# nl1xx/simple-multimodal

Hardware: AMD Instinct MI355X
Metric: fusion fwd+bwd samples/sec at B=16 d=768 (higher is better)
Workload: dtype bf16

## Files before the change

### include/mmfusion.h

```cpp
#ifndef MMFUSION_H
#define MMFUSION_H

#include <stddef.h>
#include <stdint.h>

#ifdef __cplusplus
extern "C" {
#endif

#define MMF_ABI_VERSION 1

enum {
  MMF_OK = 0,
  MMF_E_SHAPE = -1,
  MMF_E_DTYPE = -2,
  MMF_E_ALIGN = -3,
  MMF_E_LAUNCH = -4,
  MMF_E_UNSUPPORTED = -5
};

int mmf_version(void);
const char* mmf_last_error(void);
int mmf_device_cu_count(void);

#define MMF_GEMM_MAX_PROBLEMS 48
enum { MMF_GEMM_NT = 0, MMF_GEMM_NN = 1, MMF_GEMM_TN = 2 };
enum {
  MMF_EPI_BIAS = 1,
  MMF_EPI_RELU = 2,
  MMF_EPI_MASK_AUX = 4,
  MMF_EPI_ADD_AUX = 8,
  MMF_EPI_ACCUM = 16,
  MMF_EPI_COLSUM_A = 32,
  MMF_EPI_DROPOUT = 64
};

typedef struct mmf_gemm_problem {
  const void* A;
  const void* B;
  void* C;
  const float* bias;
  const void* aux;
  int32_t M, N, K;
  int32_t lda, ldb, ldc, ldaux;
} mmf_gemm_problem;

int mmf_gemm_grouped(const mmf_gemm_problem* problems, int num_problems, int layout,
                     int epilogue, int out_f32, void* stream);
typedef struct mmf_gemm_extra {
  float alpha;
  float dropout_p;
  const uint64_t* rng_state;
  uint32_t site;
} mmf_gemm_extra;
int mmf_gemm_grouped_ex(const mmf_gemm_problem* problems, int num_problems, int layout, int epilogue,
                        int out_f32, const mmf_gemm_extra* extra, void* stream);

int mmf_gemm_select_impl(int impl);
int mmf_gemm_last_impl(void);
int mmf_gemm_set_persistent_workgroups(int n);
int mmf_gemm7_set_tile_n(int n);
int mmf_gemm7_last_tile_n(void);
int mmf_gemm7_tile_n(const mmf_gemm_problem* problems, int num_problems, int workgroups);

#define MMF_SKINNY_MAX_PROBLEMS 24
typedef struct mmf_skinny_problem {
  const void* X;
  const void* W;
  void* Y;
  const float* bias;
  const void* aux;
  int32_t M, N, K;
  int32_t ldx, ldw, ldy, ldaux;
} mmf_skinny_problem;
int mmf_skinny_linear_fwd(const mmf_skinny_problem* problems, int num_problems, int flags, int out_f32, void* stream);
int mmf_skinny_linear_dgrad(const mmf_skinny_problem* problems, int num_problems, int flags, float alpha, int out_f32,
                            void* stream);
int mmf_skinny_last_strip(void);
typedef struct mmf_skinny_problem_ex {
  mmf_skinny_problem p;
  void* Y2;
  const void* gate;
  void* dz;
  int32_t ldy2, ldgate, lddz, reserved;
} mmf_skinny_problem_ex;
typedef struct mmf_skinny_extra {
  int32_t x_f32;
  int32_t gate_f32;
  float gate_scale;
  float dropout_p;
  const uint64_t* rng_state;
  uint32_t site;
  uint32_t reserved;
} mmf_skinny_extra;
int mmf_skinny_linear_fwd_ex(const mmf_skinny_problem_ex* problems, int num_problems, int flags, int out_f32,
                             const mmf_skinny_extra* extra, void* stream);
int mmf_skinny_linear_dgrad_ex(const mmf_skinny_problem_ex* problems, int num_problems, int flags, float alpha, int out_f32,
                               const mmf_skinny_extra* extra, void* stream);

int mmf_fusion_loss(const float* logits, int ldl, const int64_t* targets, int B, int C, float label_smoothing,
                    const float* const* extra, const float* extra_w, int n_extra, float* loss, float* dlogits, void* stream);
int mmf_modality_dropout(const float* const* x, float* const* y, float* keep, int B, int d, float p,
                         const uint64_t* rng_state, uint32_t site, int draw, void* stream);

int mmf_distill_kl(const float* student, int lds, const float* teacher, int ldt, int B, int C, float temperature,
                   float* loss, float* dstudent, void* stream);
int mmf_fusion_loss_kd(const float* logits, int ldl, const int64_t* targets, int B, int C, float label_smoothing,
                       const float* const* extra, const float* extra_w, int n_extra,
                       const float* teacher, int ldt, float temperature, float kd_weight,
                       float* loss, float* dlogits, void* stream);

int mmf_robust_head_fwd(const float* const f[3], const float* h, const float* W2, const float* b2,
                        const float* const Wm[3], const float* const bm[3], int avail, float* a, float* const p[3],
                        float* wn, float* y, int B, int d, int C, void* stream);
int mmf_robust_head_bwd(const float* const f[3], const float* h, const float* W2, const float* const Wm[3],
                        const float* a, const float* const p[3], const float* wn, int avail, const float* g,
                        const float* const dP[3], const float* dA, const float* dN, float* const df[3], float* dh,
                        float* dW2, float* db2, float* const dWm[3], float* const dbm[3], int B, int d, int C, void* stream);

int mmf_fewshot_proto_fwd(const float* const s[3], float* sf, float* mean, int n_way, int n_shot, int d, void* stream);
int mmf_fewshot_proto_bwd(const float* dmean, const float* dsf, float* ds, int n_way, int n_shot, int d, void* stream);
int mmf_fewshot_dist_fwd(const float* const q[3], const float* P, float* qf, float* dist, float* pred, int Nq, int n_way,
                         int d, void* stream);
int mmf_fewshot_dist_bwd(const float* qf, const float* P, const float* dist, const float* pred, const float* gdist,
                         const float* gpred, float* dq, float* dp, int Nq, int n_way, int d, void* stream);

#define MMF_EVAL_MAX_HEADS 4
#define MMF_EVAL_NSUMS 4
int mmf_eval_accumulate(const float* const* logits, const int* ld, int n_heads, const int64_t* targets, int B, int C,
                        float label_smoothing, int64_t* counts, double* sums, int64_t* pred_out, int64_t* target_out,
                        float* prob_out, int64_t row0, int64_t capacity, void* stream);

#define MMF_ATTN_MAX_PROBLEMS 12
typedef struct mmf_attn_problem {
  const void* Q; const void* K; const void* V;
  void* O;
  float* LSE;
  const void* dO;
  float* delta;
  void* dQ; void* dK; void* dV;
  int32_t B, H, Tq, Tk;
  int32_t ldq, ldk, ldv, ldo;
} mmf_attn_problem;

int mmf_attn_fwd_grouped(const mmf_attn_problem* problems, int num_problems, int head_dim,
                         float scale, void* stream);
int mmf_attn_bwd_grouped(const mmf_attn_problem* problems, int num_problems, int head_dim,
                         float scale, void* stream);
int mmf_attn_fwd_grouped_ex(const mmf_attn_problem* problems, int num_problems, int head_dim, float scale,
                            float dropout_p, const uint64_t* rng_state, uint32_t site, void* stream);
int mmf_attn_select_impl(int impl);
int mmf_attn_bwd_grouped_ex(const mmf_attn_problem* problems, int num_problems, int head_dim, float scale,
                            float dropout_p, const uint64_t* rng_state, uint32_t site, void* stream);

#define MMF_LN_MAX_PROBLEMS 8
typedef struct mmf_ln_problem {
  const void* x;
  void* y;
  const float* gamma;
  const float* beta;
  float* mean;
  float* rstd;
  const void* dy;
  void* dx;
  float* dgamma;
  float* dbeta;
  int32_t rows;
} mmf_ln_problem;

int mmf_layernorm_fwd_grouped(const mmf_ln_problem* problems, int num_problems, int d, float eps,
                              void* stream);
size_t mmf_layernorm_bwd_workspace_bytes(int d);
int mmf_layernorm_bwd_grouped(const mmf_ln_problem* problems, int num_problems, int d,
                              void* workspace, size_t workspace_bytes, void* stream);
int mmf_layernorm_last_form(void);

int mmf_cast_f32_to_bf16(const float* src, void* dst, int64_t n, void* stream);
int mmf_cast_bf16_to_f32(const void* src, float* dst, int64_t n, void* stream);
int mmf_cast_f32_to_bf16_2d(const float* src, void* dst, int rows, int cols, int ld_src, void* stream);
int mmf_cast_bf16_to_f32_scaled(const void* src, float* dst, int64_t n, float scale, void* stream);
int mmf_add3_bf16(const void* a, const void* b, const void* c, void* y, int64_t n, void* stream);
#define MMF_ADD3_MAX 8
typedef struct mmf_add3_problem {
  const void* a; const void* b; const void* c;
  void* y;
  int64_t n;
} mmf_add3_problem;
int mmf_add3_grouped(const mmf_add3_problem* problems, int num_problems, void* stream);
#define MMF_ADDN_MAX 8
int mmf_addn_bf16(const void* const* xs, int n, void* y, int64_t numel, int out_f32, void* stream);
#define MMF_ADDN_GROUP_MAX 4
typedef struct mmf_addn_problem {
  const void* x[MMF_ADDN_MAX];
  void* y;
  int64_t numel;
  int32_t n;
} mmf_addn_problem;
int mmf_addn_grouped(const mmf_addn_problem* problems, int num_problems, void* stream);
int mmf_meanpool_fwd(const void* x, void* y, int B, int T, int d, int ldy, void* stream);
int mmf_meanpool_bwd(const void* dy, void* dx, int B, int T, int d, int lddy, void* stream);
#define MMF_POOL_MAX 4
int mmf_meanpool_cat_fwd(const void* const* xs, const int* Ts, int n, void* y, int B, int d, int ldy, void* stream);
int mmf_meanpool_cat_bwd(const void* dy, void* const* dxs, const int* Ts, int n, int B, int d, int lddy, void* stream);
int mmf_colsum_bf16(const void* x, float* out, int M, int N, int ldx, void* stream);
#define MMF_COLSUM_MAX_PROBLEMS 24
typedef struct mmf_colsum_problem {
  const void* x;
  float* out;
  int32_t M, N, ldx;
} mmf_colsum_problem;
int mmf_colsum_grouped(const mmf_colsum_problem* problems, int num_problems, void* stream);
int mmf_dropout(const void* x, void* y, int64_t n, int is_f32, float p, const uint64_t* rng_state,
                uint32_t site, void* stream);
#define MMF_ZERO_MAX_RANGES 48
int mmf_zero_ranges_f32(float* base, const int64_t* starts, const int64_t* ends, int n, void* stream);
int mmf_relu_bwd_bf16(const void* dy, const void* y, void* dx, int64_t n, void* stream);
int mmf_relu_bwd_mixed(const void* dy, int dy_f32, const void* y, int y_f32, void* dx, int64_t n, void* stream);

typedef struct mmf_gat3_params {
  int32_t B, heads, C, relu;
  float negative_slope, dropout_p;
  const uint64_t* rng_state;
  uint32_t site;
} mmf_gat3_params;
int mmf_gat3_dense_fwd(const float* h, const float* att_src, const float* att_dst, const float* bias,
                       void* y_bf16, void* pooled_bf16, float* alpha, float* sdots,
                       const mmf_gat3_params* p, void* stream);
int mmf_gat3_dense_bwd(const float* h, const float* att_src, const float* att_dst, const void* y_bf16,
                       const float* alpha, const float* sdots, const void* dy_bf16, const void* dpooled_bf16,
                       float* dh, float* datt_src, float* datt_dst, float* dbias,
                       const mmf_gat3_params* p, void* stream);
int mmf_infonce_fwd(const float* const z[3], float* const n[3], float* inv_norm, float* losses, float* lse,
                    int B, int D, float temperature, void* stream);
int mmf_infonce_bwd(const float* const n[3], const float* inv_norm, const float* lse, const float* const dn[3],
                    const float* const dloss[3], float* const dz[3], int B, int D, float temperature, void* stream);
int mmf_adaptive_combine_fwd(const float* hp, const float* W2, const float* b2, const float* attended,
                             float* aw, void* weighted_bf16, int B, int d, void* stream);
int mmf_adaptive_combine_bwd(const float* hp, const float* W2, const float* attended, const float* aw,
                             const void* dweighted_bf16, const float* daw, float* dattended, float* dhp,
                             float* dW2, float* db2, int B, int d, void* stream);
int mmf_adaptive_attn_weights(const void* qkv_bf16, float* w, int B, int heads, int head_dim, void* stream);
int mmf_attn_weights_mean(const void* qkv_bf16, float* w, int B, int T, int heads, int head_dim, void* stream);
int mmf_linear_narrow_fwd(const float* x, const float* W, const float* b, float* y, int M, int N, int K, void* stream);
int mmf_linear_narrow_bwd(const float* x, const float* W, const float* dy, float* dx, float* dW, float* db,
                          int M, int N, int K, void* stream);
int mmf_stack3_embed_fwd(const float* f0, const float* f1, const float* f2, const float* emb, void* x_bf16,
                         int B, int d, int ldf, void* stream);
int mmf_stack3_embed_bwd(const void* dx_bf16, float* d0, float* d1, float* d2, float* demb, int B, int d, int ldd,
                         void* stream);
int mmf_rowmask_apply(const float* x, const float* mask, float* y, int B, int d, void* stream);

int mmf_sqnorm_f32(const float* x, int64_t n, float* out, void* stream);
int mmf_adamw_advance(int64_t* step, float* hparams, const double* sched, void* stream);
int mmf_adamw_step(float* master, const float* grad, float* exp_avg, float* exp_avg_sq, void* shadow_bf16,
                   int64_t n, const float* hparams, const float* gnorm_sq, void* stream);

int mmf_gemm_f32_grouped(const mmf_gemm_problem* problems, int num_problems, int layout, int epilogue, float alpha,
                         void* stream);
int mmf_gemm_f32_batched(const mmf_gemm_problem* problem, int layout, int epilogue, float alpha, int nb0, int nb1,
                         const int64_t strideA[2], const int64_t strideB[2], const int64_t strideC[2], void* stream);
int mmf_softmax_rows_f32(float* S, int64_t rows, int cols, float scale, void* stream);
int mmf_softmax_bwd_rows_f32(const float* P, float* dP, int64_t rows, int cols, float scale, void* stream);
int mmf_layernorm_f32_fwd(const float* x, float* y, const float* gamma, const float* beta, float* mean, float* rstd,
                          int rows, int d, float eps, void* stream);
int mmf_layernorm_f32_bwd(const float* x, const float* dy, const float* gamma, const float* mean, const float* rstd,
                          float* dx, float* dgamma, float* dbeta, int rows, int d, void* stream);

typedef struct mmf_bilstm_args {
  const void* gx;
  const void* w_hh[2];
  const float* b_ih[2];
  const float* b_hh[2];
  void* y;
  float* gates;
  float* cell;
  const void* dy;
  void* dgates;
  int32_t T, B, H;
} mmf_bilstm_args;
size_t mmf_bilstm_workspace_bytes(void);
int mmf_bilstm_layer_fwd(const mmf_bilstm_args* args, void* workspace, size_t workspace_bytes, void* stream);
int mmf_bilstm_layer_bwd(const mmf_bilstm_args* args, void* workspace, size_t workspace_bytes, void* stream);

int mmf_swap01(const void* in, void* out, int n0, int n1, int d, int in_f32, int out_f32, void* stream);

int mmf_vit_patchify(const float* pixels, void* patches_bf16, int N, int C, int H, int W, int P, void* stream);
int mmf_vit_embed_tokens(const void* patch_emb_bf16, const float* cls, const float* pos, void* tokens_bf16, int N, int T, int d,
                         void* stream);
int mmf_bias_gelu_bf16(void* x_bf16, const float* bias, int64_t rows, int cols, int ld, void* stream);

#define MMF_W2V_STATS_SLOTS 128
int mmf_w2v_conv0_stats(const float* wave, const float* weight, float* stats, float* partial, int N, int L, int C0, int k0, int s0,
                        void* stream);
int mmf_w2v_conv0_norm_gelu(const float* wave, const float* weight, const float* stats, const float* gamma, const float* beta,
                            void* out_bf16, int N, int L, int C0, int k0, int s0, int k1, int s1, float eps, void* stream);
int mmf_w2v_gelu_window(const void* x_bf16, void* out_bf16, int N, int T_in, int C, int k, int s, void* stream);
int mmf_w2v_posconv(const void* x_bf16, const void* w_bf16, const float* bias, void* y_bf16, int N, int T, int C, int groups, int k,
                    void* stream);

int mmf_deberta_embed(const int64_t* ids, const float* embeds, const float* table, const float* gamma, const float* beta, float eps,
                      const void* mask, int mask_kind, void* out_bf16, int64_t rows, int d, int vocab, void* stream);
int mmf_deberta_attn_fwd(const void* qkv_bf16, const void* posq_bf16, const void* posk_bf16, int ld_pos, const int* idx,
                         const void* mask, int mask_kind, void* out_bf16, int n, int H, int T, int S, int head_dim, float scale,
                         void* stream);

int mmf_video_prepare(const uint8_t* frames, const uint8_t* live, const float* brightness, const uint8_t* flip, float* pixels,
                      int N, int Hs, int Ws, int H, int W, int bgr, void* stream);
int mmf_video_prepare_patches(const uint8_t* frames, const uint8_t* live, const float* brightness, const uint8_t* flip,
                              void* patches_bf16, int N, int Hs, int Ws, int H, int W, int P, int bgr, void* stream);
int mmf_audio_resample(const float* wave, const int* len, const float* table, int64_t table_elems, float* out, int B, int C,
                       int64_t Ls, int64_t L, int orig, int new_, int width, void* stream);
int mmf_audio_augment(const float* x, float* out, const uint8_t* noise_on, const int* stretch_len, const uint64_t* rng_state,
                      uint32_t site, int B, int64_t L, void* stream);

#ifdef __cplusplus
}
#endif
#endif
```

### simple-multimodal_amd/csrc/gemm.hip

```cpp
#include "mmf_internal.h"
#include <stdlib.h>

int mmf_gemm2_launch(const mmf_gemm_problem* problems, int num_problems, int layout, int epilogue,
                     int out_f32, const mmf_gemm_extra* extra, hipStream_t s);
int mmf_gemm6_launch(const mmf_gemm_problem* problems, int num_problems, int layout, int epilogue,
                     int out_f32, const mmf_gemm_extra* extra, hipStream_t s);
bool mmf_gemm6_supports(const mmf_gemm_problem* problems, int num_problems, int layout);
bool mmf_gemm6_supports_epi(int epilogue, int out_f32);
int mmf_gemm7_launch(const mmf_gemm_problem* problems, int num_problems, int layout, int epilogue,
                     int out_f32, const mmf_gemm_extra* extra, hipStream_t s);
bool mmf_gemm7_supports(const mmf_gemm_problem* problems, int num_problems, int layout, int epilogue, int out_f32, const mmf_gemm_extra* extra);

static bool impl_built(int v) { return v == 0 || v == 2 || v == 6 || v == 7; }
static int g_gemm_impl = [] {
  const char* e = getenv("MMF_GEMM_IMPL");
  const int v = (e && e[0] >= '0' && e[0] <= '9') ? e[0] - '0' : 0;
  return impl_built(v) ? v : 0;
}();

static int auto_impl(const mmf_gemm_problem* p, int n, int layout) {
  long tiles = 0;
  for (int i = 0; i < n; ++i) tiles += (long)((p[i].M + 255) / 256) * ((p[i].N + 255) / 256);
  static const int cus = [] { int c = mmf_device_cu_count(); return c > 0 ? c : 256; }();
  const long need = layout == MMF_GEMM_TN ? (cus + 1) / 2 : (cus + 3) / 4;
  return (tiles >= need && mmf_gemm6_supports(p, n, layout)) ? 6 : 2;
}
static int gemm_impl() { return g_gemm_impl; }
static thread_local int t_last_impl = 0;
extern "C" int mmf_gemm_last_impl(void) { return t_last_impl; }
extern "C" int mmf_gemm_select_impl(int impl) {
  if (!impl_built(impl))
    MMF_FAIL(MMF_E_UNSUPPORTED, "mmf_gemm_select_impl: generation %d is not built (0 = automatic, 2, 6, 7; 1 / 3 left in round 3, 4 / 5 in round 4)", impl);
  g_gemm_impl = impl;
  return MMF_OK;
}

extern "C" int mmf_gemm_grouped(const mmf_gemm_problem* problems, int num_problems, int layout,
                                int epilogue, int out_f32, void* stream) {
  return mmf_gemm_grouped_ex(problems, num_problems, layout, epilogue, out_f32, nullptr, stream);
}

extern "C" int mmf_gemm_grouped_ex(const mmf_gemm_problem* problems, int num_problems, int layout,
                                   int epilogue, int out_f32, const mmf_gemm_extra* extra, void* stream) {
  if (!problems || num_problems <= 0 || num_problems > MMF_GEMM_MAX_PROBLEMS)
    MMF_FAIL(MMF_E_SHAPE, "mmf_gemm_grouped: num_problems=%d out of range [1,%d]", num_problems,
             MMF_GEMM_MAX_PROBLEMS);
  if (layout < MMF_GEMM_NT || layout > MMF_GEMM_TN)
    MMF_FAIL(MMF_E_UNSUPPORTED, "mmf_gemm_grouped: unknown layout %d", layout);
  if ((epilogue & MMF_EPI_ACCUM) && !out_f32)
    MMF_FAIL(MMF_E_UNSUPPORTED, "mmf_gemm_grouped: MMF_EPI_ACCUM needs f32 output");
  if ((epilogue & MMF_EPI_MASK_AUX) && (epilogue & MMF_EPI_ADD_AUX))
    MMF_FAIL(MMF_E_UNSUPPORTED, "mmf_gemm_grouped: MASK_AUX and ADD_AUX are exclusive");
  if ((epilogue & MMF_EPI_COLSUM_A) && (layout != MMF_GEMM_TN || (epilogue & MMF_EPI_BIAS)))
    MMF_FAIL(MMF_E_UNSUPPORTED, "mmf_gemm_grouped: COLSUM_A is a TN (wgrad) epilogue and excludes BIAS");
  if (epilogue & MMF_EPI_DROPOUT) {
    if (!extra || !extra->rng_state || !(extra->dropout_p >= 0.f) || extra->dropout_p >= 1.f)
      MMF_FAIL(MMF_E_SHAPE, "mmf_gemm_grouped_ex: MMF_EPI_DROPOUT needs rng_state and 0 <= p < 1");
  }
  int impl = gemm_impl();
  const bool pinned = impl != 0;
  if (impl == 0) impl = auto_impl(problems, num_problems, layout);
  const bool ok6 = mmf_gemm6_supports(problems, num_problems, layout) && mmf_gemm6_supports_epi(epilogue, out_f32);
  if (impl == 6 && !pinned && mmf_gemm7_supports(problems, num_problems, layout, epilogue, out_f32, extra)) impl = 7;
  if (impl == 7 && !mmf_gemm7_supports(problems, num_problems, layout, epilogue, out_f32, extra)) impl = 6;
  if (impl == 6 && !ok6) impl = 2;
  t_last_impl = impl;
  for (int i = 0; i < num_problems; ++i) {
    const mmf_gemm_problem& p = problems[i];
    if (p.M <= 0 || p.N <= 0 || p.K <= 0)
      MMF_FAIL(MMF_E_SHAPE, "mmf_gemm_grouped[%d]: empty problem M=%d N=%d K=%d", i, p.M, p.N, p.K);
    if (!p.A || !p.B || !p.C) MMF_FAIL(MMF_E_SHAPE, "mmf_gemm_grouped[%d]: null operand", i);
    if ((epilogue & (MMF_EPI_BIAS | MMF_EPI_COLSUM_A)) && !p.bias) MMF_FAIL(MMF_E_SHAPE, "mmf_gemm_grouped[%d]: bias is null", i);
    if ((epilogue & (MMF_EPI_MASK_AUX | MMF_EPI_ADD_AUX)) && !p.aux)
      MMF_FAIL(MMF_E_SHAPE, "mmf_gemm_grouped[%d]: aux is null", i);
    const int a_cols = (layout == MMF_GEMM_TN) ? p.M : p.K;
    const int b_cols = (layout == MMF_GEMM_NT) ? p.K : p.N;
    if ((a_cols & 7) || (b_cols & 7) || (p.lda & 7) || (p.ldb & 7) || (p.N & 3) || (p.ldc & 3) ||
        ((epilogue & (MMF_EPI_MASK_AUX | MMF_EPI_ADD_AUX)) && (p.ldaux & 3)))
      MMF_FAIL(MMF_E_ALIGN, "mmf_gemm_grouped[%d]: M=%d N=%d K=%d lda=%d ldb=%d ldc=%d ldaux=%d violate "
               "the 8-element (operands) / 4-element (output) granularity", i, p.M, p.N, p.K, p.lda,
               p.ldb, p.ldc, p.ldaux);
    if (p.lda < a_cols || p.ldb < b_cols || p.ldc < p.N)
      MMF_FAIL(MMF_E_SHAPE, "mmf_gemm_grouped[%d]: leading dimension smaller than the row", i);
    if (!mmf_aligned16(p.A) || !mmf_aligned16(p.B) || !mmf_aligned16(p.C) ||
        (p.bias && !mmf_aligned16(p.bias)) || (p.aux && (reinterpret_cast<uintptr_t>(p.aux) & 7)))
      MMF_FAIL(MMF_E_ALIGN, "mmf_gemm_grouped[%d]: operand pointers must be 16-byte aligned", i);
  }
  hipStream_t s = static_cast<hipStream_t>(stream);
  if (impl == 2) return mmf_gemm2_launch(problems, num_problems, layout, epilogue, out_f32, extra, s);
  if (impl == 6) return mmf_gemm6_launch(problems, num_problems, layout, epilogue, out_f32, extra, s);
  if (impl == 7) return mmf_gemm7_launch(problems, num_problems, layout, epilogue, out_f32, extra, s);
  MMF_FAIL(MMF_E_UNSUPPORTED, "mmf_gemm_grouped: kernel generation %d is not built (2, 6, 7)", impl);
}
```

### simple-multimodal_amd/csrc/gemm7.hip

```cpp
#include <algorithm>
#include <vector>
#include "gemm6_parts.h"

namespace {

constexpr int TILE = 256 * BK * 2, PPO = BK / 8;
template <int TN> struct Form {
  static constexpr int BNT = 64 * TN, TILE_B = BNT * BK * 2, STAGE = TILE + TILE_B, PPB = TN, PPW = PPO + PPB;
  static constexpr int LDS = NS * STAGE + 4 * 8192;
};
static_assert(Form<4>::LDS == 160 * 1024 && Form<3>::LDS == 144 * 1024, "LDS of the two forms");

struct TileSrc {
  const unsigned short* Ab;
  const unsigned short* Bb;
  int recA, recB, stepB, KT;
};
struct TileDst {
  int pi, m0, n0;
};

__device__ __forceinline__ int to_sgpr(int x) {
  int r;
  asm volatile("s_nop 0\n\tv_readfirstlane_b32 %0, %1\n\ts_nop 4" : "=s"(r) : "v"(x));
  return r;
}

template <bool B_KR, int TN>
__device__ __forceinline__ void locate_tile(const GemmArgs& args, const int total_tiles, const int orig, TileSrc& s, TileDst& d, int& lda, int& ldb) {
  const int bid = to_sgpr(mmf_xcd_tile(orig, total_tiles, args.xcd_granule));
  int pi = 0;
  while (pi + 1 < args.nprob && bid >= args.tile_start[pi + 1]) ++pi;
  const mmf_gemm_problem& P = args.p[pi];
  int m0, n0;
  tile_origin<Form<TN>::BNT>(P, bid - args.tile_start[pi], m0, n0);
  m0 = to_sgpr(m0);
  n0 = to_sgpr(n0);
  d.pi = pi; d.m0 = m0; d.n0 = n0;
  lda = P.lda; ldb = P.ldb;
  s.Ab = static_cast<const unsigned short*>(P.A) + (size_t)m0 * P.lda;
  s.Bb = static_cast<const unsigned short*>(P.B) + (B_KR ? (size_t)n0 : (size_t)n0 * P.ldb);
  s.recA = (int)(((long)(P.M - m0 - 1) * P.lda + P.K) * 2);
  s.recB = (int)((B_KR ? ((long)(P.K - 1) * P.ldb + (P.N - n0)) : ((long)(P.N - n0 - 1) * P.ldb + P.K)) * 2);
  s.stepB = (B_KR ? BK * P.ldb : BK) * 2;
  s.KT = P.K / BK;
}

template <int CT, int TN>
__device__ __forceinline__ void drain_tile(const GemmArgs& args, const int pi, const mmf_gemm_problem& P, const int mb, const int nb,
                                           f32x16_t (&acc)[TN][4], char* region, const int lane) {
  constexpr bool AUX = (CT & (MMF_EPI_MASK_AUX | MMF_EPI_ADD_AUX)) != 0;
  constexpr bool DROP = (CT & MMF_EPI_DROPOUT) != 0;
  const unsigned drop_key = DROP ? mmf_rng_key(*args.rng_state, args.site, (unsigned)args.orig[pi]) : 0u;
  const float drop_scale = DROP ? 1.f / (1.f - (float)args.drop_thresh * (1.f / 4294967296.f)) : 1.f;
  const float alpha = (CT & MMF_EPI_MASK_AUX) ? args.alpha : 1.f;
  const int r = lane & 31, h = lane >> 5, q = lane >> 4, cq = lane & 15;
  const unsigned wr_base = (unsigned)(r * 256 + 8 * h + 16 * (r & 15));
  const unsigned rd_base = (unsigned)(q * 256 + ((cq ^ q) << 4));
  auto acc_at = [&](int c) { return region + (wr_base ^ (unsigned)(c << 4)); };
  auto row_at = [&](int it) { return region + it * 1024 + (rd_base ^ (unsigned)((it & 3) << 6)); };
  const bool col_ok = cq < 4 * TN && nb + 8 * cq < P.N;
  const __amdgpu_buffer_rsrc_t crs = __builtin_amdgcn_make_buffer_rsrc(P.C, 0, (int)((((long)P.M - 1) * P.ldc + P.N) * 2), 0x00020000);
  const __amdgpu_buffer_rsrc_t ars = __builtin_amdgcn_make_buffer_rsrc(const_cast<void*>(AUX ? P.aux : P.C), 0,
                                                                       AUX ? (int)((((long)P.M - 1) * P.ldaux + P.N) * 2) : 0, 0x00020000);
  const unsigned c_off0 = col_ok ? (unsigned)(((long)(mb + q) * P.ldc + nb + 8 * cq) * 2) : 0x80000000u;
  const unsigned a_off0 = col_ok ? (unsigned)(((long)(mb + q) * P.ldaux + nb + 8 * cq) * 2) : 0x80000000u;
  const unsigned c_row4 = (unsigned)(4 * P.ldc * 2), a_row4 = (unsigned)(4 * P.ldaux * 2);

  u32x4_t auxr[2][8];
  auto load_aux = [&](int tm, int slot) {
#pragma unroll
    for (int it = 0; it < 8; ++it)
      auxr[slot][it] = __builtin_bit_cast(u32x4_t, __builtin_amdgcn_raw_buffer_load_b128(ars, a_off0 + (unsigned)(8 * tm + it) * a_row4, 0, 0));
  };
  if constexpr (AUX) { load_aux(0, 0); load_aux(1, 1); }
#pragma unroll
  for (int tm = 0; tm < 4; ++tm) {
    u32x2_t axv[TN][4];
    if constexpr (AUX) {
#pragma unroll
      for (int it = 0; it < 8; ++it) *reinterpret_cast<u32x4_t*>(row_at(it)) = auxr[tm & 1][it];
#pragma unroll
      for (int tn = 0; tn < TN; ++tn)
#pragma unroll
        for (int g = 0; g < 4; ++g) axv[tn][g] = *reinterpret_cast<const u32x2_t*>(acc_at(4 * tn + g));
      __builtin_amdgcn_sched_barrier(0);
      if (tm + 2 < 4) load_aux(tm + 2, tm & 1);
      __builtin_amdgcn_sched_barrier(0);
    }
#pragma unroll
    for (int tn = 0; tn < TN; ++tn) {
      asm volatile("" : "+a"(acc[tn][tm]));
#pragma unroll
      for (int g = 0; g < 4; ++g) {
        f32x4_t v = {acc[tn][tm][4 * g], acc[tn][tm][4 * g + 1], acc[tn][tm][4 * g + 2], acc[tn][tm][4 * g + 3]};
        if constexpr (CT & MMF_EPI_RELU) {
#pragma unroll
          for (int e = 0; e < 4; ++e) v[e] = fmaxf(v[e], 0.f);
        }
        if constexpr (DROP) {
          const unsigned idx = (unsigned)(mb + 32 * tm + r) * (unsigned)P.N + (unsigned)(nb + 32 * tn + 8 * g + 4 * h);
#pragma unroll
          for (int e = 0; e < 4; ++e) v[e] = mmf_keep(drop_key, idx + e, args.drop_thresh) ? v[e] * drop_scale : 0.f;
        }
        if constexpr (AUX) {
          const u32x2_t a = axv[tn][g];
          const float a0 = bf16lo(a[0]), a1 = bf16hi(a[0]), a2 = bf16lo(a[1]), a3 = bf16hi(a[1]);
          if constexpr (CT & MMF_EPI_MASK_AUX) {
            v[0] = a0 > 0.f ? v[0] * alpha : 0.f; v[1] = a1 > 0.f ? v[1] * alpha : 0.f;
            v[2] = a2 > 0.f ? v[2] * alpha : 0.f; v[3] = a3 > 0.f ? v[3] * alpha : 0.f;
          } else {
            v[0] += a0; v[1] += a1; v[2] += a2; v[3] += a3;
          }
        }
        *reinterpret_cast<u32x2_t*>(acc_at(4 * tn + g)) = u32x2_t{pack_bf16x2(v[0], v[1]), pack_bf16x2(v[2], v[3])};
      }
      __builtin_amdgcn_sched_barrier(0);
    }
    u32x4_t w[8];
#pragma unroll
    for (int it = 0; it < 8; ++it) w[it] = *reinterpret_cast<const u32x4_t*>(row_at(it));
#pragma unroll
    for (int it = 0; it < 8; ++it) __builtin_amdgcn_raw_buffer_store_b128(w[it], crs, c_off0 + (unsigned)(8 * tm + it) * c_row4, 0, 0);
    __builtin_amdgcn_sched_barrier(0);
  }
}

template <bool B_KR, int CT, int TN>
__device__ __forceinline__ void gemm7_body(const GemmArgs& args, const int total_tiles, char* smem) {
  constexpr bool A_KR = false;
  using F = Form<TN>;
  constexpr int BNT = F::BNT, STAGE = F::STAGE, PPW = F::PPW, NMF = 4 * TN, NRD = 4 + TN;
  constexpr int WA = BK, WB = B_KR ? BNT : BK;

  const int tid = threadIdx.x, lane = tid & 63;
  const int wave = __builtin_amdgcn_readfirstlane(tid >> 6);
  const int wm = wave >> 1, wn = wave & 1;
  const int nwg = gridDim.x;
  const int wid = blockIdx.x;
  auto walk = [&](int round) { return round * nwg + ((round & 1) ? nwg - 1 - wid : wid); };
  int round = 0;
  int orig = walk(0);
  TileSrc ns;
  TileDst cd, nd;
  int KT, lda, ldb;
  locate_tile<B_KR, TN>(args, total_tiles, orig, ns, cd, lda, ldb);
  KT = ns.KT;

  unsigned voff[PPW], voffn[PPW];
  auto set_voff = [&](unsigned (&v)[PPW], int la, int lb) {
#pragma unroll
    for (int i = 0; i < PPO; ++i) v[i] = piece_voff<A_KR>(wave + 4 * i, la, lane);
#pragma unroll
    for (int i = 0; i < TN; ++i) v[PPO + i] = piece_voff<B_KR, BNT>(wave + 4 * i, lb, lane);
  };
  set_voff(voff, lda, ldb);
  char* const my_pieces = smem + wave * 1024;

  struct Desc { int lo, hi, rec; };
  auto mkdesc = [](const unsigned short* p, int rec) {
    const unsigned long long a = (unsigned long long)(uintptr_t)p;
    return Desc{(int)(unsigned)a, (int)((unsigned)(a >> 32) & 0xffffu), rec};
  };
  auto advance = [](Desc& d, int bytes) {
    const unsigned long long a = (((unsigned long long)(unsigned)d.hi << 32) | (unsigned)d.lo) + (unsigned long long)bytes;
    d.lo = (int)(unsigned)a; d.hi = (int)(unsigned)(a >> 32);
    int r;
    asm("s_sub_i32 %0, %1, %2\n\ts_max_i32 %0, %0, 0" : "=s"(r) : "s"(d.rec), "s"(bytes) : "scc");
    d.rec = r;
  };
  Desc dA = mkdesc(ns.Ab, ns.recA);
  Desc dB = mkdesc(ns.Bb, ns.recB);
  constexpr int stepA = BK * 2;
  int stepB = ns.stepB;
  const unsigned lds_pieces = (unsigned)(uintptr_t)(const __attribute__((address_space(3))) char*)my_pieces;
  auto hot_piece = [&](auto ic, const unsigned ring_base) {
    constexpr int I = decltype(ic)::value, OFF = I < PPO ? I * 4096 : TILE + (I - PPO) * 4096;
    const Desc& d = I < PPO ? dA : dB;
    const i32x4_t q = {d.lo, d.hi, d.rec, 0x00020000};
    int m0w;
    asm volatile("s_add_i32 %0, %1, %4\n\ts_nop 0\n\tbuffer_load_dwordx4 %2, %3, 0 offen lds" : "={m0}"(m0w) : "s"(ring_base), "v"(voff[I]), "s"(q), "n"(OFF) : "memory");
    __builtin_amdgcn_sched_barrier(0);
  };

#pragma unroll
  for (int s = 0; s < NS; ++s) {
    const unsigned rb = lds_pieces + (unsigned)(s * STAGE);
    hot_piece(std::integral_constant<int, 0>{}, rb); hot_piece(std::integral_constant<int, 1>{}, rb);
    hot_piece(std::integral_constant<int, 2>{}, rb); hot_piece(std::integral_constant<int, 3>{}, rb);
    if (s + 1 < NS) {
      hot_piece(std::integral_constant<int, 4>{}, rb); hot_piece(std::integral_constant<int, 5>{}, rb);
      hot_piece(std::integral_constant<int, 6>{}, rb);
      if constexpr (TN == 4) hot_piece(std::integral_constant<int, 7>{}, rb);
      advance(dA, stepA); advance(dB, stepB);
    }
  }

  bool has_next = walk(1) < total_tiles;
  nd = cd;
  if (has_next) {
    int la, lb;
    locate_tile<B_KR, TN>(args, total_tiles, walk(1), ns, nd, la, lb);
    set_voff(voffn, la, lb);
  } else {
    ns.recA = 0; ns.recB = 0; ns.stepB = 0;
#pragma unroll
    for (int i = 0; i < PPW; ++i) voffn[i] = voff[i];
  }

  unsigned la0, la1, lb0, lb1;
  Frag4<A_KR>::lane_parts(WA, lane, la0, la1);
  Frag4<B_KR>::lane_parts(WB, lane, lb0, lb1);
  const unsigned smem_base = (unsigned)(uintptr_t)(const __attribute__((address_space(3))) char*)smem;
  const unsigned qa = (unsigned)((WA / 32) * 2048 * 4 * wm);
  const unsigned qb = (unsigned)(B_KR ? 512 * TN * wn : (WB / 32) * 2048 * TN * wn);
  la0 += smem_base + qa; la1 += smem_base + qa;
  lb0 += smem_base + TILE + qb; lb1 += smem_base + TILE + qb;

  f32x16_t acc[TN][4];

  constexpr bool use_bias = (CT & MMF_EPI_BIAS) != 0;
  float bcur[TN] = {};
  auto load_bias = [&](float (&b)[TN], const TileDst& d) {
    const mmf_gemm_problem& P = args.p[d.pi];
    const __amdgpu_buffer_rsrc_t brs = __builtin_amdgcn_make_buffer_rsrc(const_cast<float*>(P.bias), 0, P.N * 4, 0x00020000);
    const unsigned off = (unsigned)((d.n0 + 32 * TN * wn + (lane & 31)) * 4);
#pragma unroll
    for (int tn = 0; tn < TN; ++tn)
      b[tn] = __uint_as_float((unsigned)__builtin_amdgcn_raw_buffer_load_b32(brs, off + (unsigned)(32 * tn * 4), 0, 0));
  };
  auto split3 = [&](float x) {
    const bool lo = lane < 32;
    const unsigned hh = __float_as_uint(x) & 0xffff0000u;
    const float r1 = x - __uint_as_float(hh);
    const unsigned mm = __float_as_uint(r1) & 0xffff0000u;
    const float r2 = r1 - __uint_as_float(mm);
    const unsigned ll = __float_as_uint(r2) & 0xffff0000u;
    const u32x4_t w = {lo ? ((hh >> 16) | mm) : 0u, lo ? (ll >> 16) : 0u, 0u, 0u};
    return __builtin_bit_cast(bf16x8_t, w);
  };
  auto bias_init = [&](const float (&b)[TN]) {
    const f32x16_t zero = {0.f, 0.f, 0.f, 0.f, 0.f, 0.f, 0.f, 0.f, 0.f, 0.f, 0.f, 0.f, 0.f, 0.f, 0.f, 0.f};
    const u32x4_t ow = {lane < 32 ? 0x3f803f80u : 0u, lane < 32 ? 0x00003f80u : 0u, 0u, 0u};
    u32x4_t ones[4] = {ow, ow, ow, ow};
#pragma unroll
    for (int tm = 0; tm < 4; ++tm) asm volatile("" : "+v"(ones[tm]));
#pragma unroll
    for (int tn = 0; tn < TN; ++tn) {
      u32x4_t bw = __builtin_bit_cast(u32x4_t, use_bias ? split3(b[tn]) : __builtin_bit_cast(bf16x8_t, u32x4_t{0u, 0u, 0u, 0u}));
      asm volatile("" : "+v"(bw));
#pragma unroll
      for (int tm = 0; tm < 4; ++tm) {
        acc[tn][tm] = __builtin_amdgcn_mfma_f32_32x32x16_bf16(__builtin_bit_cast(bf16x8_t, bw), __builtin_bit_cast(bf16x8_t, ones[tm]), zero, 0, 0, 0);
        __builtin_amdgcn_sched_barrier(0);
      }
    }
  };
  if constexpr (use_bias) load_bias(bcur, cd);

  vm_wait<PPW * (NS - 2) + PPO>();
  __builtin_amdgcn_s_barrier();
  Frag4<A_KR> fa[2];
  Frag4<B_KR, TN> fb[2];
  fa[0].template issue<WA, 0, 0>(la0, la1);
  fb[0].template issue<WB, 0, 0>(lb0, lb1);
  frag_wait(fa[0], fb[0]);

  auto mf = [&](const Frag4<A_KR>& a, const Frag4<B_KR, TN>& b, int i) {
    const int tm = i / TN, tn = i % TN;
    acc[tn][tm] = __builtin_amdgcn_mfma_f32_32x32x16_bf16(b.get(tn), a.get(tm), acc[tn][tm], 0, 0, 0);
    asm volatile("" ::"a"(acc[tn][tm]));
    __builtin_amdgcn_sched_barrier(0);
  };

  auto stage = [&](const unsigned g, const int kt, const int ksw) {
    unsigned long long swmask;
    const Desc nA = mkdesc(ns.Ab, ns.recA), nB = mkdesc(ns.Bb, ns.recB);
    const unsigned so = (g % NS) * STAGE;
    const unsigned ring_cur = lds_pieces + so, ring_prev = lds_pieces + ((g + NS - 1) % NS) * STAGE;
#pragma unroll
    for (int i = 0; i < NMF; ++i) {
      mf(fa[0], fb[0], i);
      if (i < NRD) MMF_G6_READ(TN, fa[1], fb[1], 1, i, so);
      if (i == NRD)     hot_piece(std::integral_constant<int, 4>{}, ring_prev);
      if (i == NRD + 2) hot_piece(std::integral_constant<int, 5>{}, ring_prev);
      if (i == NRD + 4) hot_piece(std::integral_constant<int, 6>{}, ring_prev);
      if constexpr (TN == 4) { if (i == NRD + 6) hot_piece(std::integral_constant<int, 7>{}, ring_prev); }
    }
    frag_wait(fa[1], fb[1]);
    const unsigned sn = ((g + 1) % NS) * STAGE;
#pragma unroll
    for (int i = 0; i < 4; ++i) mf(fa[1], fb[1], i);
    vm_wait<PPW * (NS - 2)>();
    __builtin_amdgcn_s_barrier();
    __builtin_amdgcn_sched_barrier(0);
#pragma unroll
    for (int i = 4; i < NMF; ++i) {
      mf(fa[1], fb[1], i);
      if (i < 4 + NRD) MMF_G6_READ(TN, fa[0], fb[0], 0, i - 4, sn);
      if (i == 4) {
        advance(dA, stepA);
        advance(dB, stepB);
        asm volatile("" ::"s"(dA.lo), "s"(dA.hi), "s"(dA.rec), "s"(dB.lo), "s"(dB.hi), "s"(dB.rec));
        __builtin_amdgcn_sched_barrier(0);
      }
      if (i == 5) {
        asm volatile("s_cmp_eq_u32 %8, %16\n\t"
                     "s_cselect_b32 %0, %9, %0\n\ts_cselect_b32 %1, %10, %1\n\ts_cselect_b32 %2, %11, %2\n\t"
                     "s_cselect_b32 %3, %12, %3\n\ts_cselect_b32 %4, %13, %4\n\ts_cselect_b32 %5, %14, %5\n\t"
                     "s_cselect_b32 %6, %15, %6\n\ts_cselect_b64 %7, -1, 0"
                     : "+s"(dA.lo), "+s"(dA.hi), "+s"(dA.rec), "+s"(dB.lo), "+s"(dB.hi), "+s"(dB.rec), "+s"(stepB), "=s"(swmask)
                     : "s"(kt), "s"(nA.lo), "s"(nA.hi), "s"(nA.rec), "s"(nB.lo), "s"(nB.hi), "s"(nB.rec), "s"(ns.stepB), "s"(ksw)
                     : "scc");
        __builtin_amdgcn_sched_barrier(0);
      }
      if (i == 6) {
        asm volatile("v_cndmask_b32_e64 %0, %0, %4, %8\n\tv_cndmask_b32_e64 %1, %1, %5, %8\n\t"
                     "v_cndmask_b32_e64 %2, %2, %6, %8\n\tv_cndmask_b32_e64 %3, %3, %7, %8"
                     : "+v"(voff[0]), "+v"(voff[1]), "+v"(voff[2]), "+v"(voff[3])
                     : "v"(voffn[0]), "v"(voffn[1]), "v"(voffn[2]), "v"(voffn[3]), "s"(swmask));
        __builtin_amdgcn_sched_barrier(0);
      }
      if (i == 7) {
        if constexpr (TN == 4)
          asm volatile("v_cndmask_b32_e64 %0, %0, %4, %8\n\tv_cndmask_b32_e64 %1, %1, %5, %8\n\t"
                       "v_cndmask_b32_e64 %2, %2, %6, %8\n\tv_cndmask_b32_e64 %3, %3, %7, %8"
                       : "+v"(voff[4]), "+v"(voff[5]), "+v"(voff[6]), "+v"(voff[7])
                       : "v"(voffn[4]), "v"(voffn[5]), "v"(voffn[6]), "v"(voffn[7]), "s"(swmask));
        else
          asm volatile("v_cndmask_b32_e64 %0, %0, %3, %6\n\tv_cndmask_b32_e64 %1, %1, %4, %6\n\t"
                       "v_cndmask_b32_e64 %2, %2, %5, %6"
                       : "+v"(voff[4]), "+v"(voff[5]), "+v"(voff[6])
                       : "v"(voffn[4]), "v"(voffn[5]), "v"(voffn[6]), "s"(swmask));
        __builtin_amdgcn_sched_barrier(0);
      }
      if (i == NMF - 4) hot_piece(std::integral_constant<int, 0>{}, ring_cur);
      if (i == NMF - 3) hot_piece(std::integral_constant<int, 1>{}, ring_cur);
      if (i == NMF - 2) hot_piece(std::integral_constant<int, 2>{}, ring_cur);
      if (i == NMF - 1) hot_piece(std::integral_constant<int, 3>{}, ring_cur);
    }
    frag_wait(fa[0], fb[0]);
  };

  char* const region = smem + NS * STAGE + wave * 8192;
  unsigned g = 0;
  for (;;) {
    bias_init(bcur);
    const int ksw = KT - NS;
    for (int kt = 0; kt < KT; ++kt, ++g) stage(g, kt, ksw);
    const mmf_gemm_problem& P = args.p[cd.pi];
    const int mb = cd.m0 + 128 * wm, nb = cd.n0 + 32 * TN * wn;
    if constexpr (use_bias) { if (has_next) load_bias(bcur, nd); }
#ifndef MMF_G7_NODRAIN
    drain_tile<CT & ~MMF_EPI_BIAS, TN>(args, cd.pi, P, mb, nb, acc, region, lane);
#else
    if (lane == 0 && mb == -1) static_cast<volatile unsigned short*>(P.C)[0] = (unsigned short)acc[0][0][0];
#endif
    if (!has_next) break;
    ++round;
    orig = walk(round);
    cd = nd;
    KT = ns.KT;
    has_next = walk(round + 1) < total_tiles;
    if (has_next) {
      int la, lb;
      locate_tile<B_KR, TN>(args, total_tiles, walk(round + 1), ns, nd, la, lb);
      set_voff(voffn, la, lb);
    } else {
      ns.recA = 0; ns.recB = 0; ns.stepB = 0;
    }
  }
  vm_wait<0>();
}

template <bool B_KR, int CT, int TN>
__global__ __launch_bounds__(NTHREADS, 1)
void gemm7_persistent_kernel(const GemmArgs args, const int total_tiles) {
  __shared__ __attribute__((aligned(1024))) char smem[Form<TN>::LDS];
  gemm7_body<B_KR, CT, TN>(args, total_tiles, smem);
}

template <bool B_KR, int CT>
void launch7(const GemmArgs& a, int total, int grid, int tile_n, hipStream_t s) {
  if (tile_n == 192) hipLaunchKernelGGL((gemm7_persistent_kernel<B_KR, CT, 3>), dim3(grid), dim3(NTHREADS), 0, s, a, total);
  else               hipLaunchKernelGGL((gemm7_persistent_kernel<B_KR, CT, 4>), dim3(grid), dim3(NTHREADS), 0, s, a, total);
}
bool launch7_select(int layout, int eflags, const GemmArgs* a, int total, int grid, hipStream_t s, int tile_n = 256) {
  if (layout == MMF_GEMM_NT) {
    if (eflags == 0)                                      { if (a) launch7<false, 0>(*a, total, grid, tile_n, s); return true; }
    if (eflags == MMF_EPI_BIAS)                           { if (a) launch7<false, MMF_EPI_BIAS>(*a, total, grid, tile_n, s); return true; }
    if (eflags == (MMF_EPI_BIAS | MMF_EPI_RELU))          { if (a) launch7<false, MMF_EPI_BIAS | MMF_EPI_RELU>(*a, total, grid, tile_n, s); return true; }
    if (eflags == (MMF_EPI_BIAS | MMF_EPI_ADD_AUX))       { if (a) launch7<false, MMF_EPI_BIAS | MMF_EPI_ADD_AUX>(*a, total, grid, tile_n, s); return true; }
    if (eflags == (MMF_EPI_BIAS | MMF_EPI_RELU | MMF_EPI_DROPOUT)) {
      if (a) launch7<false, MMF_EPI_BIAS | MMF_EPI_RELU | MMF_EPI_DROPOUT>(*a, total, grid, tile_n, s);
      return true;
    }
  } else if (layout == MMF_GEMM_NN) {
    if (eflags == 0)                                      { if (a) launch7<true, 0>(*a, total, grid, tile_n, s); return true; }
    if (eflags == MMF_EPI_MASK_AUX)                       { if (a) launch7<true, MMF_EPI_MASK_AUX>(*a, total, grid, tile_n, s); return true; }
    if (eflags == MMF_EPI_ADD_AUX)                        { if (a) launch7<true, MMF_EPI_ADD_AUX>(*a, total, grid, tile_n, s); return true; }
  }
  return false;
}
}

static int g_persistent_wgs = [] { const char* e = getenv("MMF_GEMM7_WGS"); const int v = e ? atoi(e) : 0; return v > 0 ? v : 0; }();
extern "C" int mmf_gemm_set_persistent_workgroups(int n) {
  if (n < 0 || n > 65536) MMF_FAIL(MMF_E_SHAPE, "mmf_gemm_set_persistent_workgroups: %d not in 0..65536", n);
  g_persistent_wgs = n;
  return MMF_OK;
}
static int g_tile_n = 0;
static thread_local int t_last_tile_n = 0;
extern "C" int mmf_gemm7_set_tile_n(int n) {
  if (n != 0 && n != 256 && n != 192) MMF_FAIL(MMF_E_SHAPE, "mmf_gemm7_set_tile_n: %d is not 0, 256 or 192", n);
  g_tile_n = n;
  return MMF_OK;
}
extern "C" int mmf_gemm7_last_tile_n(void) { return t_last_tile_n; }

namespace {
int persistent_grid_cap() {
  static const int cus = [] { int c = mmf_device_cu_count(); return c > 0 ? c : 256; }();
  return g_persistent_wgs > 0 ? g_persistent_wgs : cus;
}
int tiles_of(const mmf_gemm_problem& p, int bn) { return ((p.M + BM - 1) / BM) * ((p.N + bn - 1) / bn); }
long long walk_makespan(const mmf_gemm_problem* problems, const int* order, int n, int bn, int cap, int granule) {
  int start[MMF_GEMM_MAX_PROBLEMS + 1];
  start[0] = 0;
  for (int i = 0; i < n; ++i) start[i + 1] = start[i] + tiles_of(problems[order[i]], bn);
  const int total = start[n], grid = total < cap ? total : cap;
  if (total == 0) return 0;
  static thread_local std::vector<long long> load;
  load.assign(grid, 0);
  for (int o = 0; o < total; ++o) {
    const int round = o / grid, pos = o % grid, wid = (round & 1) ? grid - 1 - pos : pos;
    const int bid = mmf_xcd_tile(o, total, granule);
    const int pi = (int)(std::upper_bound(start, start + n + 1, bid) - start) - 1;
    load[wid] += (long long)problems[order[pi]].K * bn;
  }
  return *std::max_element(load.begin(), load.end());
}
struct TileNMemo {
  int cap, granule, n, width;
  int mnk[3 * MMF_GEMM_MAX_PROBLEMS];
};
int pick_tile_n(const mmf_gemm_problem* problems, const int* order, int n, int cap) {
  const int granule = mmf_xcd_granule();
  static thread_local TileNMemo memo[16];
  static thread_local int used = 0, next = 0;
  TileNMemo key;
  key.cap = cap; key.granule = granule; key.n = n;
  for (int i = 0; i < n; ++i) {
    const mmf_gemm_problem& p = problems[order[i]];
    key.mnk[3 * i] = p.M; key.mnk[3 * i + 1] = p.N; key.mnk[3 * i + 2] = p.K;
  }
  for (int e = 0; e < used; ++e) {
    const TileNMemo& m = memo[e];
    if (m.cap == cap && m.granule == granule && m.n == n && std::equal(key.mnk, key.mnk + 3 * n, m.mnk)) return m.width;
  }
  key.width = walk_makespan(problems, order, n, 192, cap, granule) < walk_makespan(problems, order, n, 256, cap, granule) ? 192 : 256;
  memo[next] = key;
  next = (next + 1) % 16;
  if (used < 16) ++used;
  return key.width;
}
void sort_by_k(const mmf_gemm_problem* problems, int n, int* order) {
  for (int i = 0; i < n; ++i) order[i] = i;
  std::stable_sort(order, order + n, [&](int x, int y) { return problems[x].K > problems[y].K; });
}
}

extern "C" int mmf_gemm7_tile_n(const mmf_gemm_problem* problems, int num_problems, int workgroups) {
  if (!problems || num_problems < 1 || num_problems > MMF_GEMM_MAX_PROBLEMS || workgroups < 0)
    MMF_FAIL(MMF_E_SHAPE, "mmf_gemm7_tile_n: %d problems, %d workgroups", num_problems, workgroups);
  int order[MMF_GEMM_MAX_PROBLEMS];
  sort_by_k(problems, num_problems, order);
  return pick_tile_n(problems, order, num_problems, workgroups > 0 ? workgroups : persistent_grid_cap());
}

bool mmf_gemm7_supports(const mmf_gemm_problem* problems, int num_problems, int layout, int epilogue, int out_f32, const mmf_gemm_extra* extra) {
  if (out_f32 || !launch7_select(layout, epilogue, nullptr, 0, 0, nullptr)) return false;
  if (extra && extra->alpha != 1.f && !(layout == MMF_GEMM_NN && epilogue == MMF_EPI_MASK_AUX)) return false;
  if ((epilogue & MMF_EPI_DROPOUT) && !(extra && extra->rng_state)) return false;
  for (int i = 0; i < num_problems; ++i) {
    const mmf_gemm_problem& p = problems[i];
    if (p.K % BK || p.K < (NS + 1) * BK || (p.N & 7) || (p.ldc & 7) || (p.aux && ((p.ldaux & 7) || !mmf_aligned16(p.aux)))) return false;
  }
  return true;
}

int mmf_gemm7_launch(const mmf_gemm_problem* problems, int num_problems, int layout, int epilogue,
                     int out_f32, const mmf_gemm_extra* extra, hipStream_t s) {
  if (!mmf_gemm7_supports(problems, num_problems, layout, epilogue, out_f32, extra))
    MMF_FAIL(MMF_E_UNSUPPORTED, "mmf_gemm_grouped: the persistent kernel takes NT / NN launches with bf16 output, K %% 32 == 0, K >= %d, N and the "
             "leading dimensions of C / aux multiples of 8, and the flag sets of the fusion step (alpha only with the NN ReLU mask)", (NS + 1) * BK);
  GemmArgs a;
  a.nprob = num_problems;
  a.epi = epilogue;
  a.xcd_granule = mmf_xcd_granule();
  a.alpha = extra ? extra->alpha : 1.f;
  a.drop_thresh = (extra && (epilogue & MMF_EPI_DROPOUT)) ? mmf_drop_thresh(extra->dropout_p) : 0u;
  a.site = extra ? extra->site : 0u;
  a.rng_state = extra ? reinterpret_cast<const unsigned long long*>(extra->rng_state) : nullptr;
  int total = 0;
  int order[MMF_GEMM_MAX_PROBLEMS];
  sort_by_k(problems, num_problems, order);
  const int cap = persistent_grid_cap();
  const int tile_n = g_tile_n ? g_tile_n : pick_tile_n(problems, order, num_problems, cap);
  for (int i = 0; i < num_problems; ++i) {
    const mmf_gemm_problem& p = problems[order[i]];
    const size_t a_bytes = (size_t)p.M * p.lda * 2;
    const size_t b_bytes = (size_t)(layout == MMF_GEMM_NT ? p.N : p.K) * p.ldb * 2;
    const size_t c_bytes = (size_t)p.M * p.ldc * 2, x_bytes = p.aux ? (size_t)p.M * p.ldaux * 2 : 0;
    if (a_bytes >= 0x7fffffffull || b_bytes >= 0x7fffffffull || c_bytes >= 0x7fffffffull || x_bytes >= 0x7fffffffull)
      MMF_FAIL(MMF_E_UNSUPPORTED, "mmf_gemm_grouped[%d]: operand larger than 2 GiB", i);
    a.tile_start[i] = total;
    total += tiles_of(p, tile_n);
    a.p[i] = p;
    a.orig[i] = (short)order[i];
  }
  a.tile_start[num_problems] = total;
  const int grid = total < cap ? total : cap;
  t_last_tile_n = tile_n;
  launch7_select(layout, epilogue, &a, total, grid, s, tile_n);
  MMF_CHECK_LAUNCH("mmf_gemm_grouped(v7)");
  return MMF_OK;
}
```

### simple-multimodal_amd/csrc/layernorm.hip

```cpp
#include "mmf_internal.h"

namespace {

constexpr int ROWS_PER_BLOCK = 4;
constexpr int MAX_CH = 4;

constexpr int FWD_BLOCKS = 1024, FWD_BLOCKS_LARGE = 2048;
constexpr long long FWD_LARGE_ROWS = 20000;
constexpr int BWD_BLOCKS_LANE = 512;
constexpr int BWD_BLOCKS_CHUNK = 2048;

struct LnArgs {
  int nprob;
  int d;
  float eps;
  float* ws;
  int blk_start[MMF_LN_MAX_PROBLEMS + 1];
  mmf_ln_problem p[MMF_LN_MAX_PROBLEMS];
};

template <int NCH>
__global__ __launch_bounds__(256)
void ln_fwd_kernel(const LnArgs a) {
  const int pi = mmf_group_problem(a.blk_start, a.nprob, blockIdx.x);
  const mmf_ln_problem& P = a.p[pi];
  const int lane = threadIdx.x & 63, wave = threadIdx.x >> 6;
  const int row = ((int)blockIdx.x - a.blk_start[pi]) * ROWS_PER_BLOCK + wave;
  if (row >= P.rows) return;
  const int d = a.d;
  const unsigned short* x = static_cast<const unsigned short*>(P.x) + (size_t)row * d;
  float v[NCH][8];
  float s = 0.f;
#pragma unroll
  for (int c = 0; c < NCH; ++c) {
    const int col = (c * 64 + lane) * 8;
    if (col < d) {
      unpack8(*reinterpret_cast<const u32x4_t*>(x + col), v[c]);
#pragma unroll
      for (int e = 0; e < 8; ++e) s += v[c][e];
    } else {
#pragma unroll
      for (int e = 0; e < 8; ++e) v[c][e] = 0.f;
    }
  }
  const float mean = wave_sum(s) / (float)d;
  float q = 0.f;
#pragma unroll
  for (int c = 0; c < NCH; ++c) {
    const int col = (c * 64 + lane) * 8;
    if (col < d) {
#pragma unroll
      for (int e = 0; e < 8; ++e) { const float t = v[c][e] - mean; q += t * t; }
    }
  }
  const float rstd = rsqrtf(wave_sum(q) / (float)d + a.eps);
  unsigned short* y = static_cast<unsigned short*>(P.y) + (size_t)row * d;
#pragma unroll
  for (int c = 0; c < NCH; ++c) {
    const int col = (c * 64 + lane) * 8;
    if (col < d) {
      const f32x4_t g0 = *reinterpret_cast<const f32x4_t*>(P.gamma + col);
      const f32x4_t g1 = *reinterpret_cast<const f32x4_t*>(P.gamma + col + 4);
      const f32x4_t b0 = *reinterpret_cast<const f32x4_t*>(P.beta + col);
      const f32x4_t b1 = *reinterpret_cast<const f32x4_t*>(P.beta + col + 4);
      float o[8];
#pragma unroll
      for (int e = 0; e < 4; ++e) {
        o[e] = (v[c][e] - mean) * rstd * g0[e] + b0[e];
        o[e + 4] = (v[c][e + 4] - mean) * rstd * g1[e] + b1[e];
      }
      *reinterpret_cast<u32x4_t*>(y + col) = pack8(o);
    }
  }
  if (lane == 0) { P.mean[row] = mean; P.rstd[row] = rstd; }
}

template <int NV, int H8>
struct LaneCols {
  static constexpr int EP = 8 * NV + 4 * H8, D = 512 * NV + 256 * H8;
  struct Bf16 { u32x4_t v[NV > 0 ? NV : 1]; u32x2_t t; };
  static __device__ __forceinline__ void load(const unsigned short* row, int lane, Bf16& r) {
#pragma unroll
    for (int c = 0; c < NV; ++c) r.v[c] = *reinterpret_cast<const u32x4_t*>(row + 512 * c + 8 * lane);
    if (H8) r.t = *reinterpret_cast<const u32x2_t*>(row + 512 * NV + 4 * lane);
  }
  static __device__ __forceinline__ void unpack(const Bf16& r, float (&f)[EP]) {
#pragma unroll
    for (int c = 0; c < NV; ++c) {
      float t[8];
      unpack8(r.v[c], t);
#pragma unroll
      for (int e = 0; e < 8; ++e) f[8 * c + e] = t[e];
    }
    if (H8) { f[8 * NV] = bf16lo(r.t[0]); f[8 * NV + 1] = bf16hi(r.t[0]); f[8 * NV + 2] = bf16lo(r.t[1]); f[8 * NV + 3] = bf16hi(r.t[1]); }
  }
  static __device__ __forceinline__ void store(unsigned short* row, int lane, const float (&o)[EP]) {
#pragma unroll
    for (int c = 0; c < NV; ++c) {
      const u32x4_t w = {pack_bf16x2(o[8 * c], o[8 * c + 1]), pack_bf16x2(o[8 * c + 2], o[8 * c + 3]),
                         pack_bf16x2(o[8 * c + 4], o[8 * c + 5]), pack_bf16x2(o[8 * c + 6], o[8 * c + 7])};
      *reinterpret_cast<u32x4_t*>(row + 512 * c + 8 * lane) = w;
    }
    if (H8) {
      const u32x2_t w = {pack_bf16x2(o[8 * NV], o[8 * NV + 1]), pack_bf16x2(o[8 * NV + 2], o[8 * NV + 3])};
      *reinterpret_cast<u32x2_t*>(row + 512 * NV + 4 * lane) = w;
    }
  }
  static __device__ __forceinline__ void load_f32(const float* p, int lane, float (&f)[EP]) {
#pragma unroll
    for (int c = 0; c < NV; ++c)
#pragma unroll
      for (int h = 0; h < 2; ++h) {
        const f32x4_t g = *reinterpret_cast<const f32x4_t*>(p + 512 * c + 8 * lane + 4 * h);
#pragma unroll
        for (int e = 0; e < 4; ++e) f[8 * c + 4 * h + e] = g[e];
      }
    if (H8) {
      const f32x4_t g = *reinterpret_cast<const f32x4_t*>(p + 512 * NV + 4 * lane);
#pragma unroll
      for (int e = 0; e < 4; ++e) f[8 * NV + e] = g[e];
    }
  }
  static __device__ __forceinline__ void store_f32(float* p, int lane, const float (&f)[EP]) {
#pragma unroll
    for (int c = 0; c < NV; ++c)
#pragma unroll
      for (int h = 0; h < 2; ++h)
        *reinterpret_cast<f32x4_t*>(p + 512 * c + 8 * lane + 4 * h) =
            f32x4_t{f[8 * c + 4 * h], f[8 * c + 4 * h + 1], f[8 * c + 4 * h + 2], f[8 * c + 4 * h + 3]};
    if (H8) *reinterpret_cast<f32x4_t*>(p + 512 * NV + 4 * lane) = f32x4_t{f[8 * NV], f[8 * NV + 1], f[8 * NV + 2], f[8 * NV + 3]};
  }
};

template <int NV, int H8>
__global__ __launch_bounds__(256)
void ln_fwd_lane_kernel(const LnArgs a) {
  using LC = LaneCols<NV, H8>;
  constexpr int EP = LC::EP, d = LC::D;
  const int pi = mmf_group_problem(a.blk_start, a.nprob, blockIdx.x);
  const mmf_ln_problem& P = a.p[pi];
  const int lane = threadIdx.x & 63, wave = threadIdx.x >> 6;
  const int nblk = a.blk_start[pi + 1] - a.blk_start[pi];
  const float inv_d = 1.f / (float)d;
  float gam[EP], bet[EP];
  LC::load_f32(P.gamma, lane, gam);
  LC::load_f32(P.beta, lane, bet);
  auto fetch = [&](int row, typename LC::Bf16& r) { LC::load(static_cast<const unsigned short*>(P.x) + (size_t)row * d, lane, r); };
  const int step = nblk * ROWS_PER_BLOCK;
  int row = ((int)blockIdx.x - a.blk_start[pi]) * ROWS_PER_BLOCK + wave;
  typename LC::Bf16 cur, nxt;
  if (row < P.rows) fetch(row, cur);
  for (; row < P.rows; row += step) {
    const bool more = row + step < P.rows;
    if (more) fetch(row + step, nxt);
    float v[EP];
    LC::unpack(cur, v);
    float s = 0.f;
#pragma unroll
    for (int e = 0; e < EP; ++e) s += v[e];
    const float mean = wave_sum(s) * inv_d;
    float q = 0.f;
#pragma unroll
    for (int e = 0; e < EP; ++e) { v[e] -= mean; q += v[e] * v[e]; }
    const float rstd = rsqrtf(wave_sum(q) * inv_d + a.eps);
    float o[EP];
#pragma unroll
    for (int e = 0; e < EP; ++e) o[e] = v[e] * rstd * gam[e] + bet[e];
    LC::store(static_cast<unsigned short*>(P.y) + (size_t)row * d, lane, o);
    if (lane == 0) { P.mean[row] = mean; P.rstd[row] = rstd; }
    if (more) cur = nxt;
  }
}

template <int NCH>
__global__ __launch_bounds__(256)
void ln_bwd_kernel(const LnArgs a) {
  __shared__ float red[2][3][NCH * 512];
  const int pi = mmf_group_problem(a.blk_start, a.nprob, blockIdx.x);
  const mmf_ln_problem& P = a.p[pi];
  const int lane = threadIdx.x & 63, wave = threadIdx.x >> 6;
  const int nblk = a.blk_start[pi + 1] - a.blk_start[pi];
  const int d = a.d;
  float dg[NCH][8], db[NCH][8];
#pragma unroll
  for (int c = 0; c < NCH; ++c)
#pragma unroll
    for (int e = 0; e < 8; ++e) { dg[c][e] = 0.f; db[c][e] = 0.f; }

  for (int row = ((int)blockIdx.x - a.blk_start[pi]) * ROWS_PER_BLOCK + wave; row < P.rows;
       row += nblk * ROWS_PER_BLOCK) {
    const unsigned short* x = static_cast<const unsigned short*>(P.x) + (size_t)row * d;
    const unsigned short* dy = static_cast<const unsigned short*>(P.dy) + (size_t)row * d;
    const float mean = P.mean[row], rstd = P.rstd[row];
    float xh[NCH][8], g[NCH][8];
    float s1 = 0.f, s2 = 0.f;
#pragma unroll
    for (int c = 0; c < NCH; ++c) {
      const int col = (c * 64 + lane) * 8;
      if (col < d) {
        float xv[8], dv[8];
        unpack8(*reinterpret_cast<const u32x4_t*>(x + col), xv);
        unpack8(*reinterpret_cast<const u32x4_t*>(dy + col), dv);
        const f32x4_t g0 = *reinterpret_cast<const f32x4_t*>(P.gamma + col);
        const f32x4_t g1 = *reinterpret_cast<const f32x4_t*>(P.gamma + col + 4);
#pragma unroll
        for (int e = 0; e < 8; ++e) {
          const float gam = e < 4 ? g0[e] : g1[e - 4];
          xh[c][e] = (xv[e] - mean) * rstd;
          g[c][e] = dv[e] * gam;
          s1 += g[c][e];
          s2 += g[c][e] * xh[c][e];
          dg[c][e] += dv[e] * xh[c][e];
          db[c][e] += dv[e];
        }
      } else {
#pragma unroll
        for (int e = 0; e < 8; ++e) { xh[c][e] = 0.f; g[c][e] = 0.f; }
      }
    }
    const float c1 = wave_sum(s1) / (float)d, c2 = wave_sum(s2) / (float)d;
    unsigned short* dx = static_cast<unsigned short*>(P.dx) + (size_t)row * d;
#pragma unroll
    for (int c = 0; c < NCH; ++c) {
      const int col = (c * 64 + lane) * 8;
      if (col < d) {
        float o[8];
#pragma unroll
        for (int e = 0; e < 8; ++e) o[e] = rstd * (g[c][e] - c1 - xh[c][e] * c2);
        *reinterpret_cast<u32x4_t*>(dx + col) = pack8(o);
      }
    }
  }
  if (wave > 0) {
#pragma unroll
    for (int c = 0; c < NCH; ++c)
#pragma unroll
      for (int e = 0; e < 8; ++e) {
        red[0][wave - 1][(c * 64 + lane) * 8 + e] = dg[c][e];
        red[1][wave - 1][(c * 64 + lane) * 8 + e] = db[c][e];
      }
  }
  __syncthreads();
  if (wave == 0) {
    float* wsg = a.ws + (size_t)blockIdx.x * 2 * d;
#pragma unroll
    for (int c = 0; c < NCH; ++c) {
      const int col = (c * 64 + lane) * 8;
      if (col < d) {
        f32x4_t g0, g1, b0, b1;
#pragma unroll
        for (int e = 0; e < 8; ++e) {
          float sg = dg[c][e], sb = db[c][e];
#pragma unroll
          for (int w = 0; w < 3; ++w) { sg += red[0][w][col + e]; sb += red[1][w][col + e]; }
          if (e < 4) { g0[e] = sg; b0[e] = sb; } else { g1[e - 4] = sg; b1[e - 4] = sb; }
        }
        *reinterpret_cast<f32x4_t*>(wsg + col) = g0;
        *reinterpret_cast<f32x4_t*>(wsg + col + 4) = g1;
        *reinterpret_cast<f32x4_t*>(wsg + d + col) = b0;
        *reinterpret_cast<f32x4_t*>(wsg + d + col + 4) = b1;
      }
    }
  }
}

template <int NV, int H8>
__global__ __launch_bounds__(256)
void ln_bwd_lane_kernel(const LnArgs a) {
  using LC = LaneCols<NV, H8>;
  constexpr int EP = LC::EP, d = LC::D;
  __shared__ float red[2][3][64 * EP];
  const int pi = mmf_group_problem(a.blk_start, a.nprob, blockIdx.x);
  const mmf_ln_problem& P = a.p[pi];
  const int lane = threadIdx.x & 63, wave = threadIdx.x >> 6;
  const int nblk = a.blk_start[pi + 1] - a.blk_start[pi];
  const float inv_d = 1.f / (float)d;
  float gam[EP], dg[EP], db[EP];
  LC::load_f32(P.gamma, lane, gam);
#pragma unroll
  for (int e = 0; e < EP; ++e) { dg[e] = 0.f; db[e] = 0.f; }

  struct Row { typename LC::Bf16 x, dy; float mean, rstd; };
  auto fetch = [&](int row, Row& r) {
    LC::load(static_cast<const unsigned short*>(P.x) + (size_t)row * d, lane, r.x);
    LC::load(static_cast<const unsigned short*>(P.dy) + (size_t)row * d, lane, r.dy);
    r.mean = P.mean[row];
    r.rstd = P.rstd[row];
  };
  const int step = nblk * ROWS_PER_BLOCK;
  int row = ((int)blockIdx.x - a.blk_start[pi]) * ROWS_PER_BLOCK + wave;
  Row cur, nxt;
  if (row < P.rows) fetch(row, cur);
  for (; row < P.rows; row += step) {
    const bool more = row + step < P.rows;
    if (more) fetch(row + step, nxt);
    float xv[EP], dv[EP];
    LC::unpack(cur.x, xv);
    LC::unpack(cur.dy, dv);
    const float mean = cur.mean, rstd = cur.rstd;
    float s1 = 0.f, s2 = 0.f;
#pragma unroll
    for (int e = 0; e < EP; ++e) {
      xv[e] = (xv[e] - mean) * rstd;
      const float g = dv[e] * gam[e];
      s1 += g;
      s2 += g * xv[e];
      dg[e] += dv[e] * xv[e];
      db[e] += dv[e];
      dv[e] = g;
    }
    const float c1 = wave_sum(s1) * inv_d, c2 = wave_sum(s2) * inv_d;
    float o[EP];
#pragma unroll
    for (int e = 0; e < EP; ++e) o[e] = rstd * (dv[e] - c1 - xv[e] * c2);
    LC::store(static_cast<unsigned short*>(P.dx) + (size_t)row * d, lane, o);
    if (more) cur = nxt;
  }
  if (wave > 0) {
#pragma unroll
    for (int e = 0; e < EP; ++e) { red[0][wave - 1][e * 64 + lane] = dg[e]; red[1][wave - 1][e * 64 + lane] = db[e]; }
  }
  __syncthreads();
  if (wave == 0) {
    float* wsg = a.ws + (size_t)blockIdx.x * 2 * d;
#pragma unroll
    for (int e = 0; e < EP; ++e)
#pragma unroll
      for (int w = 0; w < 3; ++w) { dg[e] += red[0][w][e * 64 + lane]; db[e] += red[1][w][e * 64 + lane]; }
    LC::store_f32(wsg, lane, dg);
    LC::store_f32(wsg + d, lane, db);
  }
}

constexpr int FIN_SLICES = 64;
__global__ __launch_bounds__(256)
void ln_bwd_finalize_kernel(const LnArgs a) {
  const int pi = blockIdx.y;
  const int col = blockIdx.x * 256 + threadIdx.x;
  if (col >= a.d) return;
  const int b0 = a.blk_start[pi], nb = a.blk_start[pi + 1] - b0;
  const int per = (nb + FIN_SLICES - 1) / FIN_SLICES;
  const int lo = b0 + blockIdx.z * per, hi = min(b0 + nb, lo + per);
  if (lo >= hi) return;
  float sg[4] = {0.f, 0.f, 0.f, 0.f}, sb[4] = {0.f, 0.f, 0.f, 0.f};
  int b = lo;
  for (; b + 4 <= hi; b += 4) {
#pragma unroll
    for (int u = 0; u < 4; ++u) {
      const float* w = a.ws + (size_t)(b + u) * 2 * a.d;
      sg[u] += w[col];
      sb[u] += w[a.d + col];
    }
  }
  for (; b < hi; ++b) {
    const float* w = a.ws + (size_t)b * 2 * a.d;
    sg[0] += w[col];
    sb[0] += w[a.d + col];
  }
  atomicAdd(a.p[pi].dgamma + col, (sg[0] + sg[1]) + (sg[2] + sg[3]));
  atomicAdd(a.p[pi].dbeta + col, (sb[0] + sb[1]) + (sb[2] + sb[3]));
}

thread_local int t_last_form = 0;

using LnKernel = void (*)(const LnArgs);
const LnKernel CHUNK_FWD[MAX_CH] = {ln_fwd_kernel<1>, ln_fwd_kernel<2>, ln_fwd_kernel<3>, ln_fwd_kernel<4>};
const LnKernel CHUNK_BWD[MAX_CH] = {ln_bwd_kernel<1>, ln_bwd_kernel<2>, ln_bwd_kernel<3>, ln_bwd_kernel<4>};
struct LaneWidth { int d, form; LnKernel fwd, bwd; };
template <int NV, int H8>
constexpr LaneWidth lane_width_of() {
  return {LaneCols<NV, H8>::D, 100 + 10 * NV + H8, ln_fwd_lane_kernel<NV, H8>, ln_bwd_lane_kernel<NV, H8>};
}
const LaneWidth LANE_WIDTHS[] = {lane_width_of<0, 1>(), lane_width_of<1, 0>(), lane_width_of<1, 1>(), lane_width_of<2, 0>()};
const LaneWidth* lane_width(int d) {
  for (const LaneWidth& w : LANE_WIDTHS) if (w.d == d) return &w;
  return nullptr;
}

int check_common(const char* who, const mmf_ln_problem* p, int n, int d) {
  if (!p || n <= 0 || n > MMF_LN_MAX_PROBLEMS) MMF_FAIL(MMF_E_SHAPE, "%s: num_problems=%d out of range", who, n);
  if (d <= 0 || (d & 7) || d > MAX_CH * 512) MMF_FAIL(MMF_E_SHAPE, "%s: d=%d must be a multiple of 8, <= 2048", who, d);
  return MMF_OK;
}

int full_blocks(int rows) { return (rows + ROWS_PER_BLOCK - 1) / ROWS_PER_BLOCK; }

int share_blocks(LnArgs& a, const mmf_ln_problem* problems, int num_problems, int budget) {
  long long total_rows = 0;
  for (int i = 0; i < num_problems; ++i) total_rows += problems[i].rows;
  int total = 0;
  for (int i = 0; i < num_problems; ++i) {
    const int rows = problems[i].rows, full = full_blocks(rows);
    const int nb = (int)(((long long)rows * budget + total_rows - 1) / total_rows);
    a.blk_start[i] = total;
    total += nb > full ? full : (nb < 1 ? 1 : nb);
  }
  a.blk_start[num_problems] = total;
  return total;
}

}

extern "C" int mmf_layernorm_last_form(void) { return t_last_form; }

extern "C" int mmf_layernorm_fwd_grouped(const mmf_ln_problem* problems, int num_problems, int d,
                                         float eps, void* stream) {
  if (int rc = check_common("mmf_layernorm_fwd_grouped", problems, num_problems, d)) return rc;
  LnArgs a; a.nprob = num_problems; a.d = d; a.eps = eps; a.ws = nullptr;
  int total = 0;
  long long total_rows = 0;
  for (int i = 0; i < num_problems; ++i) {
    const mmf_ln_problem& p = problems[i];
    if (p.rows <= 0 || !p.x || !p.y || !p.gamma || !p.beta || !p.mean || !p.rstd)
      MMF_FAIL(MMF_E_SHAPE, "mmf_layernorm_fwd_grouped[%d]: null operand or rows=%d", i, p.rows);
    if (!mmf_aligned16(p.x) || !mmf_aligned16(p.y) || !mmf_aligned16(p.gamma) || !mmf_aligned16(p.beta))
      MMF_FAIL(MMF_E_ALIGN, "mmf_layernorm_fwd_grouped[%d]: pointers must be 16-byte aligned", i);
    a.blk_start[i] = total;
    total += full_blocks(p.rows);
    total_rows += p.rows;
    a.p[i] = p;
  }
  a.blk_start[num_problems] = total;
  hipStream_t s = static_cast<hipStream_t>(stream);
  const int budget = total_rows > FWD_LARGE_ROWS ? FWD_BLOCKS_LARGE : FWD_BLOCKS;
  const LaneWidth* lw = lane_width(d);
  if (lw && total > budget) {
    total = share_blocks(a, problems, num_problems, budget);
    hipLaunchKernelGGL(lw->fwd, dim3(total), dim3(256), 0, s, a);
    t_last_form = lw->form;
    MMF_CHECK_LAUNCH("mmf_layernorm_fwd_grouped(lane)");
    return MMF_OK;
  }
  const int nch = (d + 511) / 512;
  hipLaunchKernelGGL(CHUNK_FWD[nch - 1], dim3(total), dim3(256), 0, s, a);
  t_last_form = nch;
  MMF_CHECK_LAUNCH("mmf_layernorm_fwd_grouped");
  return MMF_OK;
}

extern "C" size_t mmf_layernorm_bwd_workspace_bytes(int d) {
  return (size_t)(BWD_BLOCKS_CHUNK + MMF_LN_MAX_PROBLEMS) * 2 * (size_t)(d > 0 ? d : 0) * sizeof(float);
}

extern "C" int mmf_layernorm_bwd_grouped(const mmf_ln_problem* problems, int num_problems, int d,
                                         void* workspace, size_t workspace_bytes, void* stream) {
  if (int rc = check_common("mmf_layernorm_bwd_grouped", problems, num_problems, d)) return rc;
  if (!workspace || workspace_bytes < mmf_layernorm_bwd_workspace_bytes(d) || !mmf_aligned16(workspace))
    MMF_FAIL(MMF_E_SHAPE, "mmf_layernorm_bwd_grouped: workspace of %zu bytes (16-byte aligned) required",
             mmf_layernorm_bwd_workspace_bytes(d));
  LnArgs a; a.nprob = num_problems; a.d = d; a.eps = 0.f; a.ws = static_cast<float*>(workspace);
  for (int i = 0; i < num_problems; ++i) {
    const mmf_ln_problem& p = problems[i];
    if (p.rows <= 0 || !p.x || !p.dy || !p.dx || !p.gamma || !p.mean || !p.rstd || !p.dgamma || !p.dbeta)
      MMF_FAIL(MMF_E_SHAPE, "mmf_layernorm_bwd_grouped[%d]: null operand or rows=%d", i, p.rows);
    if (!mmf_aligned16(p.x) || !mmf_aligned16(p.dy) || !mmf_aligned16(p.dx) || !mmf_aligned16(p.gamma))
      MMF_FAIL(MMF_E_ALIGN, "mmf_layernorm_bwd_grouped[%d]: pointers must be 16-byte aligned", i);
    a.p[i] = p;
  }
  const LaneWidth* lw = lane_width(d);
  const int total = share_blocks(a, problems, num_problems, lw ? BWD_BLOCKS_LANE : BWD_BLOCKS_CHUNK);
  hipStream_t s = static_cast<hipStream_t>(stream);
  const int nch = (d + 511) / 512;
  hipLaunchKernelGGL(lw ? lw->bwd : CHUNK_BWD[nch - 1], dim3(total), dim3(256), 0, s, a);
  t_last_form = lw ? lw->form : nch;
  MMF_CHECK_LAUNCH(lw ? "mmf_layernorm_bwd_grouped(lane)" : "mmf_layernorm_bwd_grouped");
  hipLaunchKernelGGL(ln_bwd_finalize_kernel, dim3((d + 255) / 256, num_problems, FIN_SLICES), dim3(256), 0, s, a);
  MMF_CHECK_LAUNCH("mmf_layernorm_bwd_grouped(finalize)");
  return MMF_OK;
}
```

### simple-multimodal_amd/mmfusion/lib.py

```python
from __future__ import annotations

import ctypes as C
import os
from typing import List, Optional, Sequence

_HERE = os.path.dirname(os.path.abspath(__file__))
LIB_PATH = os.environ.get("MMF_LIB_PATH") or os.path.join(_HERE, "libmmfusion.so")

GEMM_NT, GEMM_NN, GEMM_TN = 0, 1, 2
EPI_BIAS, EPI_RELU, EPI_MASK_AUX, EPI_ADD_AUX, EPI_ACCUM, EPI_COLSUM_A, EPI_DROPOUT = 1, 2, 4, 8, 16, 32, 64
GEMM_MAX_PROBLEMS, ATTN_MAX_PROBLEMS, LN_MAX_PROBLEMS, COLSUM_MAX_PROBLEMS = 48, 12, 8, 24
EVAL_MAX_HEADS, EVAL_NSUMS = 4, 4

SYMBOLS = (
    "mmf_version", "mmf_last_error", "mmf_device_cu_count", "mmf_gemm_grouped", "mmf_gemm_grouped_ex", "mmf_gemm_select_impl", "mmf_gemm_last_impl", "mmf_gemm_set_persistent_workgroups",
    "mmf_gemm7_set_tile_n", "mmf_gemm7_last_tile_n", "mmf_gemm7_tile_n",
    "mmf_attn_fwd_grouped_ex", "mmf_attn_bwd_grouped_ex", "mmf_dropout", "mmf_attn_select_impl",
    "mmf_attn_fwd_grouped", "mmf_attn_bwd_grouped", "mmf_layernorm_fwd_grouped",
    "mmf_layernorm_bwd_grouped", "mmf_layernorm_bwd_workspace_bytes", "mmf_layernorm_last_form", "mmf_cast_f32_to_bf16", "mmf_cast_bf16_to_f32", "mmf_cast_bf16_to_f32_scaled", "mmf_cast_f32_to_bf16_2d", "mmf_add3_bf16", "mmf_add3_grouped", "mmf_addn_bf16", "mmf_addn_grouped",
    "mmf_meanpool_fwd", "mmf_meanpool_bwd", "mmf_meanpool_cat_fwd", "mmf_meanpool_cat_bwd", "mmf_colsum_bf16", "mmf_colsum_grouped", "mmf_relu_bwd_bf16", "mmf_relu_bwd_mixed",
    "mmf_sqnorm_f32", "mmf_adamw_step", "mmf_adamw_advance", "mmf_skinny_linear_fwd", "mmf_skinny_linear_dgrad", "mmf_skinny_linear_fwd_ex", "mmf_skinny_linear_dgrad_ex", "mmf_skinny_last_strip",
    "mmf_gat3_dense_fwd", "mmf_gat3_dense_bwd", "mmf_infonce_fwd", "mmf_infonce_bwd", "mmf_adaptive_combine_fwd",
    "mmf_adaptive_combine_bwd", "mmf_adaptive_attn_weights", "mmf_linear_narrow_fwd", "mmf_linear_narrow_bwd", "mmf_stack3_embed_fwd",
    "mmf_stack3_embed_bwd", "mmf_rowmask_apply", "mmf_zero_ranges_f32", "mmf_fusion_loss", "mmf_modality_dropout",
    "mmf_attn_weights_mean", "mmf_gemm_f32_grouped", "mmf_gemm_f32_batched", "mmf_softmax_rows_f32", "mmf_softmax_bwd_rows_f32",
    "mmf_layernorm_f32_fwd", "mmf_layernorm_f32_bwd", "mmf_bilstm_workspace_bytes", "mmf_bilstm_layer_fwd", "mmf_bilstm_layer_bwd", "mmf_swap01",
    "mmf_distill_kl", "mmf_fusion_loss_kd", "mmf_robust_head_fwd", "mmf_robust_head_bwd",
    "mmf_fewshot_proto_fwd", "mmf_fewshot_proto_bwd", "mmf_fewshot_dist_fwd", "mmf_fewshot_dist_bwd",
    "mmf_eval_accumulate",
    "mmf_vit_patchify", "mmf_vit_embed_tokens", "mmf_bias_gelu_bf16",
    "mmf_w2v_conv0_stats", "mmf_w2v_conv0_norm_gelu", "mmf_w2v_gelu_window", "mmf_w2v_posconv",
    "mmf_deberta_embed", "mmf_deberta_attn_fwd",
    "mmf_video_prepare", "mmf_video_prepare_patches", "mmf_audio_resample", "mmf_audio_augment",
)


class GemmProblem(C.Structure):
    _fields_ = [("A", C.c_void_p), ("B", C.c_void_p), ("C", C.c_void_p), ("bias", C.c_void_p),
                ("aux", C.c_void_p), ("M", C.c_int32), ("N", C.c_int32), ("K", C.c_int32),
                ("lda", C.c_int32), ("ldb", C.c_int32), ("ldc", C.c_int32), ("ldaux", C.c_int32)]


class AttnProblem(C.Structure):
    _fields_ = [("Q", C.c_void_p), ("K", C.c_void_p), ("V", C.c_void_p), ("O", C.c_void_p),
                ("LSE", C.c_void_p), ("dO", C.c_void_p), ("delta", C.c_void_p), ("dQ", C.c_void_p),
                ("dK", C.c_void_p), ("dV", C.c_void_p), ("B", C.c_int32), ("H", C.c_int32),
                ("Tq", C.c_int32), ("Tk", C.c_int32), ("ldq", C.c_int32), ("ldk", C.c_int32),
                ("ldv", C.c_int32), ("ldo", C.c_int32)]


class LnProblem(C.Structure):
    _fields_ = [("x", C.c_void_p), ("y", C.c_void_p), ("gamma", C.c_void_p), ("beta", C.c_void_p),
                ("mean", C.c_void_p), ("rstd", C.c_void_p), ("dy", C.c_void_p), ("dx", C.c_void_p),
                ("dgamma", C.c_void_p), ("dbeta", C.c_void_p), ("rows", C.c_int32)]


class GemmExtra(C.Structure):
    _fields_ = [("alpha", C.c_float), ("dropout_p", C.c_float), ("rng_state", C.c_void_p), ("site", C.c_uint32)]


class SkinnyProblem(C.Structure):
    _fields_ = [("X", C.c_void_p), ("W", C.c_void_p), ("Y", C.c_void_p), ("bias", C.c_void_p), ("aux", C.c_void_p),
                ("M", C.c_int32), ("N", C.c_int32), ("K", C.c_int32), ("ldx", C.c_int32), ("ldw", C.c_int32),
                ("ldy", C.c_int32), ("ldaux", C.c_int32)]


class SkinnyProblemEx(C.Structure):
    _fields_ = [("p", SkinnyProblem), ("Y2", C.c_void_p), ("gate", C.c_void_p), ("dz", C.c_void_p),
                ("ldy2", C.c_int32), ("ldgate", C.c_int32), ("lddz", C.c_int32), ("reserved", C.c_int32)]


class SkinnyExtra(C.Structure):
    _fields_ = [("x_f32", C.c_int32), ("gate_f32", C.c_int32), ("gate_scale", C.c_float), ("dropout_p", C.c_float),
                ("rng_state", C.c_void_p), ("site", C.c_uint32), ("reserved", C.c_uint32)]


SKINNY_MAX_M, SKINNY_MAX_PROBLEMS = 64, 24
ADD3_MAX = 8
ADDN_MAX = 8
ADDN_GROUP_MAX = 4


class AddNProblem(C.Structure):
    _fields_ = [("x", C.c_void_p * 8), ("y", C.c_void_p), ("numel", C.c_int64), ("n", C.c_int32)]


class Add3Problem(C.Structure):
    _fields_ = [("a", C.c_void_p), ("b", C.c_void_p), ("c", C.c_void_p), ("y", C.c_void_p), ("n", C.c_int64)]

ZERO_MAX_RANGES = 48
POOL_MAX = 4


class Gat3Params(C.Structure):
    _fields_ = [("B", C.c_int32), ("heads", C.c_int32), ("C", C.c_int32), ("relu", C.c_int32),
                ("negative_slope", C.c_float), ("dropout_p", C.c_float), ("rng_state", C.c_void_p), ("site", C.c_uint32)]


class BiLstmArgs(C.Structure):
    _fields_ = [("gx", C.c_void_p), ("w_hh", C.c_void_p * 2), ("b_ih", C.c_void_p * 2), ("b_hh", C.c_void_p * 2),
                ("y", C.c_void_p), ("gates", C.c_void_p), ("cell", C.c_void_p), ("dy", C.c_void_p), ("dgates", C.c_void_p),
                ("T", C.c_int32), ("B", C.c_int32), ("H", C.c_int32)]


class ColsumProblem(C.Structure):
    _fields_ = [("x", C.c_void_p), ("out", C.c_void_p), ("M", C.c_int32), ("N", C.c_int32), ("ldx", C.c_int32)]


_lib: Optional[C.CDLL] = None


def load() -> C.CDLL:
    global _lib
    if _lib is not None:
        return _lib
    if not os.path.exists(LIB_PATH):
        raise RuntimeError(
            f"{LIB_PATH} is missing: the MI355X fusion path has no fallback. Build it with "
            f"`python -c 'import __graft_entry__ as g; g.build()'` or `make -C simple-multimodal_amd/csrc`.")
    import torch
    lib = C.CDLL(LIB_PATH)
    lib.mmf_last_error.restype = C.c_char_p
    lib.mmf_version.restype = C.c_int
    vp, i32, i64, f32 = C.c_void_p, C.c_int, C.c_int64, C.c_float
    lib.mmf_gemm_grouped.argtypes = [C.POINTER(GemmProblem), i32, i32, i32, i32, vp]
    lib.mmf_gemm_grouped_ex.argtypes = [C.POINTER(GemmProblem), i32, i32, i32, i32, C.POINTER(GemmExtra), vp]
    lib.mmf_gemm7_tile_n.argtypes = [C.POINTER(GemmProblem), i32, i32]
    lib.mmf_attn_fwd_grouped_ex.argtypes = [C.POINTER(AttnProblem), i32, i32, f32, f32, vp, C.c_uint32, vp]
    lib.mmf_attn_bwd_grouped_ex.argtypes = [C.POINTER(AttnProblem), i32, i32, f32, f32, vp, C.c_uint32, vp]
    lib.mmf_dropout.argtypes = [vp, vp, i64, i32, f32, vp, C.c_uint32, vp]
    lib.mmf_attn_fwd_grouped.argtypes = [C.POINTER(AttnProblem), i32, i32, f32, vp]
    lib.mmf_attn_select_impl.argtypes = [i32]
    lib.mmf_attn_bwd_grouped.argtypes = [C.POINTER(AttnProblem), i32, i32, f32, vp]
    lib.mmf_layernorm_fwd_grouped.argtypes = [C.POINTER(LnProblem), i32, i32, f32, vp]
    lib.mmf_layernorm_bwd_grouped.argtypes = [C.POINTER(LnProblem), i32, i32, vp, C.c_size_t, vp]
    lib.mmf_layernorm_bwd_workspace_bytes.argtypes = [i32]
    lib.mmf_layernorm_bwd_workspace_bytes.restype = C.c_size_t
    lib.mmf_cast_f32_to_bf16.argtypes = [vp, vp, i64, vp]
    lib.mmf_cast_bf16_to_f32.argtypes = [vp, vp, i64, vp]
    lib.mmf_cast_bf16_to_f32_scaled.argtypes = [vp, vp, i64, f32, vp]
    lib.mmf_cast_f32_to_bf16_2d.argtypes = [vp, vp, i32, i32, i32, vp]
    lib.mmf_add3_bf16.argtypes = [vp, vp, vp, vp, i64, vp]
    lib.mmf_add3_grouped.argtypes = [C.POINTER(Add3Problem), i32, vp]
    lib.mmf_addn_bf16.argtypes = [C.POINTER(C.c_void_p), i32, vp, i64, i32, vp]
    lib.mmf_addn_grouped.argtypes = [C.POINTER(AddNProblem), i32, vp]
    lib.mmf_meanpool_fwd.argtypes = [vp, vp, i32, i32, i32, i32, vp]
    lib.mmf_meanpool_bwd.argtypes = [vp, vp, i32, i32, i32, i32, vp]
    lib.mmf_meanpool_cat_fwd.argtypes = [C.POINTER(C.c_void_p), C.POINTER(C.c_int), i32, vp, i32, i32, i32, vp]
    lib.mmf_meanpool_cat_bwd.argtypes = [vp, C.POINTER(C.c_void_p), C.POINTER(C.c_int), i32, i32, i32, i32, vp]
    lib.mmf_colsum_bf16.argtypes = [vp, vp, i32, i32, i32, vp]
    lib.mmf_colsum_grouped.argtypes = [C.POINTER(ColsumProblem), i32, vp]
    lib.mmf_relu_bwd_bf16.argtypes = [vp, vp, vp, i64, vp]
    lib.mmf_relu_bwd_mixed.argtypes = [vp, C.c_int, vp, C.c_int, vp, i64, vp]
    lib.mmf_skinny_linear_fwd.argtypes = [C.POINTER(SkinnyProblem), i32, i32, i32, vp]
    lib.mmf_skinny_linear_dgrad.argtypes = [C.POINTER(SkinnyProblem), i32, i32, f32, i32, vp]
    lib.mmf_fusion_loss.argtypes = [vp, i32, vp, i32, i32, f32, C.POINTER(vp), C.POINTER(f32), i32, vp, vp, vp]
    lib.mmf_modality_dropout.argtypes = [C.POINTER(vp), C.POINTER(vp), vp, i32, i32, f32, vp, C.c_uint32, i32, vp]
    lib.mmf_distill_kl.argtypes = [vp, i32, vp, i32, i32, i32, f32, vp, vp, vp]
    lib.mmf_fusion_loss_kd.argtypes = [vp, i32, vp, i32, i32, f32, C.POINTER(vp), C.POINTER(f32), i32, vp, i32, f32, f32, vp, vp, vp]
    pp = C.POINTER(vp)
    lib.mmf_robust_head_fwd.argtypes = [pp, vp, vp, vp, pp, pp, i32, vp, pp, vp, vp, i32, i32, i32, vp]
    lib.mmf_robust_head_bwd.argtypes = [pp, vp, vp, pp, vp, pp, vp, i32, vp, pp, vp, vp, pp, vp, vp, vp, pp, pp,
                                        i32, i32, i32, vp]
    lib.mmf_fewshot_proto_fwd.argtypes = [pp, vp, vp, i32, i32, i32, vp]
    lib.mmf_fewshot_proto_bwd.argtypes = [vp, vp, vp, i32, i32, i32, vp]
    lib.mmf_fewshot_dist_fwd.argtypes = [pp, vp, vp, vp, vp, i32, i32, i32, vp]
    lib.mmf_fewshot_dist_bwd.argtypes = [vp, vp, vp, vp, vp, vp, vp, vp, i32, i32, i32, vp]
    lib.mmf_eval_accumulate.argtypes = [pp, C.POINTER(C.c_int), i32, vp, i32, i32, f32, vp, vp, vp, vp, vp, i64, i64, vp]
    lib.mmf_skinny_linear_fwd_ex.argtypes = [C.POINTER(SkinnyProblemEx), i32, i32, i32, C.POINTER(SkinnyExtra), vp]
    lib.mmf_skinny_linear_dgrad_ex.argtypes = [C.POINTER(SkinnyProblemEx), i32, i32, f32, i32, C.POINTER(SkinnyExtra), vp]
    lib.mmf_sqnorm_f32.argtypes = [vp, i64, vp, vp]
    P3 = C.c_void_p * 3
    lib.mmf_gat3_dense_fwd.argtypes = [vp] * 8 + [C.POINTER(Gat3Params), vp]
    lib.mmf_gat3_dense_bwd.argtypes = [vp] * 12 + [C.POINTER(Gat3Params), vp]
    lib.mmf_infonce_fwd.argtypes = [P3, P3, vp, vp, vp, i32, i32, f32, vp]
    lib.mmf_infonce_bwd.argtypes = [P3, vp, vp, P3, P3, P3, i32, i32, f32, vp]
    lib.mmf_adaptive_combine_fwd.argtypes = [vp] * 6 + [i32, i32, vp]
    lib.mmf_adaptive_combine_bwd.argtypes = [vp] * 10 + [i32, i32, vp]
    lib.mmf_adaptive_attn_weights.argtypes = [vp, vp, i32, i32, i32, vp]
    lib.mmf_attn_weights_mean.argtypes = [vp, vp, i32, i32, i32, i32, vp]
    lib.mmf_linear_narrow_fwd.argtypes = [vp, vp, vp, vp, i32, i32, i32, vp]
    lib.mmf_linear_narrow_bwd.argtypes = [vp, vp, vp, vp, vp, vp, i32, i32, i32, vp]
    lib.mmf_stack3_embed_fwd.argtypes = [vp, vp, vp, vp, vp, i32, i32, i32, vp]
    lib.mmf_stack3_embed_bwd.argtypes = [vp, vp, vp, vp, vp, i32, i32, i32, vp]
    lib.mmf_rowmask_apply.argtypes = [vp, vp, vp, i32, i32, vp]
    lib.mmf_zero_ranges_f32.argtypes = [vp, C.POINTER(C.c_int64), C.POINTER(C.c_int64), i32, vp]
    lib.mmf_adamw_step.argtypes = [vp, vp, vp, vp, vp, i64, vp, vp, vp]
    lib.mmf_adamw_advance.argtypes = [vp, vp, vp, vp]
    lib.mmf_bilstm_workspace_bytes.restype = C.c_size_t
    lib.mmf_bilstm_layer_fwd.argtypes = [C.POINTER(BiLstmArgs), vp, C.c_size_t, vp]
    lib.mmf_bilstm_layer_bwd.argtypes = [C.POINTER(BiLstmArgs), vp, C.c_size_t, vp]
    lib.mmf_swap01.argtypes = [vp, vp, i32, i32, i32, i32, i32, vp]
    lib.mmf_vit_patchify.argtypes = [vp, vp, i32, i32, i32, i32, i32, vp]
    lib.mmf_vit_embed_tokens.argtypes = [vp, vp, vp, vp, i32, i32, i32, vp]
    lib.mmf_bias_gelu_bf16.argtypes = [vp, vp, i64, i32, i32, vp]
    lib.mmf_w2v_conv0_stats.argtypes = [vp, vp, vp, vp, i32, i32, i32, i32, i32, vp]
    lib.mmf_w2v_conv0_norm_gelu.argtypes = [vp, vp, vp, vp, vp, vp, i32, i32, i32, i32, i32, i32, i32, f32, vp]
    lib.mmf_w2v_gelu_window.argtypes = [vp, vp, i32, i32, i32, i32, i32, vp]
    lib.mmf_w2v_posconv.argtypes = [vp, vp, vp, vp, i32, i32, i32, i32, i32, vp]
    lib.mmf_deberta_embed.argtypes = [vp, vp, vp, vp, vp, f32, vp, i32, vp, i64, i32, i32, vp]
    lib.mmf_deberta_attn_fwd.argtypes = [vp, vp, vp, i32, vp, vp, i32, vp, i32, i32, i32, i32, i32, f32, vp]
    lib.mmf_video_prepare.argtypes = [vp, vp, vp, vp, vp, i32, i32, i32, i32, i32, i32, vp]
    lib.mmf_video_prepare_patches.argtypes = [vp, vp, vp, vp, vp, i32, i32, i32, i32, i32, i32, i32, vp]
    lib.mmf_audio_resample.argtypes = [vp, vp, vp, i64, vp, i32, i32, i64, i64, i32, i32, i32, vp]
    lib.mmf_audio_augment.argtypes = [vp, vp, vp, vp, vp, C.c_uint32, i32, i64, vp]
    S2 = C.c_int64 * 2
    lib.mmf_gemm_f32_grouped.argtypes = [C.POINTER(GemmProblem), i32, i32, i32, f32, vp]
    lib.mmf_gemm_f32_batched.argtypes = [C.POINTER(GemmProblem), i32, i32, f32, i32, i32, S2, S2, S2, vp]
    lib.mmf_softmax_rows_f32.argtypes = [vp, i64, i32, f32, vp]
    lib.mmf_softmax_bwd_rows_f32.argtypes = [vp, vp, i64, i32, f32, vp]
    lib.mmf_layernorm_f32_fwd.argtypes = [vp, vp, vp, vp, vp, vp, i32, i32, f32, vp]
    lib.mmf_layernorm_f32_bwd.argtypes = [vp, vp, vp, vp, vp, vp, vp, vp, i32, i32, vp]
    for name in SYMBOLS:
        getattr(lib, name)
    if lib.mmf_version() != 1:
        raise RuntimeError(f"libmmfusion ABI version {lib.mmf_version()} != 1")
    _lib = lib
    if os.environ.get("MMF_GEMM_IMPL"):
        check(lib.mmf_gemm_select_impl(int(os.environ["MMF_GEMM_IMPL"])))
    return lib


def check(rc: int) -> None:
    if rc != 0:
        raise RuntimeError(f"libmmfusion error {rc}: {load().mmf_last_error().decode()}")


def stream_ptr() -> int:
    import torch
    return torch.cuda.current_stream().cuda_stream


PROFILE: Optional[list] = None
_LAYOUT_NAME = {GEMM_NT: "NT", GEMM_NN: "NN", GEMM_TN: "TN"}


class _Timed:
    def __init__(self, label: str, flops: float, detail=None):
        self.label, self.flops, self.detail = label, flops, detail

    def __enter__(self):
        if PROFILE is not None:
            import torch
            self.e0, self.e1 = torch.cuda.Event(enable_timing=True), torch.cuda.Event(enable_timing=True)
            self.e0.record(torch.cuda.current_stream())
        return self

    def __exit__(self, *exc):
        if PROFILE is not None:
            import torch
            self.e1.record(torch.cuda.current_stream())
            PROFILE.append((self.label, self.flops, self.e0, self.e1, self.detail))


def gemm_grouped(problems: Sequence[GemmProblem], layout: int, epilogue: int, out_f32: bool,
                 alpha: float = 1.0, dropout_p: float = 0.0, rng_state_ptr: Optional[int] = None, site: int = 0) -> None:
    arr = (GemmProblem * len(problems))(*problems)
    flops = sum(2.0 * p.M * p.N * p.K for p in problems) if PROFILE is not None else 0.0
    detail = [(p.M, p.N, p.K) for p in problems] if PROFILE is not None else None
    with _Timed(f"gemm_grouped_kernel<{_LAYOUT_NAME[layout]},{'f32' if out_f32 else 'bf16'}>", flops, detail) as tm:
        if alpha == 1.0 and not (epilogue & EPI_DROPOUT):
            check(load().mmf_gemm_grouped(arr, len(problems), layout, epilogue, int(out_f32), stream_ptr()))
        else:
            ex = GemmExtra(alpha, dropout_p, rng_state_ptr, site)
            check(load().mmf_gemm_grouped_ex(arr, len(problems), layout, epilogue, int(out_f32), C.byref(ex), stream_ptr()))
        if PROFILE is not None:
            tm.label = f"gemm{load().mmf_gemm_last_impl()}_grouped_kernel<{_LAYOUT_NAME[layout]},{'f32' if out_f32 else 'bf16'}>"


def attn_fwd_grouped(problems: Sequence[AttnProblem], head_dim: int, scale: float, dropout_p: float = 0.0,
                     rng_state_ptr: Optional[int] = None, site: int = 0) -> None:
    arr = (AttnProblem * len(problems))(*problems)
    flops = sum(4.0 * p.B * p.H * p.Tq * p.Tk * head_dim for p in problems) if PROFILE is not None else 0.0
    with _Timed(f"attn_fwd_kernel<{head_dim}>", flops, [(p.Tq, p.Tk) for p in problems] if PROFILE is not None else None):
        check(load().mmf_attn_fwd_grouped_ex(arr, len(problems), head_dim, scale, dropout_p, rng_state_ptr, site,
                                             stream_ptr()))


def attn_bwd_grouped(problems: Sequence[AttnProblem], head_dim: int, scale: float, dropout_p: float = 0.0,
                     rng_state_ptr: Optional[int] = None, site: int = 0) -> None:
    arr = (AttnProblem * len(problems))(*problems)
    flops = sum(8.0 * p.B * p.H * p.Tq * p.Tk * head_dim for p in problems) if PROFILE is not None else 0.0
    with _Timed(f"attn_bwd_kernels<{head_dim}>", flops, [(p.Tq, p.Tk) for p in problems] if PROFILE is not None else None):
        check(load().mmf_attn_bwd_grouped_ex(arr, len(problems), head_dim, scale, dropout_p, rng_state_ptr, site,
                                             stream_ptr()))


def layernorm_fwd_grouped(problems: Sequence[LnProblem], d: int, eps: float) -> None:
    arr = (LnProblem * len(problems))(*problems)
    check(load().mmf_layernorm_fwd_grouped(arr, len(problems), d, eps, stream_ptr()))


def layernorm_bwd_grouped(problems: Sequence[LnProblem], d: int, workspace) -> None:
    arr = (LnProblem * len(problems))(*problems)
    check(load().mmf_layernorm_bwd_grouped(arr, len(problems), d, workspace.data_ptr(),
                                           workspace.numel() * workspace.element_size(), stream_ptr()))


def colsum_grouped(problems: Sequence[ColsumProblem]) -> None:
    for i in range(0, len(problems), COLSUM_MAX_PROBLEMS):
        chunk = problems[i:i + COLSUM_MAX_PROBLEMS]
        arr = (ColsumProblem * len(chunk))(*chunk)
        check(load().mmf_colsum_grouped(arr, len(chunk), stream_ptr()))


def skinny_fwd(problems: Sequence[SkinnyProblem], flags: int, out_f32: bool) -> None:
    for i in range(0, len(problems), SKINNY_MAX_PROBLEMS):
        chunk = problems[i:i + SKINNY_MAX_PROBLEMS]
        arr = (SkinnyProblem * len(chunk))(*chunk)
        check(load().mmf_skinny_linear_fwd(arr, len(chunk), flags, int(out_f32), stream_ptr()))


def skinny_fwd_ex(problems: Sequence[SkinnyProblemEx], flags: int, out_f32: bool, extra: SkinnyExtra) -> None:
    if len(problems) > SKINNY_MAX_PROBLEMS:
        raise ValueError("a fused row-linear group must fit one launch")
    arr = (SkinnyProblemEx * len(problems))(*problems)
    check(load().mmf_skinny_linear_fwd_ex(arr, len(problems), flags, int(out_f32), C.byref(extra), stream_ptr()))


def skinny_dgrad_ex(problems: Sequence[SkinnyProblemEx], flags: int, alpha: float, out_f32: bool, extra: SkinnyExtra) -> None:
    if len(problems) > SKINNY_MAX_PROBLEMS:
        raise ValueError("a fused row-linear group must fit one launch")
    arr = (SkinnyProblemEx * len(problems))(*problems)
    check(load().mmf_skinny_linear_dgrad_ex(arr, len(problems), flags, alpha, int(out_f32), C.byref(extra), stream_ptr()))


def skinny_dgrad(problems: Sequence[SkinnyProblem], flags: int, alpha: float, out_f32: bool) -> None:
    for i in range(0, len(problems), SKINNY_MAX_PROBLEMS):
        chunk = problems[i:i + SKINNY_MAX_PROBLEMS]
        arr = (SkinnyProblem * len(chunk))(*chunk)
        check(load().mmf_skinny_linear_dgrad(arr, len(chunk), flags, alpha, int(out_f32), stream_ptr()))


def vit_patchify(pixels, patches, N: int, C: int, H: int, W: int, P: int) -> None:
    if pixels.numel() != N * C * H * W or not pixels.is_contiguous() or not patches.is_contiguous() \
            or patches.numel() != pixels.numel():
        raise ValueError("vit_patchify: pixels / patches do not hold N x C x H x W contiguous elements")
    with _Timed("vit_patchify_kernel", 0.0, [(N, C * H * W)]):
        check(load().mmf_vit_patchify(pixels.data_ptr(), patches.data_ptr(), N, C, H, W, P, stream_ptr()))


def vit_embed_tokens(patch_emb, cls, pos, tokens, N: int, T: int, d: int) -> None:
    if patch_emb.numel() != N * (T - 1) * d or not patch_emb.is_contiguous() or cls.numel() != d or pos.numel() != T * d \
            or tokens.numel() < N * T * d or not tokens.is_contiguous():
        raise ValueError("vit_embed_tokens: operand sizes do not match N, T, d")
    with _Timed("vit_embed_tokens_kernel", 0.0, [(N * T, d)]):
        check(load().mmf_vit_embed_tokens(patch_emb.data_ptr(), cls.data_ptr(), pos.data_ptr(), tokens.data_ptr(), N, T, d,
                                          stream_ptr()))


def bias_gelu(x, bias=None) -> None:
    if x.dim() != 2 or x.stride(1) != 1 or (bias is not None and (bias.numel() != x.shape[1] or not bias.is_contiguous())):
        raise ValueError("bias_gelu: x must be 2-D with contiguous rows and bias one value per column")
    with _Timed("bias_gelu_kernel", 0.0, [tuple(x.shape)]):
        check(load().mmf_bias_gelu_bf16(x.data_ptr(), bias.data_ptr() if bias is not None else None, x.shape[0], x.shape[1],
                                        x.stride(0), stream_ptr()))


W2V_STATS_SLOTS = 128


def _w2v_f32(*ts) -> None:
    import torch
    for t in ts:
        if not t.is_cuda:
            raise RuntimeError("w2v kernels run on the GPU only (no CPU fallback)")
        if t.dtype != torch.float32 or not t.is_contiguous():
            raise ValueError("w2v: the f32 operands must be contiguous float32 tensors")


def _w2v_bf16(*ts) -> None:
    import torch
    for t in ts:
        if not t.is_cuda:
            raise RuntimeError("w2v kernels run on the GPU only (no CPU fallback)")
        if t.dtype != torch.bfloat16:
            raise TypeError(f"w2v: expected a bfloat16 operand, got {t.dtype}")


def w2v_conv0_stats(wave, weight, stats, partial, k0: int, s0: int) -> None:
    _w2v_f32(wave, weight, stats, partial)
    N, L = wave.shape
    C0 = weight.shape[0]
    if weight.numel() != C0 * k0 or stats.numel() < N * 2 * C0 or partial.numel() < N * W2V_STATS_SLOTS * 2 * C0:
        raise ValueError("w2v_conv0_stats: operand sizes do not match N, C0, k0")
    with _Timed("w2v_conv0_stats_kernels", 2.0 * N * ((L - k0) // s0 + 1) * C0 * k0, [(N, L)]):
        check(load().mmf_w2v_conv0_stats(wave.data_ptr(), weight.data_ptr(), stats.data_ptr(), partial.data_ptr(), N, L, C0, k0, s0,
                                         stream_ptr()))


def w2v_conv0_norm_gelu(wave, weight, stats, gamma, beta, out, k0: int, s0: int, k1: int, s1: int, eps: float) -> None:
    _w2v_f32(wave, weight, stats, gamma, beta)
    _w2v_bf16(out)
    N, L = wave.shape
    C0 = weight.shape[0]
    T1 = (((L - k0) // s0 + 1) - k1) // s1 + 1
    if weight.numel() != C0 * k0 or stats.numel() < N * 2 * C0 or gamma.numel() != C0 or beta.numel() != C0 \
            or T1 < 1 or out.numel() < N * T1 * k1 * C0 or not out.is_contiguous():
        raise ValueError("w2v_conv0_norm_gelu: operand sizes do not match N, L, C0 and the two kernels")
    with _Timed("w2v_conv0_norm_gelu_kernel", 2.0 * N * ((L - k0) // s0 + 1) * C0 * k0, [(N, L)]):
        check(load().mmf_w2v_conv0_norm_gelu(wave.data_ptr(), weight.data_ptr(), stats.data_ptr(), gamma.data_ptr(), beta.data_ptr(),
                                             out.data_ptr(), N, L, C0, k0, s0, k1, s1, eps, stream_ptr()))


def w2v_gelu_window(x, out, N: int, T_in: int, C: int, k: int, s: int) -> None:
    _w2v_bf16(x, out)
    T_out = (T_in - k) // s + 1
    if x.numel() < N * T_in * C or not x.is_contiguous() or T_out < 1 or out.numel() < N * T_out * k * C or not out.is_contiguous():
        raise ValueError("w2v_gelu_window: operand sizes do not match N, T_in, C, k, s")
    with _Timed("w2v_gelu_window_kernel", 0.0, [(N * T_out, k * C)]):
        check(load().mmf_w2v_gelu_window(x.data_ptr(), out.data_ptr(), N, T_in, C, k, s, stream_ptr()))


def w2v_posconv(x, w, bias, y, N: int, T: int, C: int, groups: int, k: int) -> None:
    _w2v_bf16(x, w, y)
    _w2v_f32(bias)
    cg = C // max(groups, 1)
    Kp = (k * cg + 31) // 32 * 32
    if x.numel() < N * T * C or y.numel() < N * T * C or w.numel() != C * Kp or bias.numel() != C or not (
            x.is_contiguous() and y.is_contiguous() and w.is_contiguous() and bias.is_contiguous()):
        raise ValueError("w2v_posconv: operand sizes do not match N, T, C, groups, k")
    with _Timed("w2v_posconv_kernel", 2.0 * N * T * C * cg * k, [(N * T, C, k * cg)]):
        check(load().mmf_w2v_posconv(x.data_ptr(), w.data_ptr(), bias.data_ptr(), y.data_ptr(), N, T, C, groups, k, stream_ptr()))


def _deberta_mask(mask, numel: int):
    import torch
    if mask is None:
        return None, 0
    if not mask.is_cuda:
        raise RuntimeError("deberta kernels run on the GPU only (no CPU fallback)")
    if mask.dtype not in (torch.float32, torch.uint8, torch.bool) or not mask.is_contiguous() or mask.numel() != numel:
        raise ValueError("deberta: the mask must be a contiguous float32 / uint8 / bool tensor with one value per token")
    return mask.data_ptr(), 1 if mask.dtype == torch.float32 else 2


def deberta_embed(out, table, gamma, beta, eps: float, ids=None, embeds=None, mask=None) -> None:
    import torch
    _w2v_bf16(out)
    _w2v_f32(gamma, beta)
    if (ids is None) == (embeds is None):
        raise ValueError("deberta_embed: exactly one of ids / embeds")
    rows, d = out.shape
# ... 101 lines not shown
```

### simple-multimodal_amd/mmfusion/ops.py

```python
from __future__ import annotations

import ctypes as C
import math
import os
from dataclasses import dataclass
from itertools import accumulate
from typing import List, Optional, Sequence, Tuple

import torch

from . import lib
from .lib import (AttnProblem, GemmProblem, LnProblem, EPI_ACCUM, EPI_ADD_AUX, EPI_BIAS, EPI_COLSUM_A,
                  EPI_DROPOUT, EPI_MASK_AUX, EPI_RELU, GEMM_NN, GEMM_NT, GEMM_TN)

BF16 = torch.bfloat16

_PRECISION = "bf16"


def set_precision(mode: str) -> str:
    global _PRECISION
    if mode not in ("bf16", "fp32"):
        raise ValueError(f"precision must be 'bf16' or 'fp32', got {mode!r}")
    old, _PRECISION = _PRECISION, mode
    return old


def fp32_mode() -> bool:
    return _PRECISION == "fp32"


def _f32():
    from . import ops_f32
    return ops_f32


@dataclass
class W:
    p: torch.nn.Parameter
    r0: int = 0
    r1: Optional[int] = None

    def rows(self) -> Tuple[int, int]:
        return self.r0, (self.p.shape[0] if self.r1 is None else self.r1)

    @property
    def w16(self) -> torch.Tensor:
        return shadow(self.p)[self.rows()[0]:self.rows()[1]]

    @property
    def grad(self) -> torch.Tensor:
        g = self.p.grad
        if g is None or g.dtype != torch.float32 or not g.is_contiguous():
            raise RuntimeError("parameter has no fp32 arena gradient: call mmfusion.arena.ensure(module)")
        a, b = self.rows()
        return g[a:b]

    @property
    def master(self) -> torch.Tensor:
        a, b = self.rows()
        return self.p.detach()[a:b]


def shadow(p: torch.nn.Parameter) -> torch.Tensor:
    s = getattr(p, "_mmf_bf16", None)
    if s is None:
        raise RuntimeError("parameter is not arena-managed: call mmfusion.arena.ensure(module) first")
    if _PRECISION == "fp32":
        return p.detach()
    if p._mmf_late:
        p._mmf_arena.join()
    return s


def _ld(t: torch.Tensor) -> int:
    if t.dim() != 2 or t.stride(1) != 1:
        raise ValueError(f"expected a 2-D row-major (possibly row-strided) tensor, got {tuple(t.shape)} strides {t.stride()}")
    return t.stride(0)


def _req(t: torch.Tensor, dtype) -> None:
    if not t.is_cuda:
        raise RuntimeError("mmfusion ops run on the GPU only (no CPU fallback)")
    if t.dtype != dtype:
        raise TypeError(f"expected {dtype}, got {t.dtype}")


def _ptr(t: Optional[torch.Tensor]) -> Optional[int]:
    return None if t is None else t.data_ptr()


def _column_views(t: Optional[torch.Tensor], widths: Sequence[int]) -> list:
    offs = [0, *accumulate(widths)]
    return [None if t is None else t[:, a:b] for a, b in zip(offs, offs[1:])]


def _column_blocks(ts: Sequence[torch.Tensor]) -> Optional[torch.Tensor]:
    base = ts[0]._base if len(ts) else None
    if base is None or base.dim() != 2 or not base.is_contiguous():
        return None
    rows, width = base.shape
    off = 0
    for t in ts:
        if (t._base is not base or t.dtype != base.dtype or t.dim() != 2 or t.shape[0] != rows
                or t.stride() != (width, 1) or t.data_ptr() != base.data_ptr() + base.element_size() * off):
            return None
        off += t.shape[1]
    return base if off == width else None


def cast_to_bf16(x: torch.Tensor) -> torch.Tensor:
    _req(x, torch.float32)
    if (x.dim() == 2 and not x.is_contiguous() and x.stride(1) == 1 and x.shape[1] % 4 == 0 and x.stride(0) % 4 == 0
            and x.data_ptr() % 16 == 0):
        y = torch.empty(x.shape, dtype=BF16, device=x.device)
        lib.check(lib.load().mmf_cast_f32_to_bf16_2d(x.data_ptr(), y.data_ptr(), x.shape[0], x.shape[1], x.stride(0),
                                                     lib.stream_ptr()))
        return y
    x = x.contiguous()
    y = torch.empty(x.shape, dtype=BF16, device=x.device)
    lib.check(lib.load().mmf_cast_f32_to_bf16(x.data_ptr(), y.data_ptr(), x.numel(), lib.stream_ptr()))
    return y


def cast_to_f32(x: torch.Tensor) -> torch.Tensor:
    _req(x, BF16)
    x = x.contiguous()
    y = torch.empty(x.shape, dtype=torch.float32, device=x.device)
    lib.check(lib.load().mmf_cast_bf16_to_f32(x.data_ptr(), y.data_ptr(), x.numel(), lib.stream_ptr()))
    return y


def _grad_bf16(g: Optional[torch.Tensor]) -> Optional[torch.Tensor]:
    if g is None:
        return None
    return g.contiguous() if g.dtype == BF16 else cast_to_bf16(g)


def _gemm_problems(layout: int, probs: Sequence[tuple], epilogue: int, dtype, c_dtype) -> List[GemmProblem]:
    ps: List[GemmProblem] = []
    for (A, Bm, Cm, bias, aux) in probs:
        _req(A, dtype), _req(Bm, dtype)
        M, N = Cm.shape
        K = A.shape[0] if layout == GEMM_TN else A.shape[1]
        a_shape, b_shape = (K, M) if layout == GEMM_TN else (M, K), (N, K) if layout == GEMM_NT else (K, N)
        if A.shape != a_shape or Bm.shape != b_shape or Cm.dtype != c_dtype:
            raise ValueError(f"gemm layout {layout}: A{tuple(A.shape)} B{tuple(Bm.shape)} C{tuple(Cm.shape)} {Cm.dtype}")
        if aux is not None and tuple(aux.shape) != (M, N):
            raise ValueError("aux must match C")
        if bias is not None:
            _req(bias, torch.float32)
            if bias.numel() != (M if epilogue & EPI_COLSUM_A else N) or not bias.is_contiguous():
                raise ValueError("bias must be contiguous [N] ([M] for the fused bias gradient)")
        ps.append(GemmProblem(A.data_ptr(), Bm.data_ptr(), Cm.data_ptr(), _ptr(bias), _ptr(aux), M, N, K,
                              _ld(A), _ld(Bm), _ld(Cm), _ld(aux) if aux is not None else 0))
    return ps


def gemm(layout: int, A: torch.Tensor, Bm: torch.Tensor, C: torch.Tensor, *, bias=None, aux=None,
         epilogue: int = 0) -> None:
    gemm_group(layout, [(A, Bm, C, bias, aux)], epilogue)


def gemm_group(layout: int, probs: Sequence[tuple], epilogue: int, alpha: float = 1.0,
               dropout: Optional[tuple] = None) -> None:
    out_f32 = probs[0][2].dtype == torch.float32
    ps = _gemm_problems(layout, probs, epilogue, BF16, torch.float32 if out_f32 else BF16)
    if dropout is not None:
        if len(ps) > lib.GEMM_MAX_PROBLEMS:
            raise ValueError("a dropout GEMM group must fit one launch (the problem index keys the mask)")
        lib.gemm_grouped(ps, layout, epilogue | EPI_DROPOUT, out_f32, alpha, dropout[0],
                         rng_state().data_ptr(), dropout[1])
        return
    for i in range(0, len(ps), lib.GEMM_MAX_PROBLEMS):
        lib.gemm_grouped(ps[i:i + lib.GEMM_MAX_PROBLEMS], layout, epilogue, out_f32, alpha)


_rng_state: Optional[torch.Tensor] = None
_site = 0


def rng_state() -> torch.Tensor:
    global _rng_state
    if _rng_state is None:
        _rng_state = torch.full((1,), (torch.initial_seed() & 0x7FFFFFFF) << 20, dtype=torch.int64, device="cuda")
    return _rng_state


def seed_dropout(seed: int) -> None:
    rng_state().fill_((seed & 0x7FFFFFFF) << 20)


def begin_training_forward() -> None:
    global _site
    _site = 0
    rng_state().add_(1)


def next_site() -> int:
    global _site
    _site += 1
    return _site


class dropout_state:

    def __init__(self, state: torch.Tensor):
        self.state = state

    def __enter__(self):
        global _rng_state, _site
        self.saved = (rng_state(), _site)
        _rng_state, _site = self.state, 0
        return self.state

    def __exit__(self, *exc):
        global _rng_state, _site
        _rng_state, _site = self.saved


class _Dropout(torch.autograd.Function):
    @staticmethod
    def forward(ctx, x, p, site):
        x = x.contiguous()
        y = torch.empty_like(x)
        lib.check(lib.load().mmf_dropout(x.data_ptr(), y.data_ptr(), x.numel(), int(x.dtype == torch.float32), p,
                                         rng_state().data_ptr(), site, lib.stream_ptr()))
        ctx.p, ctx.site = p, site
        return y

    @staticmethod
    def backward(ctx, g):
        g = g.contiguous()
        dx = torch.empty_like(g)
        lib.check(lib.load().mmf_dropout(g.data_ptr(), dx.data_ptr(), g.numel(), int(g.dtype == torch.float32), ctx.p,
                                         rng_state().data_ptr(), ctx.site, lib.stream_ptr()))
        return dx, None, None


def dropout(x: torch.Tensor, p: float, training: bool) -> torch.Tensor:
    if not training or p <= 0.0:
        return x
    if _PRECISION == "fp32":
        raise RuntimeError("the fp32 parity mode runs without dropout (use p = 0 or eval())")
    if x.dtype not in (BF16, torch.float32):
        raise TypeError("dropout expects bf16 or fp32")
    return _Dropout.apply(x, float(p), next_site())


_WGRAD_EARLY = os.environ.get("MMF_WGRAD_EARLY", "0") == "1"
_pending_wgrad: List[tuple] = []
_wgrad_stream: Optional[torch.cuda.Stream] = None


class _Backward:

    def __init__(self, expected: int = 0):
        self.expected = expected
        self.multi_writer: set = set()
        self.callback_queued = False
        self.early = 0
        self.round_issued = 0
        self.rounds_cut = 0
        self.round_ptrs: List[int] = []


_bw = _Backward()


_branch_streams: List[torch.cuda.Stream] = []


def branch_stream(i: int = 0) -> torch.cuda.Stream:
    while len(_branch_streams) <= i:
        _branch_streams.append(torch.cuda.Stream())
    return _branch_streams[i]


def join_branch_streams() -> None:
    cur = torch.cuda.current_stream()
    for s in _branch_streams:
        cur.wait_stream(s)


def _wgrad_rounds(pend: List[tuple]) -> List[List[tuple]]:
    rounds: List[List[tuple]] = []
    spans: List[Tuple[int, int, int]] = []
    def span(t: torch.Tensor) -> Tuple[int, int]:
        if t.dim() == 2:
            return t.data_ptr(), t.data_ptr() + 4 * ((t.shape[0] - 1) * t.stride(0) + t.shape[1])
        return t.data_ptr(), t.data_ptr() + 4 * t.numel()

    for q in pend:
        mine = [span(q[2])]
        if q[3] is not None:
            mine.append(span(q[3]))
        r = 0
        for a, b in mine:
            for s0, e0, r0 in spans:
                if a < e0 and s0 < b:
                    r = max(r, r0 + 1)
        for a, b in mine:
            spans.append((a, b, r))
        while len(rounds) <= r:
            rounds.append([])
        rounds[r].append(q)
    return rounds


# ... 284 lines not shown
            if g is None:
                continue
            if ctx.x_needs[i]:
                dx = dxs[i] if dxs else torch.empty(xs[i].shape, dtype=torch.float32 if ctx.f32_in else BF16, device=g.device)
                dgrad.append((g, ws[i], dx, None, None))
                grads[4 * i] = dx
            if s.w.p.requires_grad:
                queue_wgrad(g, xs[i], s.w.grad, s.b.grad if has_bias else None)
            if ctx.has_res:
                grads[4 * i + 1] = g
        if dgrad:
            if all(g.shape[0] <= lib.SKINNY_MAX_M for (g, _, _, _, _) in dgrad):
                lib.skinny_dgrad([_skinny(g, w, dx) for (g, w, dx, _, _) in dgrad], 0, 1.0, ctx.f32_in)
            else:
                gemm_group(GEMM_NN, dgrad, 0)
        return (None, None, None, *grads)


def _rows2d(t: torch.Tensor) -> torch.Tensor:
    if t.dim() != 2:
        raise ValueError(f"expected a 2-D tensor, got {tuple(t.shape)}")
    return t if t.stride(1) == 1 else t.contiguous()


class _RowLinear(torch.autograd.Function):

    @staticmethod
    def forward(ctx, specs: List[LinearSpec], opts, *tensors):
        out_f32, p, dual = opts
        n = len(specs)
        relu, has_bias, _ = _one_epilogue(specs)
        xs = [_rows2d(tensors[3 * i]) for i in range(n)]
        f32_in = xs[0].dtype == torch.float32
        for x in xs:
            if not x.is_cuda:
                raise RuntimeError("mmfusion ops run on the GPU only (no CPU fallback)")
            if x.dtype not in (BF16, torch.float32) or (x.dtype == torch.float32) != f32_in:
                raise TypeError("a row-linear group's inputs must share one dtype (bf16 or f32)")
        site = next_site() if p > 0.0 else 0
        probs, outs, outs2, x16s = [], [], [], []
        for i, s in enumerate(specs):
            x, w16 = xs[i], s.w.w16
            M, K, N = x.shape[0], x.shape[1], w16.shape[0]
            y = torch.empty((M, N), dtype=torch.float32 if out_f32 else BF16, device=x.device)
            y2 = torch.empty((M, N), dtype=BF16 if out_f32 else torch.float32, device=x.device) if dual else None
            x16 = torch.empty((M, K), dtype=BF16, device=x.device) if f32_in else x
            bias = s.b.master if has_bias else None
            probs.append(lib.SkinnyProblemEx(
                _skinny(x, w16, y, bias), _ptr(y2), None, x16.data_ptr() if f32_in else None,
                _ld(y2) if y2 is not None else 0, 0, _ld(x16) if f32_in else 0, 0))
            outs.append(y), outs2.append(y2), x16s.append(x16)
        flags = (EPI_BIAS if has_bias else 0) | (EPI_RELU if relu else 0) | (EPI_DROPOUT if p > 0.0 else 0)
        extra = lib.SkinnyExtra(int(f32_in), 0, 1.0, float(p), rng_state().data_ptr() if p > 0.0 else None, site, 0)
        lib.skinny_fwd_ex(probs, flags, out_f32, extra)
        ctx.specs, ctx.opts, ctx.site, ctx.f32_in = specs, opts, site, f32_in
        ctx.save_for_backward(*x16s, *(outs if relu else []))
        ctx.x_needs = [tensors[3 * i].requires_grad for i in range(n)]
        return tuple(outs) + (tuple(outs2) if dual else ())

    @staticmethod
    def backward(ctx, *gs):
        specs = ctx.specs
        out_f32, p, dual = ctx.opts
        n = len(specs)
        relu, has_bias = specs[0].relu, specs[0].b is not None
        saved = ctx.saved_tensors
        x16s, ys = saved[:n], (saved[n:] if relu else [None] * n)
        grads: List[Optional[torch.Tensor]] = [None] * (3 * n)
        todo = []
        for i in range(n):
            g, g2 = gs[i], (gs[n + i] if dual else None)
            if g is not None and g2 is not None:
                g = g.float() + g2.float()
            elif g is None:
                g = g2
            if g is not None:
                g = _rows2d(g)
                if g.data_ptr() % 16 or g.stride(0) % (4 if g.dtype == torch.float32 else 8):
                    g = g.contiguous()
                todo.append((i, g))
        for want_f32 in (False, True):
            grp = [(i, g) for i, g in todo if (g.dtype == torch.float32) == want_f32]
            if not grp:
                continue
            gated = relu or p > 0.0
            probs, dxs = [], []
            for i, g in grp:
                w16 = specs[i].w.w16
                M, N, K = g.shape[0], w16.shape[0], w16.shape[1]
                if g.dtype not in (BF16, torch.float32):
                    raise TypeError("row-linear backward: bf16 or f32 gradients only")
                dz = torch.empty((M, N), dtype=BF16, device=g.device) if (gated or want_f32) else g
                dx = torch.empty((M, K), dtype=torch.float32 if ctx.f32_in else BF16, device=g.device)
                y = ys[i]
                probs.append(lib.SkinnyProblemEx(
                    _skinny(g, w16, dx), None, _ptr(y), dz.data_ptr() if dz is not g else None,
                    0, _ld(y) if y is not None else 0, _ld(dz) if dz is not g else 0, 0))
                dxs.append(dx)
                if specs[i].w.p.requires_grad:
                    queue_wgrad(dz, x16s[i], specs[i].w.grad, specs[i].b.grad if has_bias else None)
                if ctx.x_needs[i]:
                    grads[3 * i] = dx
            regen = p > 0.0 and not relu
            extra = lib.SkinnyExtra(int(want_f32), int(relu and ys[grp[0][0]].dtype == torch.float32),
                                    1.0 / (1.0 - p) if (relu and p > 0.0) else 1.0, float(p) if regen else 0.0,
                                    rng_state().data_ptr() if regen else None, ctx.site, 0)
            lib.skinny_dgrad_ex(probs, EPI_DROPOUT if regen else 0, 1.0, ctx.f32_in, extra)
        return (None, None, *grads)


def row_linear_ok(items: Sequence[tuple]) -> bool:
    if _PRECISION == "fp32" or len(items) > lib.SKINNY_MAX_PROBLEMS:
        return False
    for x, spec, res in items:
        if res is not None or x.dim() != 2 or x.shape[0] > lib.SKINNY_MAX_M or x.shape[1] % 8 or spec.w.w16.shape[0] % 4:
            return False
        if x.dtype == torch.float32 and (x.stride(1) != 1 or x.stride(0) % 4 or x.data_ptr() % 16):
            return False
        if x.dtype == BF16 and (x.stride(1) != 1 or x.stride(0) % 8 or x.data_ptr() % 16):
            return False
    return True


def linear_group(items: Sequence[tuple], out_f32: bool = False, cat: bool = False, dropout_p: float = 0.0, dual: bool = False):
    if _PRECISION == "fp32":
        ys = _f32().linear_group(items, cat)
        if dropout_p > 0.0:
            raise RuntimeError("the fp32 parity mode runs without dropout (use p = 0 or eval())")
        return [(y, y) for y in ys] if dual else ys
    if not cat and row_linear_ok(items):
        specs, tensors = _flatten_items(items, residual=False)
        outs = _RowLinear.apply(specs, (bool(out_f32), float(dropout_p), bool(dual)), *tensors)
        n = len(specs)
        return [(outs[i], outs[n + i]) for i in range(n)] if dual else list(outs)
    specs, tensors = _flatten_items(items)
    if cat:
        if dropout_p > 0.0 or dual:
            raise ValueError("a concatenated linear group has no dropout / dual form")
        return _GroupedLinear.apply(specs, bool(out_f32), True, *tensors)
    ys = [dropout(y, dropout_p, True) for y in _GroupedLinear.apply(specs, bool(out_f32), False, *tensors)]
    if dual:
        return [(y, (to_bf16(y) if out_f32 else to_f32(y))) for y in ys]
    return ys


def linear(x: torch.Tensor, w: W, b: Optional[W] = None, relu: bool = False,
           residual: Optional[torch.Tensor] = None, out_f32: bool = False, dropout_p: float = 0.0, dual: bool = False):
    return linear_group([(x, LinearSpec(w, b, relu), residual)], out_f32, dropout_p=dropout_p, dual=dual)[0]


class _GroupedFFN(torch.autograd.Function):

    @staticmethod
    def forward(ctx, layers, drop, *tensors):
        n = len(layers)
        xs = [tensors[5 * i] for i in range(n)]
        for x in xs:
            _req(x, BF16)
        hs = [torch.empty((x.shape[0], l1.weight.shape[0]), dtype=BF16, device=x.device) for x, (l1, _) in zip(xs, layers)]
        gemm_group(GEMM_NT, [(x, shadow(l1.weight), h, l1.bias.detach(), None)
                             for x, h, (l1, _) in zip(xs, hs, layers)], EPI_BIAS | EPI_RELU, dropout=drop)
        ctx.keep_scale = 1.0 / (1.0 - drop[0]) if drop is not None else 1.0
        ys = [torch.empty_like(x) for x in xs]
        gemm_group(GEMM_NT, [(h, shadow(l2.weight), y, l2.bias.detach(), x)
                             for x, h, y, (_, l2) in zip(xs, hs, ys, layers)], EPI_BIAS | EPI_ADD_AUX)
        ctx.layers = layers
        ctx.save_for_backward(*xs, *hs)
        return tuple(ys)

    @staticmethod
    def backward(ctx, *gys):
        layers = ctx.layers
        n = len(layers)
        xs, hs = ctx.saved_tensors[:n], ctx.saved_tensors[n:]
        idx = [i for i, g in enumerate(gys) if g is not None]
        dys = {i: gys[i].contiguous() for i in idx}
        dhs = {i: torch.empty_like(hs[i]) for i in idx}
        dxs = {i: torch.empty_like(xs[i]) for i in idx}
        gemm_group(GEMM_NN, [(dys[i], shadow(layers[i][1].weight), dhs[i], None, hs[i]) for i in idx], EPI_MASK_AUX,
                   alpha=ctx.keep_scale)
        gemm_group(GEMM_NN, [(dhs[i], shadow(layers[i][0].weight), dxs[i], None, dys[i]) for i in idx], EPI_ADD_AUX)
        for i in idx:
            for l, dy_, x_ in ((layers[i][1], dys[i], hs[i]), (layers[i][0], dhs[i], xs[i])):
                if l.weight.requires_grad:
                    queue_wgrad(dy_, x_, l.weight.grad, l.bias.grad)
        grads: List[Optional[torch.Tensor]] = [None] * (5 * n)
        for i in idx:
            grads[5 * i] = dxs[i]
        return (None, None, *grads)


def ffn_residual_group(items: Sequence[tuple], dropout_p: float = 0.0) -> List[torch.Tensor]:
    if _PRECISION == "fp32":
        if dropout_p > 0.0:
            raise RuntimeError("the fp32 parity mode runs without dropout (use p = 0 or eval())")
        return _f32().ffn_residual_group(items)
    layers, tensors = [], []
    for x, l1, l2 in items:
        for p in (l1.weight, l1.bias, l2.weight, l2.bias):
            if getattr(p, "_mmf_bf16", None) is None or p.grad is None:
                raise RuntimeError("FFN parameters are not arena-managed: call mmfusion.arena.ensure(module)")
        layers.append((l1, l2))
        tensors += [x, l1.weight, l1.bias, l2.weight, l2.bias]
    drop = (float(dropout_p), next_site()) if dropout_p > 0.0 else None
    return list(_GroupedFFN.apply(layers, drop, *tensors))


class _GroupedLayerNorm(torch.autograd.Function):

    @staticmethod
    def forward(ctx, eps: float, *tensors):
        n = len(tensors) // 3
        d = tensors[0].shape[-1]
        outs, stats, probs, keep = [], [], [], []
        for i in range(n):
            x, g, b = tensors[3 * i:3 * i + 3]
            _req(x, BF16)
            x = x.contiguous()
            keep.append(x)
            rows = x.numel() // d
            y = torch.empty_like(x)
            st = torch.empty((2, rows), dtype=torch.float32, device=x.device)
            probs.append(LnProblem(x.data_ptr(), y.data_ptr(), g.data_ptr(), b.data_ptr(), st[0].data_ptr(),
                                   st[1].data_ptr(), None, None, None, None, rows))
            outs.append(y), stats.append(st)
        for i in range(0, n, lib.LN_MAX_PROBLEMS):
            lib.layernorm_fwd_grouped(probs[i:i + lib.LN_MAX_PROBLEMS], d, eps)
        ctx.n, ctx.d = n, d
        ctx.params = [(tensors[3 * i + 1], tensors[3 * i + 2]) for i in range(n)]
        ctx.save_for_backward(*[tensors[3 * i] for i in range(n)], *stats)
        return tuple(outs)

    @staticmethod
    def backward(ctx, *gys):
        n, d = ctx.n, ctx.d
        xs, stats = ctx.saved_tensors[:n], ctx.saved_tensors[n:]
        grads: List[Optional[torch.Tensor]] = [None] * (3 * n)
        probs, keep = [], []
        for i, g in enumerate(gys):
            if g is None:
                continue
            g = g.contiguous()
            x = xs[i].contiguous()
            keep += [g, x]
            gamma, beta = ctx.params[i]
            if gamma.grad is None or beta.grad is None:
                raise RuntimeError("LayerNorm parameters have no arena gradient")
            dx = torch.empty_like(x)
            rows = x.numel() // d
            probs.append(LnProblem(x.data_ptr(), None, gamma.data_ptr(), None, stats[i][0].data_ptr(),
                                   stats[i][1].data_ptr(), g.data_ptr(), dx.data_ptr(),
                                   gamma.grad.data_ptr(), beta.grad.data_ptr(), rows))
            grads[3 * i] = dx
        ws_bytes = lib.load().mmf_layernorm_bwd_workspace_bytes(d)
        for i in range(0, len(probs), lib.LN_MAX_PROBLEMS):
            ws = torch.empty(ws_bytes // 4, dtype=torch.float32, device=xs[0].device)
            keep.append(ws)
            lib.layernorm_bwd_grouped(probs[i:i + lib.LN_MAX_PROBLEMS], d, ws)
        return (None, *grads)


def layernorm_group(items: Sequence[tuple], eps: float = 1e-5) -> List[torch.Tensor]:
    if _PRECISION == "fp32":
        return _f32().layernorm_group(items, eps)
    flat = []
    for x, g, b in items:
        flat += [x, g, b]
    return list(_GroupedLayerNorm.apply(eps, *flat))


@dataclass
class AttnSpec:
    B: int
    Tq: int
    Tk: int
    q: Tuple[int, int]
    k: Tuple[int, int]
    v: Tuple[int, int]


class _GroupedAttention(torch.autograd.Function):
    @staticmethod
    def forward(ctx, specs: List[AttnSpec], H: int, dh: int, drop, *srcs):
        scale = 1.0 / math.sqrt(dh)
        d = H * dh
        outs, lses, probs = [], [], []
        for s in specs:
            for (si, col), T in ((s.q, s.Tq), (s.k, s.Tk), (s.v, s.Tk)):
                t = srcs[si]
                _req(t, BF16)
                if t.dim() != 2 or not t.is_contiguous() or t.shape[0] != s.B * T or col + d > t.shape[1]:
                    raise ValueError(f"attention source {si}: shape {tuple(t.shape)} does not hold B*T={s.B * T} rows x {d} columns at {col}")
            dev = srcs[0].device
            o = torch.empty((s.B * s.Tq, d), dtype=BF16, device=dev)
            lse = torch.empty((s.B * H * s.Tq,), dtype=torch.float32, device=dev)
            qs, ks, vs = srcs[s.q[0]], srcs[s.k[0]], srcs[s.v[0]]
            probs.append(AttnProblem(qs.data_ptr() + 2 * s.q[1], ks.data_ptr() + 2 * s.k[1], vs.data_ptr() + 2 * s.v[1],
                                     o.data_ptr(), lse.data_ptr(), None, None, None, None, None,
                                     s.B, H, s.Tq, s.Tk, qs.shape[1], ks.shape[1], vs.shape[1], d))
            outs.append(o), lses.append(lse)
        if drop is not None and len(probs) > lib.ATTN_MAX_PROBLEMS:
            raise ValueError("an attention group with dropout must fit one launch (the problem index keys the mask)")
        dp_, st_, site_ = (drop[0], rng_state().data_ptr(), drop[1]) if drop is not None else (0.0, None, 0)
        for i in range(0, len(probs), lib.ATTN_MAX_PROBLEMS):
            lib.attn_fwd_grouped(probs[i:i + lib.ATTN_MAX_PROBLEMS], dh, scale, dp_, st_, site_)
        ctx.specs, ctx.H, ctx.dh, ctx.nsrc, ctx.drop = specs, H, dh, len(srcs), drop
        ctx.save_for_backward(*srcs, *outs, *lses)
        return tuple(outs)

    @staticmethod
    def backward(ctx, *gos):
        specs, H, dh, ns = ctx.specs, ctx.H, ctx.dh, ctx.nsrc
        n = len(specs)
        d = H * dh
        srcs = ctx.saved_tensors[:ns]
        outs = ctx.saved_tensors[ns:ns + n]
        lses = ctx.saved_tensors[ns + n:]
        covered = [set() for _ in range(ns)]
        for s, g in zip(specs, gos):
            if g is None:
                continue
            for si, col in (s.q, s.k, s.v):
                covered[si].add(col)
        gsrc: List[Optional[torch.Tensor]] = []
        for si, t in enumerate(srcs):
            if not covered[si]:
                gsrc.append(None)
                continue
            full = len(covered[si]) * d == t.shape[1]
            gsrc.append(torch.empty_like(t) if full else torch.zeros_like(t))
        probs, keep = [], []
        for i, (s, g) in enumerate(zip(specs, gos)):
            if g is None:
                continue
            g = g.contiguous()
            delta = torch.empty_like(lses[i])
            keep += [g, delta]
            qs, ks, vs = srcs[s.q[0]], srcs[s.k[0]], srcs[s.v[0]]
            probs.append(AttnProblem(qs.data_ptr() + 2 * s.q[1], ks.data_ptr() + 2 * s.k[1], vs.data_ptr() + 2 * s.v[1],
                                     outs[i].data_ptr(), lses[i].data_ptr(), g.data_ptr(), delta.data_ptr(),
                                     gsrc[s.q[0]].data_ptr() + 2 * s.q[1], gsrc[s.k[0]].data_ptr() + 2 * s.k[1],
                                     gsrc[s.v[0]].data_ptr() + 2 * s.v[1],
                                     s.B, H, s.Tq, s.Tk, qs.shape[1], ks.shape[1], vs.shape[1], d))
        drop = ctx.drop
        if drop is not None and len(probs) != len(specs):
            raise RuntimeError("attention dropout backward needs the gradient of every problem of the group")
        dp_, st_, site_ = (drop[0], rng_state().data_ptr(), drop[1]) if drop is not None else (0.0, None, 0)
        for i in range(0, len(probs), lib.ATTN_MAX_PROBLEMS):
            lib.attn_bwd_grouped(probs[i:i + lib.ATTN_MAX_PROBLEMS], dh, 1.0 / math.sqrt(dh), dp_, st_, site_)
        return (None, None, None, None, *gsrc)


def attention_group(specs: List[AttnSpec], H: int, dh: int, srcs: Sequence[torch.Tensor],
                    dropout_p: float = 0.0) -> List[torch.Tensor]:
    if _PRECISION == "fp32":
        if dropout_p > 0.0:
            raise RuntimeError("the fp32 parity mode runs without dropout (use p = 0 or eval())")
        return _f32().attention_group(specs, H, dh, srcs)
    drop = (float(dropout_p), next_site()) if dropout_p > 0.0 else None
    return list(_GroupedAttention.apply(specs, H, dh, drop, *srcs))


class _Add3(torch.autograd.Function):
    @staticmethod
    def forward(ctx, a, b, c):
        _req(a, BF16)
        a, b = a.contiguous(), b.contiguous()
        c = c.contiguous() if c is not None else None
        y = torch.empty_like(a)
        lib.check(lib.load().mmf_add3_bf16(a.data_ptr(), b.data_ptr(), c.data_ptr() if c is not None else None,
                                           y.data_ptr(), a.numel(), lib.stream_ptr()))
        ctx.has_c = c is not None
        return y

    @staticmethod
    def backward(ctx, g):
        return g, g, (g if ctx.has_c else None)


def add3(a, b, c=None):
    if _PRECISION == "fp32":
        return a + b if c is None else a + b + c
    return _Add3.apply(a, b, c)


class _Add3Group(torch.autograd.Function):

    @staticmethod
    def forward(ctx, *tensors):
        n = len(tensors) // 3
        probs, outs, keep = [], [], []
        for i in range(n):
            a, b, c = (t.contiguous() for t in tensors[3 * i:3 * i + 3])
            _req(a, BF16), _req(b, BF16), _req(c, BF16)
            if a.shape != b.shape or a.shape != c.shape:
                raise ValueError("add3 group: operands of one sum must have one shape")
            y = torch.empty_like(a)
            keep += [a, b, c]
            outs.append(y)
            probs.append(lib.Add3Problem(a.data_ptr(), b.data_ptr(), c.data_ptr(), y.data_ptr(), a.numel()))
        arr = (lib.Add3Problem * n)(*probs)
        lib.check(lib.load().mmf_add3_grouped(arr, n, lib.stream_ptr()))
        return tuple(outs)

    @staticmethod
    def backward(ctx, *gs):
        out = []
        for g in gs:
            out += [g, g, g]
        return tuple(out)


def add3_group(triples: Sequence[tuple]) -> List[torch.Tensor]:
    if _PRECISION == "fp32":
        return [a + b + c for a, b, c in triples]
    if not 0 < len(triples) <= lib.ADD3_MAX:
        raise ValueError(f"add3 group of {len(triples)} sums (1..{lib.ADD3_MAX})")
    return list(_Add3Group.apply(*[t for tr in triples for t in tr]))


class _Fanout(torch.autograd.Function):
# ... 122 lines not shown
```

### simple-multimodal_amd/models/fusion_layers.py

```python
from __future__ import annotations

import math
import warnings
from typing import Dict, List, Optional, Sequence, Tuple

import torch
import torch.nn as nn
import torch.nn.functional as F

from mmfusion import arena as _arena
from mmfusion import ops
from mmfusion import small_ops as sops
from mmfusion.ops import AttnSpec, LinearSpec, W

_depth = 0
import os as _os
_BRANCH_STREAM = _os.environ.get("MMF_HIER_STREAMS", "1") != "0"
_between: list = []


def _tick() -> None:
    if _between:
        fn = _between.pop(0)
        if fn is not None:
            fn()
_RECAST = _os.environ.get("MMF_RECAST_EACH_STEP", "0") == "1"
_MULT_STREAMS = int(_os.environ.get("MMF_MULT_STREAMS", "2"))
if _MULT_STREAMS not in (1, 2):
    raise ValueError(f"MMF_MULT_STREAMS must be 1 or 2, got {_MULT_STREAMS}")


class _FusionBase(nn.Module):

    def _precision(self) -> str:
        return (getattr(self, "precision", None) or getattr(getattr(self, "config", None), "fusion_precision", None)
                or _os.environ.get("MMF_PRECISION") or "bf16")

    def _enter(self):
        global _depth
        if _depth == 0:
            _arena.ensure(self, refresh=self.training and _RECAST)
            self._saved_precision = ops.set_precision(self._precision())
            if self.training:
                ops.begin_training_forward()
        _depth += 1

    def _exit(self):
        global _depth
        _depth -= 1
        if _depth == 0:
            ops.set_precision(getattr(self, "_saved_precision", "bf16"))
            _cat3_memo.clear()
            arena = getattr(next(self.parameters(), None), "_mmf_arena", None)
            if arena is not None:
                arena.join()

    def __call__(self, *args, **kwargs):
        self._enter()
        try:
            return super().__call__(*args, **kwargs)
        finally:
            self._exit()


def _p(module: nn.Module, p: float) -> float:
    return float(p) if (module.training and p > 0.0) else 0.0


def _as_rows(x: torch.Tensor) -> torch.Tensor:
    if not x.is_cuda:
        raise RuntimeError("mmfusion fusion layers run on the GPU only (no CPU fallback)")
    return ops.to_bf16(x.contiguous()).reshape(-1, x.shape[-1])


def synth_flat(out) -> List[torch.Tensor]:
    if isinstance(out, torch.Tensor):
        return [out]
    if isinstance(out, dict):
        return [t for v in out.values() for t in synth_flat(v)]
    return []


_cat3_memo: Dict[tuple, Tuple[torch.Tensor, torch.Tensor]] = {}


def _cat3(t: torch.Tensor, a: torch.Tensor, v: torch.Tensor) -> Tuple[torch.Tensor, torch.Tensor]:
    if not t.is_cuda:
        raise RuntimeError("mmfusion fusion layers run on the GPU only (no CPU fallback)")
    key = (t.data_ptr(), a.data_ptr(), v.data_ptr(), t._version, a._version, v._version, tuple(t.shape))
    hit = _cat3_memo.get(key)
    if hit is None:
        c32 = sops.cat3(t, a, v)
        hit = (c32, ops.to_bf16(c32))
        if _depth > 0:
            _cat3_memo[key] = hit
    return hit


def _lin(layer: nn.Linear, relu: bool = False) -> LinearSpec:
    return LinearSpec(W(layer.weight), W(layer.bias) if layer.bias is not None else None, relu)


class _MHAParams(nn.Module):

    def __init__(self, embed_dim: int, num_heads: int):
        super().__init__()
        if embed_dim % num_heads:
            raise ValueError("embed_dim must be divisible by num_heads")
        self.embed_dim, self.num_heads, self.head_dim = embed_dim, num_heads, embed_dim // num_heads
        self.in_proj_weight = nn.Parameter(torch.empty(3 * embed_dim, embed_dim))
        self.in_proj_bias = nn.Parameter(torch.zeros(3 * embed_dim))
        self.out_proj = nn.Linear(embed_dim, embed_dim)
        nn.init.xavier_uniform_(self.in_proj_weight)
        nn.init.zeros_(self.out_proj.bias)

    def q_spec(self) -> LinearSpec:
        d = self.embed_dim
        return LinearSpec(W(self.in_proj_weight, 0, d), W(self.in_proj_bias, 0, d))

    def kv_spec(self) -> LinearSpec:
        d = self.embed_dim
        return LinearSpec(W(self.in_proj_weight, d, 3 * d), W(self.in_proj_bias, d, 3 * d))

    def qkv_spec(self) -> LinearSpec:
        return LinearSpec(W(self.in_proj_weight), W(self.in_proj_bias))


def _cross_blocks(blocks: Sequence["CrossModalTransformer"], qs: Sequence[torch.Tensor],
                  kvs: Sequence[torch.Tensor], B: int, Tqs: Sequence[int], Tks: Sequence[int],
                  p: float = 0.0, ress: Optional[Sequence[torch.Tensor]] = None) -> List[torch.Tensor]:
    proj = _cross_in_proj(blocks, qs, kvs)
    _tick()
    att = _cross_attention(blocks, proj, B, Tqs, Tks, p)
    _tick()
    return _cross_tail(blocks, att, qs if ress is None else ress, p)


def _cross_in_proj(blocks, qs, kvs) -> List[torch.Tensor]:
    items = []
    for blk, q, kv in zip(blocks, qs, kvs):
        items.append((q, blk.attention.q_spec(), None))
        items.append((kv, blk.attention.kv_spec(), None))
    return ops.linear_group(items)


def _cross_attention(blocks, proj, B, Tqs, Tks, p) -> List[torch.Tensor]:
    mp0 = blocks[0].attention
    d, H, dh = mp0.embed_dim, mp0.num_heads, mp0.head_dim
    specs = [AttnSpec(B, Tqs[i], Tks[i], q=(2 * i, 0), k=(2 * i + 1, 0), v=(2 * i + 1, d))
             for i in range(len(blocks))]
    return ops.attention_group(specs, H, dh, proj, dropout_p=p)


def _cross_tail(blocks, att, qs, p) -> List[torch.Tensor]:
    pre1 = ops.linear_group([(att[i], _lin(blk.attention.out_proj), qs[i]) for i, blk in enumerate(blocks)])
    _tick()
    x = ops.layernorm_group([(pre1[i], blk.norm1.weight, blk.norm1.bias) for i, blk in enumerate(blocks)],
                            blocks[0].norm1.eps)
    _tick()
    pre2 = ops.ffn_residual_group([(x[i], blk.ffn[0], blk.ffn[3]) for i, blk in enumerate(blocks)], dropout_p=p)
    _tick()
    return ops.layernorm_group([(pre2[i], blk.norm2.weight, blk.norm2.bias) for i, blk in enumerate(blocks)],
                               blocks[0].norm2.eps)


def _self_attention_core(mhas: Sequence[_MHAParams], xs: Sequence[torch.Tensor], B: int, Ts: Sequence[int],
                         p: float = 0.0) -> List[torch.Tensor]:
    d, H, dh = mhas[0].embed_dim, mhas[0].num_heads, mhas[0].head_dim
    qkv = ops.linear_group([(x, m.qkv_spec(), None) for m, x in zip(mhas, xs)])
    specs = [AttnSpec(B, Ts[i], Ts[i], q=(i, 0), k=(i, d), v=(i, 2 * d)) for i in range(len(mhas))]
    return ops.attention_group(specs, H, dh, qkv, dropout_p=p)


def _self_attention(mhas: Sequence[_MHAParams], xs: Sequence[torch.Tensor], B: int, Ts: Sequence[int],
                    p: float = 0.0) -> List[torch.Tensor]:
    att = _self_attention_core(mhas, xs, B, Ts, p)
    return ops.linear_group([(att[i], _lin(m.out_proj), None) for i, m in enumerate(mhas)])


class EarlyFusion(_FusionBase):
    def __init__(self, config):
        super().__init__()
        self.config = config
        d = config.fusion_hidden_size
        self.fusion_layers = nn.Sequential(
            nn.Linear(3 * d, 2 * d), nn.ReLU(), nn.Dropout(config.fusion_dropout),
            nn.Linear(2 * d, d), nn.ReLU(), nn.Dropout(config.fusion_dropout))

    def forward(self, text_features, audio_features, video_features) -> torch.Tensor:
        p = _p(self, self.config.fusion_dropout)
        _, x = _cat3(text_features, audio_features, video_features)
        h = ops.linear(x, *_wb(self.fusion_layers[0]), relu=True, dropout_p=p)
        return ops.linear(h, *_wb(self.fusion_layers[3]), relu=True, out_f32=True, dropout_p=p)


def _wb(layer: nn.Linear):
    return W(layer.weight), (W(layer.bias) if layer.bias is not None else None)


class LateFusion(_FusionBase):
    def __init__(self, config):
        super().__init__()
        self.config = config
        d, n = config.fusion_hidden_size, config.num_emotions
        self.text_classifier = nn.Linear(d, n)
        self.audio_classifier = nn.Linear(d, n)
        self.video_classifier = nn.Linear(d, n)
        self.fusion_weights = nn.Parameter(torch.ones(3) / 3)

    def forward(self, text_features, audio_features, video_features) -> Dict[str, torch.Tensor]:
        if not text_features.is_cuda:
            raise RuntimeError("mmfusion fusion layers run on the GPU only (no CPU fallback)")
        tl = sops.narrow_linear(text_features, self.text_classifier)
        al = sops.narrow_linear(audio_features, self.audio_classifier)
        vl = sops.narrow_linear(video_features, self.video_classifier)
        w = F.softmax(self.fusion_weights, dim=0)
        return {"fused_logits": w[0] * tl + w[1] * al + w[2] * vl, "text_logits": tl,
                "audio_logits": al, "video_logits": vl, "fusion_weights": w}


class CrossModalTransformer(_FusionBase):
    def __init__(self, config):
        super().__init__()
        d = config.fusion_hidden_size
        self.dropout_p = config.fusion_dropout
        self.attention = _MHAParams(d, config.fusion_num_heads)
        self.norm1 = nn.LayerNorm(d)
        self.norm2 = nn.LayerNorm(d)
        self.ffn = nn.Sequential(nn.Linear(d, 4 * d), nn.ReLU(), nn.Dropout(config.fusion_dropout),
                                 nn.Linear(4 * d, d))

    def forward(self, query: torch.Tensor, key_value: torch.Tensor) -> torch.Tensor:
        B, Tq, d = query.shape
        Tk = key_value.shape[1]
        y = _cross_blocks([self], [_as_rows(query)], [_as_rows(key_value)], B, [Tq], [Tk], _p(self, self.dropout_p))[0]
        return ops.to_f32(y).reshape(B, Tq, d)


class MultimodalTransformer(_FusionBase):
    def __init__(self, config):
        super().__init__()
        self.config = config
        d, H = config.fusion_hidden_size, config.fusion_num_heads
        self.text_to_audio = CrossModalTransformer(config)
        self.text_to_video = CrossModalTransformer(config)
        self.audio_to_text = CrossModalTransformer(config)
        self.audio_to_video = CrossModalTransformer(config)
        self.video_to_text = CrossModalTransformer(config)
        self.video_to_audio = CrossModalTransformer(config)
        self.text_self_attn = _MHAParams(d, H)
        self.audio_self_attn = _MHAParams(d, H)
        self.video_self_attn = _MHAParams(d, H)
        self.final_fusion = nn.Sequential(nn.Linear(3 * d, d), nn.ReLU(), nn.Dropout(config.fusion_dropout))

    def forward(self, text_features, audio_features, video_features) -> Dict[str, torch.Tensor]:
        p = _p(self, self.config.fusion_dropout)
        if text_features.dim() == 2:
            text_features, audio_features, video_features = (
                text_features.unsqueeze(1), audio_features.unsqueeze(1), video_features.unsqueeze(1))
        B, Tt, d = text_features.shape
        Ta, Tv = audio_features.shape[1], video_features.shape[1]
        t, a, v = _as_rows(text_features), _as_rows(audio_features), _as_rows(video_features)
        blocks = [self.text_to_audio, self.text_to_video, self.audio_to_text, self.audio_to_video,
                  self.video_to_text, self.video_to_audio]
        tf, af, vf = ops.fanout_group([t, a, v], 7)
        qs, kvs = [tf[0], tf[1], af[0], af[1], vf[0], vf[1]], [af[2], vf[2], tf[2], vf[3], tf[3], af[3]]
        ress = [tf[4], tf[5], af[4], af[5], vf[4], vf[5]]
        Tqs, Tks = [Tt, Tt, Ta, Ta, Tv, Tv], [Ta, Tv, Tt, Tv, Tt, Ta]
        t, a, v = tf[6], af[6], vf[6]
        mhas = [self.text_self_attn, self.audio_self_attn, self.video_self_attn]
        streams = _MULT_STREAMS > 1 and _depth == 1 and t.is_cuda and not ops.fp32_mode()
        if streams:
            xs3, Ts3 = [t, a, v], [Tt, Ta, Tv]

            def chain(ms):
                g = [2 * m + j for m in ms for j in (0, 1)]
                outs = _cross_blocks([blocks[i] for i in g], [qs[i] for i in g], [kvs[i] for i in g], B,
                                     [Tqs[i] for i in g], [Tks[i] for i in g], p, [ress[i] for i in g])
                es = ops.add3_group([(xs3[m], outs[2 * i], outs[2 * i + 1]) for i, m in enumerate(ms)])
                return _self_attention_core([mhas[m] for m in ms], es, B, [Ts3[m] for m in ms], p)
            main = torch.cuda.current_stream()
            side = ops.branch_stream(1)
            side.wait_stream(main)
            with torch.cuda.stream(side):
                att_side = chain([1, 2])
            att = [*chain([0]), *att_side]
            main.wait_stream(side)
            for x in att_side:
                x.record_stream(main)
        else:
            t_a, t_v, a_t, a_v, v_t, v_a = _cross_blocks(blocks, qs, kvs, B, Tqs, Tks, p, ress)
            et, ea, ev = ops.add3_group([(t, t_a, t_v), (a, a_t, a_v), (v, v_t, v_a)])
            att = _self_attention_core(mhas, [et, ea, ev], B, [Tt, Ta, Tv], p)
        pooled_att = ops.meanpool_cat([att[0].view(B, Tt, d), att[1].view(B, Ta, d), att[2].view(B, Tv, d)])
        pf = ops.linear_group([(x, _lin(m.out_proj), None) for x, m in zip(sops.split3(pooled_att), mhas)],
                              out_f32=True, cat=True)
        fused = ops.linear(pf, *_wb(self.final_fusion[0]), relu=True, out_f32=True, dropout_p=p)
        return {"fused_features": fused, "text_features": pf[:, :d], "audio_features": pf[:, d:2 * d],
                "video_features": pf[:, 2 * d:]}


class _DenseGAT(nn.Module):
    heads = 4

    def __init__(self, in_channels: int, out_channels: int):
        super().__init__()
        self.in_channels, self.out_channels = in_channels, out_channels
        self.lin = nn.Linear(in_channels, self.heads * out_channels, bias=False)
        self.att_src = nn.Parameter(torch.empty(1, self.heads, out_channels))
        self.att_dst = nn.Parameter(torch.empty(1, self.heads, out_channels))
        self.bias = nn.Parameter(torch.zeros(out_channels))
        nn.init.xavier_uniform_(self.lin.weight)
        nn.init.xavier_uniform_(self.att_src)
        nn.init.xavier_uniform_(self.att_dst)

    def _load_from_state_dict(self, state_dict, prefix, *args, **kwargs):
        for old in ("lin_src.weight", "lin_dst.weight"):
            if prefix + old in state_dict:
                w = state_dict.pop(prefix + old)
                state_dict.setdefault(prefix + "lin.weight", w)
        super()._load_from_state_dict(state_dict, prefix, *args, **kwargs)

    def forward(self, x: torch.Tensor, B: int, p: float = 0.0, pool: bool = False):
        h = ops.linear(x, W(self.lin.weight), None, out_f32=True)
        if ops.fp32_mode():
            return sops.gat3_f32(h, self.att_src, self.att_dst, self.bias, B, self.heads, pool=pool)
        return sops.gat3(h, self.att_src, self.att_dst, self.bias, B, self.heads, relu=True, pool=pool, dropout_p=p)


class GraphFusion(_FusionBase):
    def __init__(self, config):
        super().__init__()
        self.config = config
        d, G, L = config.fusion_hidden_size, config.graph_hidden_size, config.graph_num_layers
        self.gcn_layers = nn.ModuleList([_DenseGAT(d if l == 0 else G, G) for l in range(L)])
        self.node_type_embedding = nn.Embedding(3, d)
        self.output_projection = nn.Linear(G, d)

    def forward(self, text_features, audio_features, video_features) -> torch.Tensor:
        B = text_features.shape[0]
        c32, _ = _cat3(text_features, audio_features, video_features)
        if ops.fp32_mode():
            x = (c32.view(B, 3, -1) + self.node_type_embedding.weight).reshape(B * 3, -1)
        else:
            x = sops.stack3_embed(c32, self.node_type_embedding.weight)
        pg = _p(self, self.config.graph_dropout)
        pooled = None
        for l, layer in enumerate(self.gcn_layers):
            if l + 1 < len(self.gcn_layers):
                x = layer(x, B, pg)
            else:
                x, pooled = layer(x, B, pg, pool=True)
        return ops.linear(pooled, *_wb(self.output_projection), out_f32=True)


class ContrastiveFusion(_FusionBase):
    def __init__(self, config):
        super().__init__()
        self.config = config
        self.temperature = config.contrastive_temperature
        d = config.fusion_hidden_size
        mk = lambda: nn.Sequential(nn.Linear(d, d), nn.ReLU(), nn.Linear(d, d // 2))
        self.text_projector, self.audio_projector, self.video_projector = mk(), mk(), mk()
        self.fusion_layer = nn.Sequential(nn.Linear(3 * d, d), nn.ReLU(), nn.Dropout(config.fusion_dropout))

    def forward(self, text_features, audio_features, video_features,
                compute_contrastive_loss: bool = False) -> Dict[str, torch.Tensor]:
        p = _p(self, self.config.fusion_dropout)
        d = text_features.shape[-1]
        _, cat = _cat3(text_features, audio_features, video_features)
        xs = list(sops.split3(cat))
        projs = [self.text_projector, self.audio_projector, self.video_projector]
        h = ops.linear_group([(x, _lin(p[0], relu=True), None) for x, p in zip(xs, projs)])
        z = ops.linear_group([(hh, _lin(p[2]), None) for hh, p in zip(h, projs)], out_f32=True)
        losses = {}
        if text_features.shape[0] <= sops.NCE_MAX_B:
            (tp, ap, vp), ls = sops.normalize_infonce(z, self.temperature, compute_contrastive_loss)
            if compute_contrastive_loss:
                losses = {"text_audio": ls[0], "text_video": ls[1], "audio_video": ls[2]}
        else:
            tp, ap, vp = (F.normalize(t, dim=-1) for t in z)
            if compute_contrastive_loss:
                losses = {"text_audio": self.contrastive_loss(tp, ap),
                          "text_video": self.contrastive_loss(tp, vp),
                          "audio_video": self.contrastive_loss(ap, vp)}
        fused = ops.linear(cat, *_wb(self.fusion_layer[0]), relu=True, out_f32=True, dropout_p=p)
        return {"fused_features": fused, "text_proj": tp, "audio_proj": ap, "video_proj": vp,
                "contrastive_losses": losses}

    def contrastive_loss(self, z1: torch.Tensor, z2: torch.Tensor) -> torch.Tensor:
        sim = torch.mm(z1, z2.t()) / self.temperature
        labels = torch.arange(z1.size(0), device=z1.device)
        return (F.cross_entropy(sim, labels) + F.cross_entropy(sim.t(), labels)) / 2


class AdaptiveFusion(_FusionBase):
    def __init__(self, config):
        super().__init__()
        self.config = config
        d = config.fusion_hidden_size
        self.attention = _MHAParams(d, config.fusion_num_heads)
        self.text_transform = nn.Linear(d, d)
        self.audio_transform = nn.Linear(d, d)
        self.video_transform = nn.Linear(d, d)
        self.weight_predictor = nn.Sequential(nn.Linear(3 * d, d), nn.ReLU(), nn.Linear(d, 3), nn.Softmax(dim=-1))
        self.fusion_layer = nn.Sequential(nn.Linear(d, d), nn.ReLU(), nn.Dropout(config.fusion_dropout))

    def forward(self, text_features, audio_features, video_features) -> Dict[str, torch.Tensor]:
        p = _p(self, self.config.fusion_dropout)
        B, d = text_features.shape
        mp = self.attention
        H, dh = mp.num_heads, mp.head_dim
        _, cat = _cat3(text_features, audio_features, video_features)
        xs = list(sops.split3(cat))
        stacked = ops.linear_group([(x, _lin(l), None) for x, l in
                                    zip(xs, (self.text_transform, self.audio_transform, self.video_transform))],
                                   cat=True).view(B * 3, d)
        qkv = ops.linear(stacked, mp.qkv_spec().w, mp.qkv_spec().b)
        att = ops.attention_group([AttnSpec(B, 3, 3, q=(0, 0), k=(0, d), v=(0, 2 * d))], H, dh, [qkv], dropout_p=p)[0]
        attended = ops.linear(att, *_wb(mp.out_proj), out_f32=True).view(B, 3, d)
        attn_w = torch.empty((B, 3, 3), dtype=torch.float32, device=qkv.device)
        if H <= 16 and not ops.fp32_mode():
            from mmfusion import lib as _lib
            _lib.check(_lib.load().mmf_adaptive_attn_weights(qkv.data_ptr(), attn_w.data_ptr(), B, H, dh, _lib.stream_ptr()))
        else:
            with torch.no_grad():
                q4 = qkv.detach().float().view(B, 3, 3, H, dh)
                sc = torch.einsum("bihd,bjhd->bhij", q4[:, :, 0], q4[:, :, 1]) / math.sqrt(dh)
                attn_w = F.softmax(sc, dim=-1).mean(dim=1)
        hp = ops.linear(cat, *_wb(self.weight_predictor[0]), relu=True, out_f32=True)
        if ops.fp32_mode():
            aw = F.softmax(F.linear(hp, self.weight_predictor[2].weight, self.weight_predictor[2].bias), dim=-1)
            weighted = (attended * aw.unsqueeze(-1)).sum(dim=1)
        else:
            weighted, aw = sops.adaptive_combine(hp, attended, self.weight_predictor[2].weight, self.weight_predictor[2].bias)
        fused = ops.linear(weighted, *_wb(self.fusion_layer[0]), relu=True, out_f32=True, dropout_p=p)
        return {"fused_features": fused, "attention_weights": attn_w, "adaptive_weights": aw}


class HierarchicalFusion(_FusionBase):

    def __init__(self, config):
        super().__init__()
        self.config = config
        d = config.fusion_hidden_size
# ... 75 lines not shown
```

Measured before the change: 7620.

## Fuse norm2 LayerNorms into add3 and store ReLU masks as bitmasks

Adds a fused kernel that runs two LayerNorms and the three-way residual sum in one pass, replacing a grouped LayerNorm followed by add3 in the cross-modal fusion path. The GEMM7 epilogue can now emit ReLU sign bits as a compact bitmask in the FFN forward and read them back in the backward mask GEMM, so the full bf16 activation no longer has to be reread as the mask. Both are meant to cut memory traffic and kernel launches. The cost is more epilogue template variants and tighter eligibility rules, with fallbacks when generation 7 or the fused LN kernel is not available.

```diff
diff --git a/include/mmfusion.h b/include/mmfusion.h
--- a/include/mmfusion.h
+++ b/include/mmfusion.h
@@ -32,7 +32,9 @@
   MMF_EPI_ADD_AUX = 8,
   MMF_EPI_ACCUM = 16,
   MMF_EPI_COLSUM_A = 32,
-  MMF_EPI_DROPOUT = 64
+  MMF_EPI_DROPOUT = 64,
+  MMF_EPI_RELU_BITS = 128,
+  MMF_EPI_MASK_BITS = 256
 };
 
 typedef struct mmf_gemm_problem {
@@ -55,6 +57,9 @@
 } mmf_gemm_extra;
 int mmf_gemm_grouped_ex(const mmf_gemm_problem* problems, int num_problems, int layout, int epilogue,
                         int out_f32, const mmf_gemm_extra* extra, void* stream);
+size_t mmf_gemm_relu_bits_bytes(int M, int N);
+int mmf_gemm_relu_bits_available(const mmf_gemm_problem* problems, int num_problems, int layout, int epilogue,
+                                 int out_f32, const mmf_gemm_extra* extra);
 
 int mmf_gemm_select_impl(int impl);
 int mmf_gemm_last_impl(void);
@@ -174,6 +179,25 @@
 int mmf_layernorm_bwd_grouped(const mmf_ln_problem* problems, int num_problems, int d,
                               void* workspace, size_t workspace_bytes, void* stream);
 int mmf_layernorm_last_form(void);
+
+#define MMF_LN2_ADD3_MAX_PROBLEMS 4
+typedef struct mmf_ln2_add3_problem {
+  const void* x;
+  const void* pre_a;
+  const float* gamma_a;
+  const float* beta_a;
+  const void* pre_b;
+  const float* gamma_b;
+  const float* beta_b;
+  void* e;
+  float* mean_a;
+  float* rstd_a;
+  float* mean_b;
+  float* rstd_b;
+  int32_t rows;
+} mmf_ln2_add3_problem;
+int mmf_layernorm2_add3_available(const int32_t* rows, int num_problems, int d);
+int mmf_layernorm2_add3_fwd_grouped(const mmf_ln2_add3_problem* problems, int num_problems, int d, float eps, void* stream);
 
 int mmf_cast_f32_to_bf16(const float* src, void* dst, int64_t n, void* stream);
 int mmf_cast_bf16_to_f32(const void* src, float* dst, int64_t n, void* stream);
diff --git a/simple-multimodal_amd/csrc/gemm.hip b/simple-multimodal_amd/csrc/gemm.hip
--- a/simple-multimodal_amd/csrc/gemm.hip
+++ b/simple-multimodal_amd/csrc/gemm.hip
@@ -35,6 +35,34 @@
   return MMF_OK;
 }
 
+static int select_impl(const mmf_gemm_problem* problems, int num_problems, int layout, int epilogue, int out_f32, const mmf_gemm_extra* extra) {
+  int impl = gemm_impl();
+  const bool pinned = impl != 0;
+  if (impl == 0) impl = auto_impl(problems, num_problems, layout);
+  const bool ok6 = mmf_gemm6_supports(problems, num_problems, layout) && mmf_gemm6_supports_epi(epilogue, out_f32);
+  if (impl == 6 && !pinned && mmf_gemm7_supports(problems, num_problems, layout, epilogue, out_f32, extra)) impl = 7;
+  if (impl == 7 && !mmf_gemm7_supports(problems, num_problems, layout, epilogue, out_f32, extra)) impl = 6;
+  if (impl == 6 && !ok6) impl = 2;
+  return impl;
+}
+
+constexpr int EPI_BITS = MMF_EPI_RELU_BITS | MMF_EPI_MASK_BITS;
+static bool bits_flags_ok(int epilogue) {
+  if ((epilogue & EPI_BITS) == EPI_BITS || (epilogue & (MMF_EPI_MASK_AUX | MMF_EPI_ADD_AUX))) return false;
+  return (epilogue & MMF_EPI_RELU_BITS) ? (epilogue & MMF_EPI_RELU) != 0 : true;
+}
+
+extern "C" size_t mmf_gemm_relu_bits_bytes(int M, int N) {
+  if (M <= 0 || N <= 0) return 0;
+  return (size_t)((M + 31) / 32) * (size_t)((N + 31) / 32) * 64 * sizeof(uint16_t);
+}
+
+extern "C" int mmf_gemm_relu_bits_available(const mmf_gemm_problem* problems, int num_problems, int layout, int epilogue,
+                                            int out_f32, const mmf_gemm_extra* extra) {
+  if (!problems || num_problems <= 0 || num_problems > MMF_GEMM_MAX_PROBLEMS || !(epilogue & EPI_BITS) || !bits_flags_ok(epilogue)) return 0;
+  return select_impl(problems, num_problems, layout, epilogue, out_f32, extra) == 7;
+}
+
 extern "C" int mmf_gemm_grouped(const mmf_gemm_problem* problems, int num_problems, int layout,
                                 int epilogue, int out_f32, void* stream) {
   return mmf_gemm_grouped_ex(problems, num_problems, layout, epilogue, out_f32, nullptr, stream);
@@ -53,17 +81,16 @@
     MMF_FAIL(MMF_E_UNSUPPORTED, "mmf_gemm_grouped: MASK_AUX and ADD_AUX are exclusive");
   if ((epilogue & MMF_EPI_COLSUM_A) && (layout != MMF_GEMM_TN || (epilogue & MMF_EPI_BIAS)))
     MMF_FAIL(MMF_E_UNSUPPORTED, "mmf_gemm_grouped: COLSUM_A is a TN (wgrad) epilogue and excludes BIAS");
+  if ((epilogue & EPI_BITS) && !bits_flags_ok(epilogue))
+    MMF_FAIL(MMF_E_UNSUPPORTED, "mmf_gemm_grouped: RELU_BITS needs RELU; RELU_BITS, MASK_BITS, MASK_AUX and ADD_AUX are exclusive (one aux pointer)");
   if (epilogue & MMF_EPI_DROPOUT) {
     if (!extra || !extra->rng_state || !(extra->dropout_p >= 0.f) || extra->dropout_p >= 1.f)
       MMF_FAIL(MMF_E_SHAPE, "mmf_gemm_grouped_ex: MMF_EPI_DROPOUT needs rng_state and 0 <= p < 1");
   }
-  int impl = gemm_impl();
-  const bool pinned = impl != 0;
-  if (impl == 0) impl = auto_impl(problems, num_problems, layout);
-  const bool ok6 = mmf_gemm6_supports(problems, num_problems, layout) && mmf_gemm6_supports_epi(epilogue, out_f32);
-  if (impl == 6 && !pinned && mmf_gemm7_supports(problems, num_problems, layout, epilogue, out_f32, extra)) impl = 7;
-  if (impl == 7 && !mmf_gemm7_supports(problems, num_problems, layout, epilogue, out_f32, extra)) impl = 6;
-  if (impl == 6 && !ok6) impl = 2;
+  const int impl = select_impl(problems, num_problems, layout, epilogue, out_f32, extra);
+  if ((epilogue & EPI_BITS) && impl != 7)
+    MMF_FAIL(MMF_E_UNSUPPORTED, "mmf_gemm_grouped: RELU_BITS / MASK_BITS exist in generation 7 only and this launch goes to generation %d "
+             "(mmf_gemm_relu_bits_available)", impl);
   t_last_impl = impl;
   for (int i = 0; i < num_problems; ++i) {
     const mmf_gemm_problem& p = problems[i];
@@ -71,7 +98,7 @@
       MMF_FAIL(MMF_E_SHAPE, "mmf_gemm_grouped[%d]: empty problem M=%d N=%d K=%d", i, p.M, p.N, p.K);
     if (!p.A || !p.B || !p.C) MMF_FAIL(MMF_E_SHAPE, "mmf_gemm_grouped[%d]: null operand", i);
     if ((epilogue & (MMF_EPI_BIAS | MMF_EPI_COLSUM_A)) && !p.bias) MMF_FAIL(MMF_E_SHAPE, "mmf_gemm_grouped[%d]: bias is null", i);
-    if ((epilogue & (MMF_EPI_MASK_AUX | MMF_EPI_ADD_AUX)) && !p.aux)
+    if ((epilogue & (MMF_EPI_MASK_AUX | MMF_EPI_ADD_AUX | EPI_BITS)) && !p.aux)
       MMF_FAIL(MMF_E_SHAPE, "mmf_gemm_grouped[%d]: aux is null", i);
     const int a_cols = (layout == MMF_GEMM_TN) ? p.M : p.K;
     const int b_cols = (layout == MMF_GEMM_NT) ? p.K : p.N;
diff --git a/simple-multimodal_amd/csrc/gemm7.hip b/simple-multimodal_amd/csrc/gemm7.hip
--- a/simple-multimodal_amd/csrc/gemm7.hip
+++ b/simple-multimodal_amd/csrc/gemm7.hip
@@ -46,14 +46,24 @@
   s.KT = P.K / BK;
 }
 
+__device__ __forceinline__ unsigned bf16x2_not_positive(unsigned w) {
+  typedef unsigned short u16x2_t __attribute__((ext_vector_type(2)));
+  const u16x2_t y = __builtin_bit_cast(u16x2_t, w) - (u16x2_t){1, 1};
+  const u16x2_t z = __builtin_elementwise_add_sat(y, (u16x2_t){0x80, 0x80});
+  return __builtin_bit_cast(unsigned, (u16x2_t)(z >> 15));
+}
+__device__ __forceinline__ constexpr int keep_bit(int g, int e) { return 2 * g + (e >> 1) + 8 * (e & 1); }
+
 template <int CT, int TN>
 __device__ __forceinline__ void drain_tile(const GemmArgs& args, const int pi, const mmf_gemm_problem& P, const int mb, const int nb,
                                            f32x16_t (&acc)[TN][4], char* region, const int lane) {
   constexpr bool AUX = (CT & (MMF_EPI_MASK_AUX | MMF_EPI_ADD_AUX)) != 0;
   constexpr bool DROP = (CT & MMF_EPI_DROPOUT) != 0;
+  constexpr bool EMIT_BITS = (CT & MMF_EPI_RELU_BITS) != 0, MASK_BITS = (CT & MMF_EPI_MASK_BITS) != 0;
+  static_assert(!(AUX && (EMIT_BITS || MASK_BITS)) && !(EMIT_BITS && MASK_BITS), "aux is one of: a bf16 tile, bits written, bits read");
   const unsigned drop_key = DROP ? mmf_rng_key(*args.rng_state, args.site, (unsigned)args.orig[pi]) : 0u;
   const float drop_scale = DROP ? 1.f / (1.f - (float)args.drop_thresh * (1.f / 4294967296.f)) : 1.f;
-  const float alpha = (CT & MMF_EPI_MASK_AUX) ? args.alpha : 1.f;
+  const float alpha = (CT & (MMF_EPI_MASK_AUX | MMF_EPI_MASK_BITS)) ? args.alpha : 1.f;
   const int r = lane & 31, h = lane >> 5, q = lane >> 4, cq = lane & 15;
   const unsigned wr_base = (unsigned)(r * 256 + 8 * h + 16 * (r & 15));
   const unsigned rd_base = (unsigned)(q * 256 + ((cq ^ q) << 4));
@@ -67,6 +77,22 @@
   const unsigned a_off0 = col_ok ? (unsigned)(((long)(mb + q) * P.ldaux + nb + 8 * cq) * 2) : 0x80000000u;
   const unsigned c_row4 = (unsigned)(4 * P.ldc * 2), a_row4 = (unsigned)(4 * P.ldaux * 2);
 
+  const int nb32 = (P.N + 31) >> 5;
+  const __amdgpu_buffer_rsrc_t brs = __builtin_amdgcn_make_buffer_rsrc(const_cast<void*>((EMIT_BITS || MASK_BITS) ? P.aux : P.C), 0,
+      (EMIT_BITS || MASK_BITS) ? ((P.M + 31) >> 5) * nb32 * 128 : 0, 0x00020000);
+  auto bits_off = [&](int tm, int tn) {
+    const int bn = (nb >> 5) + tn;
+    return bn < nb32 ? (unsigned)((((mb >> 5) + tm) * nb32 + bn) * 128 + 2 * lane) : 0x80000000u;
+  };
+  unsigned keep[TN][4];
+  if constexpr (MASK_BITS) {
+#pragma unroll
+    for (int tm = 0; tm < 4; ++tm)
+#pragma unroll
+      for (int tn = 0; tn < TN; ++tn)
+        keep[tn][tm] = (unsigned short)__builtin_amdgcn_raw_buffer_load_b16(brs, bits_off(tm, tn), 0, 0);
+  }
+
   u32x4_t auxr[2][8];
   auto load_aux = [&](int tm, int slot) {
 #pragma unroll
@@ -91,6 +117,7 @@
 #pragma unroll
     for (int tn = 0; tn < TN; ++tn) {
       asm volatile("" : "+a"(acc[tn][tm]));
+      unsigned npos = 0;
 #pragma unroll
       for (int g = 0; g < 4; ++g) {
         f32x4_t v = {acc[tn][tm][4 * g], acc[tn][tm][4 * g + 1], acc[tn][tm][4 * g + 2], acc[tn][tm][4 * g + 3]};
@@ -113,8 +140,21 @@
             v[0] += a0; v[1] += a1; v[2] += a2; v[3] += a3;
           }
         }
-        *reinterpret_cast<u32x2_t*>(acc_at(4 * tn + g)) = u32x2_t{pack_bf16x2(v[0], v[1]), pack_bf16x2(v[2], v[3])};
+        if constexpr (MASK_BITS) {
+#pragma unroll
+          for (int e = 0; e < 4; ++e) {
+            int m;
+            asm("v_bfe_i32 %0, %1, %2, 1" : "=v"(m) : "v"(keep[tn][tm]), "s"(keep_bit(g, e)));
+            v[e] = __uint_as_float(__float_as_uint(v[e] * alpha) & (unsigned)m);
+          }
+        }
+        const u32x2_t w = {pack_bf16x2(v[0], v[1]), pack_bf16x2(v[2], v[3])};
+        if constexpr (EMIT_BITS) {
+          npos |= bf16x2_not_positive(w[0]) << (2 * g) | bf16x2_not_positive(w[1]) << (2 * g + 1);
+        }
+        *reinterpret_cast<u32x2_t*>(acc_at(4 * tn + g)) = w;
       }
+      if constexpr (EMIT_BITS) __builtin_amdgcn_raw_buffer_store_b16((short)~((npos & 0xffu) | (npos >> 8)), brs, bits_off(tm, tn), 0, 0);
       __builtin_amdgcn_sched_barrier(0);
     }
     u32x4_t w[8];
@@ -395,9 +435,15 @@
       if (a) launch7<false, MMF_EPI_BIAS | MMF_EPI_RELU | MMF_EPI_DROPOUT>(*a, total, grid, tile_n, s);
       return true;
     }
+    constexpr int RB = MMF_EPI_RELU | MMF_EPI_RELU_BITS;
+    if (eflags == RB)                                     { if (a) launch7<false, RB>(*a, total, grid, tile_n, s); return true; }
+    if (eflags == (RB | MMF_EPI_BIAS))                    { if (a) launch7<false, RB | MMF_EPI_BIAS>(*a, total, grid, tile_n, s); return true; }
+    if (eflags == (RB | MMF_EPI_DROPOUT))                 { if (a) launch7<false, RB | MMF_EPI_DROPOUT>(*a, total, grid, tile_n, s); return true; }
+    if (eflags == (RB | MMF_EPI_BIAS | MMF_EPI_DROPOUT))  { if (a) launch7<false, RB | MMF_EPI_BIAS | MMF_EPI_DROPOUT>(*a, total, grid, tile_n, s); return true; }
   } else if (layout == MMF_GEMM_NN) {
     if (eflags == 0)                                      { if (a) launch7<true, 0>(*a, total, grid, tile_n, s); return true; }
     if (eflags == MMF_EPI_MASK_AUX)                       { if (a) launch7<true, MMF_EPI_MASK_AUX>(*a, total, grid, tile_n, s); return true; }
+    if (eflags == MMF_EPI_MASK_BITS)                      { if (a) launch7<true, MMF_EPI_MASK_BITS>(*a, total, grid, tile_n, s); return true; }
     if (eflags == MMF_EPI_ADD_AUX)                        { if (a) launch7<true, MMF_EPI_ADD_AUX>(*a, total, grid, tile_n, s); return true; }
   }
   return false;
@@ -481,11 +527,13 @@
 
 bool mmf_gemm7_supports(const mmf_gemm_problem* problems, int num_problems, int layout, int epilogue, int out_f32, const mmf_gemm_extra* extra) {
   if (out_f32 || !launch7_select(layout, epilogue, nullptr, 0, 0, nullptr)) return false;
-  if (extra && extra->alpha != 1.f && !(layout == MMF_GEMM_NN && epilogue == MMF_EPI_MASK_AUX)) return false;
+  if (extra && extra->alpha != 1.f && !(layout == MMF_GEMM_NN && (epilogue == MMF_EPI_MASK_AUX || epilogue == MMF_EPI_MASK_BITS))) return false;
+  const bool bits = (epilogue & (MMF_EPI_RELU_BITS | MMF_EPI_MASK_BITS)) != 0;
   if ((epilogue & MMF_EPI_DROPOUT) && !(extra && extra->rng_state)) return false;
   for (int i = 0; i < num_problems; ++i) {
     const mmf_gemm_problem& p = problems[i];
-    if (p.K % BK || p.K < (NS + 1) * BK || (p.N & 7) || (p.ldc & 7) || (p.aux && ((p.ldaux & 7) || !mmf_aligned16(p.aux)))) return false;
+    if (p.K % BK || p.K < (NS + 1) * BK || (p.N & 7) || (p.ldc & 7) || (p.aux && ((!bits && (p.ldaux & 7)) || !mmf_aligned16(p.aux)))) return false;
+    if (bits && !p.aux) return false;
   }
   return true;
 }
@@ -512,7 +560,8 @@
     const mmf_gemm_problem& p = problems[order[i]];
     const size_t a_bytes = (size_t)p.M * p.lda * 2;
     const size_t b_bytes = (size_t)(layout == MMF_GEMM_NT ? p.N : p.K) * p.ldb * 2;
-    const size_t c_bytes = (size_t)p.M * p.ldc * 2, x_bytes = p.aux ? (size_t)p.M * p.ldaux * 2 : 0;
+    const bool bits = (epilogue & (MMF_EPI_RELU_BITS | MMF_EPI_MASK_BITS)) != 0;
+    const size_t c_bytes = (size_t)p.M * p.ldc * 2, x_bytes = bits ? mmf_gemm_relu_bits_bytes(p.M, p.N) : p.aux ? (size_t)p.M * p.ldaux * 2 : 0;
     if (a_bytes >= 0x7fffffffull || b_bytes >= 0x7fffffffull || c_bytes >= 0x7fffffffull || x_bytes >= 0x7fffffffull)
       MMF_FAIL(MMF_E_UNSUPPORTED, "mmf_gemm_grouped[%d]: operand larger than 2 GiB", i);
     a.tile_start[i] = total;
diff --git a/simple-multimodal_amd/csrc/layernorm.hip b/simple-multimodal_amd/csrc/layernorm.hip
--- a/simple-multimodal_amd/csrc/layernorm.hip
+++ b/simple-multimodal_amd/csrc/layernorm.hip
@@ -131,6 +131,32 @@
     if (H8) *reinterpret_cast<f32x4_t*>(p + 512 * NV + 4 * lane) = f32x4_t{f[8 * NV], f[8 * NV + 1], f[8 * NV + 2], f[8 * NV + 3]};
   }
 };
+
+template <class LC>
+__device__ __forceinline__ void ln_lane_row(const typename LC::Bf16& r, const float (&gam)[LC::EP], const float (&bet)[LC::EP],
+                                            const float inv_d, const float eps, float (&o)[LC::EP], float& mean, float& rstd) {
+#pragma clang fp contract(off)
+  constexpr int EP = LC::EP;
+  float v[EP];
+  LC::unpack(r, v);
+  float s = 0.f;
+#pragma unroll
+  for (int e = 0; e < EP; ++e) s += v[e];
+  mean = wave_sum(s) * inv_d;
+  float q = 0.f;
+#pragma unroll
+  for (int e = 0; e < EP; ++e) {
+    v[e] -= mean;
+    const float sq = v[e] * v[e];
+    q += sq;
+  }
+  rstd = rsqrtf(__builtin_fmaf(wave_sum(q), inv_d, eps));
+#pragma unroll
+  for (int e = 0; e < EP; ++e) {
+    const float xh = v[e] * rstd;
+    o[e] = __builtin_fmaf(gam[e], xh, bet[e]);
+  }
+}
 
 template <int NV, int H8>
 __global__ __launch_bounds__(256)
@@ -153,21 +179,67 @@
   for (; row < P.rows; row += step) {
     const bool more = row + step < P.rows;
     if (more) fetch(row + step, nxt);
-    float v[EP];
-    LC::unpack(cur, v);
-    float s = 0.f;
-#pragma unroll
-    for (int e = 0; e < EP; ++e) s += v[e];
-    const float mean = wave_sum(s) * inv_d;
-    float q = 0.f;
-#pragma unroll
-    for (int e = 0; e < EP; ++e) { v[e] -= mean; q += v[e] * v[e]; }
-    const float rstd = rsqrtf(wave_sum(q) * inv_d + a.eps);
-    float o[EP];
-#pragma unroll
-    for (int e = 0; e < EP; ++e) o[e] = v[e] * rstd * gam[e] + bet[e];
+    float o[EP], mean, rstd;
+    ln_lane_row<LC>(cur, gam, bet, inv_d, a.eps, o, mean, rstd);
     LC::store(static_cast<unsigned short*>(P.y) + (size_t)row * d, lane, o);
     if (lane == 0) { P.mean[row] = mean; P.rstd[row] = rstd; }
+    if (more) cur = nxt;
+  }
+}
+
+struct Ln2Add3Args {
+  int nprob;
+  float eps;
+  int blk_start[MMF_LN2_ADD3_MAX_PROBLEMS + 1];
+  mmf_ln2_add3_problem p[MMF_LN2_ADD3_MAX_PROBLEMS];
+};
+
+template <int NV, int H8>
+__global__ __launch_bounds__(256)
+void ln2_add3_lane_kernel(const Ln2Add3Args a) {
+  using LC = LaneCols<NV, H8>;
+  constexpr int EP = LC::EP, d = LC::D;
+  const int pi = mmf_group_problem(a.blk_start, a.nprob, blockIdx.x);
+  const mmf_ln2_add3_problem& P = a.p[pi];
+  const int lane = threadIdx.x & 63, wave = threadIdx.x >> 6;
+  const int nblk = a.blk_start[pi + 1] - a.blk_start[pi];
+  const float inv_d = 1.f / (float)d;
+  float gam_a[EP], bet_a[EP], gam_b[EP], bet_b[EP];
+  LC::load_f32(P.gamma_a, lane, gam_a);
+  LC::load_f32(P.beta_a, lane, bet_a);
+  LC::load_f32(P.gamma_b, lane, gam_b);
+  LC::load_f32(P.beta_b, lane, bet_b);
+  struct Row { typename LC::Bf16 x, pa, pb; };
+  auto fetch = [&](int row, Row& r) {
+    LC::load(static_cast<const unsigned short*>(P.pre_a) + (size_t)row * d, lane, r.pa);
+    LC::load(static_cast<const unsigned short*>(P.pre_b) + (size_t)row * d, lane, r.pb);
+    LC::load(static_cast<const unsigned short*>(P.x) + (size_t)row * d, lane, r.x);
+  };
+  auto round_bf16 = [](float (&y)[EP]) {
+#pragma unroll
+    for (int e = 0; e < EP; e += 2) {
+      const unsigned w = pack_bf16x2(y[e], y[e + 1]);
+      y[e] = bf16lo(w);
+      y[e + 1] = bf16hi(w);
+    }
+  };
+  const int step = nblk * ROWS_PER_BLOCK;
+  int row = ((int)blockIdx.x - a.blk_start[pi]) * ROWS_PER_BLOCK + wave;
+  Row cur, nxt;
+  if (row < P.rows) fetch(row, cur);
+  for (; row < P.rows; row += step) {
+    const bool more = row + step < P.rows;
+    if (more) fetch(row + step, nxt);
+    float ya[EP], yb[EP], xv[EP], mean_a, rstd_a, mean_b, rstd_b;
+    ln_lane_row<LC>(cur.pa, gam_a, bet_a, inv_d, a.eps, ya, mean_a, rstd_a);
+    ln_lane_row<LC>(cur.pb, gam_b, bet_b, inv_d, a.eps, yb, mean_b, rstd_b);
+    round_bf16(ya);
+    round_bf16(yb);
+    LC::unpack(cur.x, xv);
+#pragma unroll
+    for (int e = 0; e < EP; ++e) xv[e] = xv[e] + ya[e] + yb[e];
+    LC::store(static_cast<unsigned short*>(P.e) + (size_t)row * d, lane, xv);
+    if (lane == 0) { P.mean_a[row] = mean_a; P.rstd_a[row] = rstd_a; P.mean_b[row] = mean_b; P.rstd_b[row] = rstd_b; }
     if (more) cur = nxt;
   }
 }
@@ -366,10 +438,11 @@
 using LnKernel = void (*)(const LnArgs);
 const LnKernel CHUNK_FWD[MAX_CH] = {ln_fwd_kernel<1>, ln_fwd_kernel<2>, ln_fwd_kernel<3>, ln_fwd_kernel<4>};
 const LnKernel CHUNK_BWD[MAX_CH] = {ln_bwd_kernel<1>, ln_bwd_kernel<2>, ln_bwd_kernel<3>, ln_bwd_kernel<4>};
-struct LaneWidth { int d, form; LnKernel fwd, bwd; };
+using Ln2Add3Kernel = void (*)(const Ln2Add3Args);
+struct LaneWidth { int d, form; LnKernel fwd, bwd; Ln2Add3Kernel fwd2_add3; };
 template <int NV, int H8>
 constexpr LaneWidth lane_width_of() {
-  return {LaneCols<NV, H8>::D, 100 + 10 * NV + H8, ln_fwd_lane_kernel<NV, H8>, ln_bwd_lane_kernel<NV, H8>};
+  return {LaneCols<NV, H8>::D, 100 + 10 * NV + H8, ln_fwd_lane_kernel<NV, H8>, ln_bwd_lane_kernel<NV, H8>, ln2_add3_lane_kernel<NV, H8>};
 }
 const LaneWidth LANE_WIDTHS[] = {lane_width_of<0, 1>(), lane_width_of<1, 0>(), lane_width_of<1, 1>(), lane_width_of<2, 0>()};
 const LaneWidth* lane_width(int d) {
@@ -385,7 +458,11 @@
 
 int full_blocks(int rows) { return (rows + ROWS_PER_BLOCK - 1) / ROWS_PER_BLOCK; }
 
-int share_blocks(LnArgs& a, const mmf_ln_problem* problems, int num_problems, int budget) {
+int fwd_budget(long long total_rows) { return total_rows > FWD_LARGE_ROWS ? FWD_BLOCKS_LARGE : FWD_BLOCKS; }
+bool fwd_takes_lane_form(const LaneWidth* lw, int total, long long total_rows) { return lw && total > fwd_budget(total_rows); }
+
+template <class Args, class Problem>
+int share_blocks(Args& a, const Problem* problems, int num_problems, int budget) {
   long long total_rows = 0;
   for (int i = 0; i < num_problems; ++i) total_rows += problems[i].rows;
   int total = 0;
@@ -422,10 +499,9 @@
   }
   a.blk_start[num_problems] = total;
   hipStream_t s = static_cast<hipStream_t>(stream);
-  const int budget = total_rows > FWD_LARGE_ROWS ? FWD_BLOCKS_LARGE : FWD_BLOCKS;
   const LaneWidth* lw = lane_width(d);
-  if (lw && total > budget) {
-    total = share_blocks(a, problems, num_problems, budget);
+  if (fwd_takes_lane_form(lw, total, total_rows)) {
+    total = share_blocks(a, problems, num_problems, fwd_budget(total_rows));
     hipLaunchKernelGGL(lw->fwd, dim3(total), dim3(256), 0, s, a);
     t_last_form = lw->form;
     MMF_CHECK_LAUNCH("mmf_layernorm_fwd_grouped(lane)");
@@ -435,6 +511,41 @@
   hipLaunchKernelGGL(CHUNK_FWD[nch - 1], dim3(total), dim3(256), 0, s, a);
   t_last_form = nch;
   MMF_CHECK_LAUNCH("mmf_layernorm_fwd_grouped");
+  return MMF_OK;
+}
+
+extern "C" int mmf_layernorm2_add3_available(const int32_t* rows, int num_problems, int d) {
+  if (!rows || num_problems <= 0 || num_problems > MMF_LN2_ADD3_MAX_PROBLEMS) return 0;
+  int total = 0;
+  long long total_rows = 0;
+  for (int i = 0; i < num_problems; ++i) {
+    if (rows[i] <= 0) return 0;
+    total += 2 * full_blocks(rows[i]);
+    total_rows += 2LL * rows[i];
+  }
+  return fwd_takes_lane_form(lane_width(d), total, total_rows);
+}
+
+extern "C" int mmf_layernorm2_add3_fwd_grouped(const mmf_ln2_add3_problem* problems, int num_problems, int d, float eps, void* stream) {
+  const char* who = "mmf_layernorm2_add3_fwd_grouped";
+  if (!problems || num_problems <= 0 || num_problems > MMF_LN2_ADD3_MAX_PROBLEMS)
+    MMF_FAIL(MMF_E_SHAPE, "%s: num_problems=%d out of range", who, num_problems);
+  const LaneWidth* lw = lane_width(d);
+  if (!lw) MMF_FAIL(MMF_E_SHAPE, "%s: d=%d is no lane width: compose the two launches", who, d);
+  Ln2Add3Args a; a.nprob = num_problems; a.eps = eps;
+  for (int i = 0; i < num_problems; ++i) {
+    const mmf_ln2_add3_problem& p = problems[i];
+    if (p.rows <= 0 || !p.x || !p.pre_a || !p.pre_b || !p.e || !p.gamma_a || !p.beta_a || !p.gamma_b || !p.beta_b || !p.mean_a ||
+        !p.rstd_a || !p.mean_b || !p.rstd_b)
+      MMF_FAIL(MMF_E_SHAPE, "%s[%d]: null operand or rows=%d", who, i, p.rows);
+    if (!mmf_aligned16(p.x) || !mmf_aligned16(p.pre_a) || !mmf_aligned16(p.pre_b) || !mmf_aligned16(p.e) || !mmf_aligned16(p.gamma_a) ||
+        !mmf_aligned16(p.beta_a) || !mmf_aligned16(p.gamma_b) || !mmf_aligned16(p.beta_b))
+      MMF_FAIL(MMF_E_ALIGN, "%s[%d]: pointers must be 16-byte aligned", who, i);
+    a.p[i] = p;
+  }
+  const int total = share_blocks(a, problems, num_problems, FWD_BLOCKS);
+  hipLaunchKernelGGL(lw->fwd2_add3, dim3(total), dim3(256), 0, static_cast<hipStream_t>(stream), a);
+  MMF_CHECK_LAUNCH(who);
   return MMF_OK;
 }
 
diff --git a/simple-multimodal_amd/mmfusion/lib.py b/simple-multimodal_amd/mmfusion/lib.py
--- a/simple-multimodal_amd/mmfusion/lib.py
+++ b/simple-multimodal_amd/mmfusion/lib.py
@@ -9,15 +9,17 @@
 
 GEMM_NT, GEMM_NN, GEMM_TN = 0, 1, 2
 EPI_BIAS, EPI_RELU, EPI_MASK_AUX, EPI_ADD_AUX, EPI_ACCUM, EPI_COLSUM_A, EPI_DROPOUT = 1, 2, 4, 8, 16, 32, 64
+EPI_RELU_BITS, EPI_MASK_BITS = 128, 256
 GEMM_MAX_PROBLEMS, ATTN_MAX_PROBLEMS, LN_MAX_PROBLEMS, COLSUM_MAX_PROBLEMS = 48, 12, 8, 24
+LN2_ADD3_MAX_PROBLEMS = 4
 EVAL_MAX_HEADS, EVAL_NSUMS = 4, 4
 
 SYMBOLS = (
-    "mmf_version", "mmf_last_error", "mmf_device_cu_count", "mmf_gemm_grouped", "mmf_gemm_grouped_ex", "mmf_gemm_select_impl", "mmf_gemm_last_impl", "mmf_gemm_set_persistent_workgroups",
+    "mmf_version", "mmf_last_error", "mmf_device_cu_count", "mmf_gemm_grouped", "mmf_gemm_grouped_ex", "mmf_gemm_relu_bits_bytes", "mmf_gemm_relu_bits_available", "mmf_gemm_select_impl", "mmf_gemm_last_impl", "mmf_gemm_set_persistent_workgroups",
     "mmf_gemm7_set_tile_n", "mmf_gemm7_last_tile_n", "mmf_gemm7_tile_n",
     "mmf_attn_fwd_grouped_ex", "mmf_attn_bwd_grouped_ex", "mmf_dropout", "mmf_attn_select_impl",
     "mmf_attn_fwd_grouped", "mmf_attn_bwd_grouped", "mmf_layernorm_fwd_grouped",
-    "mmf_layernorm_bwd_grouped", "mmf_layernorm_bwd_workspace_bytes", "mmf_layernorm_last_form", "mmf_cast_f32_to_bf16", "mmf_cast_bf16_to_f32", "mmf_cast_bf16_to_f32_scaled", "mmf_cast_f32_to_bf16_2d", "mmf_add3_bf16", "mmf_add3_grouped", "mmf_addn_bf16", "mmf_addn_grouped",
+    "mmf_layernorm_bwd_grouped", "mmf_layernorm_bwd_workspace_bytes", "mmf_layernorm_last_form", "mmf_layernorm2_add3_available", "mmf_layernorm2_add3_fwd_grouped", "mmf_cast_f32_to_bf16", "mmf_cast_bf16_to_f32", "mmf_cast_bf16_to_f32_scaled", "mmf_cast_f32_to_bf16_2d", "mmf_add3_bf16", "mmf_add3_grouped", "mmf_addn_bf16", "mmf_addn_grouped",
     "mmf_meanpool_fwd", "mmf_meanpool_bwd", "mmf_meanpool_cat_fwd", "mmf_meanpool_cat_bwd", "mmf_colsum_bf16", "mmf_colsum_grouped", "mmf_relu_bwd_bf16", "mmf_relu_bwd_mixed",
     "mmf_sqnorm_f32", "mmf_adamw_step", "mmf_adamw_advance", "mmf_skinny_linear_fwd", "mmf_skinny_linear_dgrad", "mmf_skinny_linear_fwd_ex", "mmf_skinny_linear_dgrad_ex", "mmf_skinny_last_strip",
     "mmf_gat3_dense_fwd", "mmf_gat3_dense_bwd", "mmf_infonce_fwd", "mmf_infonce_bwd", "mmf_adaptive_combine_fwd",
@@ -55,6 +57,13 @@
                 ("dgamma", C.c_void_p), ("dbeta", C.c_void_p), ("rows", C.c_int32)]
 
 
+class Ln2Add3Problem(C.Structure):
+    _fields_ = [("x", C.c_void_p), ("pre_a", C.c_void_p), ("gamma_a", C.c_void_p), ("beta_a", C.c_void_p),
+                ("pre_b", C.c_void_p), ("gamma_b", C.c_void_p), ("beta_b", C.c_void_p), ("e", C.c_void_p),
+                ("mean_a", C.c_void_p), ("rstd_a", C.c_void_p), ("mean_b", C.c_void_p), ("rstd_b", C.c_void_p),
+                ("rows", C.c_int32)]
+
+
 class GemmExtra(C.Structure):
     _fields_ = [("alpha", C.c_float), ("dropout_p", C.c_float), ("rng_state", C.c_void_p), ("site", C.c_uint32)]
 
@@ -125,6 +134,9 @@
     vp, i32, i64, f32 = C.c_void_p, C.c_int, C.c_int64, C.c_float
     lib.mmf_gemm_grouped.argtypes = [C.POINTER(GemmProblem), i32, i32, i32, i32, vp]
     lib.mmf_gemm_grouped_ex.argtypes = [C.POINTER(GemmProblem), i32, i32, i32, i32, C.POINTER(GemmExtra), vp]
+    lib.mmf_gemm_relu_bits_bytes.argtypes = [i32, i32]
+    lib.mmf_gemm_relu_bits_bytes.restype = C.c_size_t
+    lib.mmf_gemm_relu_bits_available.argtypes = [C.POINTER(GemmProblem), i32, i32, i32, i32, C.POINTER(GemmExtra)]
     lib.mmf_gemm7_tile_n.argtypes = [C.POINTER(GemmProblem), i32, i32]
     lib.mmf_attn_fwd_grouped_ex.argtypes = [C.POINTER(AttnProblem), i32, i32, f32, f32, vp, C.c_uint32, vp]
     lib.mmf_attn_bwd_grouped_ex.argtypes = [C.POINTER(AttnProblem), i32, i32, f32, f32, vp, C.c_uint32, vp]
@@ -136,6 +148,8 @@
     lib.mmf_layernorm_bwd_grouped.argtypes = [C.POINTER(LnProblem), i32, i32, vp, C.c_size_t, vp]
     lib.mmf_layernorm_bwd_workspace_bytes.argtypes = [i32]
     lib.mmf_layernorm_bwd_workspace_bytes.restype = C.c_size_t
+    lib.mmf_layernorm2_add3_available.argtypes = [C.POINTER(C.c_int32), i32, i32]
+    lib.mmf_layernorm2_add3_fwd_grouped.argtypes = [C.POINTER(Ln2Add3Problem), i32, i32, f32, vp]
     lib.mmf_cast_f32_to_bf16.argtypes = [vp, vp, i64, vp]
     lib.mmf_cast_bf16_to_f32.argtypes = [vp, vp, i64, vp]
     lib.mmf_cast_bf16_to_f32_scaled.argtypes = [vp, vp, i64, f32, vp]
@@ -268,6 +282,13 @@
             tm.label = f"gemm{load().mmf_gemm_last_impl()}_grouped_kernel<{_LAYOUT_NAME[layout]},{'f32' if out_f32 else 'bf16'}>"
 
 
+def gemm_relu_bits_available(problems: Sequence[GemmProblem], layout: int, epilogue: int, alpha: float = 1.0,
+                             dropout_p: float = 0.0, rng_state_ptr: Optional[int] = None, site: int = 0) -> bool:
+    arr = (GemmProblem * len(problems))(*problems)
+    ex = GemmExtra(alpha, dropout_p, rng_state_ptr, site)
+    return bool(load().mmf_gemm_relu_bits_available(arr, len(problems), layout, epilogue, 0, C.byref(ex)))
+
+
 def attn_fwd_grouped(problems: Sequence[AttnProblem], head_dim: int, scale: float, dropout_p: float = 0.0,
                      rng_state_ptr: Optional[int] = None, site: int = 0) -> None:
     arr = (AttnProblem * len(problems))(*problems)
@@ -289,6 +310,16 @@
 def layernorm_fwd_grouped(problems: Sequence[LnProblem], d: int, eps: float) -> None:
     arr = (LnProblem * len(problems))(*problems)
     check(load().mmf_layernorm_fwd_grouped(arr, len(problems), d, eps, stream_ptr()))
+
+
+def layernorm2_add3_available(rows: Sequence[int], d: int) -> bool:
+    arr = (C.c_int32 * len(rows))(*rows)
+    return bool(load().mmf_layernorm2_add3_available(arr, len(rows), d))
+
+
+def layernorm2_add3_fwd_grouped(problems: Sequence[Ln2Add3Problem], d: int, eps: float) -> None:
+    arr = (Ln2Add3Problem * len(problems))(*problems)
+    check(load().mmf_layernorm2_add3_fwd_grouped(arr, len(problems), d, eps, stream_ptr()))
 
 
 def layernorm_bwd_grouped(problems: Sequence[LnProblem], d: int, workspace) -> None:
diff --git a/simple-multimodal_amd/mmfusion/ops.py b/simple-multimodal_amd/mmfusion/ops.py
--- a/simple-multimodal_amd/mmfusion/ops.py
+++ b/simple-multimodal_amd/mmfusion/ops.py
@@ -11,7 +11,7 @@
 
 from . import lib
 from .lib import (AttnProblem, GemmProblem, LnProblem, EPI_ACCUM, EPI_ADD_AUX, EPI_BIAS, EPI_COLSUM_A,
-                  EPI_DROPOUT, EPI_MASK_AUX, EPI_RELU, GEMM_NN, GEMM_NT, GEMM_TN)
+                  EPI_DROPOUT, EPI_MASK_AUX, EPI_MASK_BITS, EPI_RELU, EPI_RELU_BITS, GEMM_NN, GEMM_NT, GEMM_TN)
 
 BF16 = torch.bfloat16
 
@@ -139,6 +139,7 @@
 
 def _gemm_problems(layout: int, probs: Sequence[tuple], epilogue: int, dtype, c_dtype) -> List[GemmProblem]:
     ps: List[GemmProblem] = []
+    bits = bool(epilogue & (EPI_RELU_BITS | EPI_MASK_BITS))
     for (A, Bm, Cm, bias, aux) in probs:
         _req(A, dtype), _req(Bm, dtype)
         M, N = Cm.shape
@@ -146,15 +147,32 @@
         a_shape, b_shape = (K, M) if layout == GEMM_TN else (M, K), (N, K) if layout == GEMM_NT else (K, N)
         if A.shape != a_shape or Bm.shape != b_shape or Cm.dtype != c_dtype:
             raise ValueError(f"gemm layout {layout}: A{tuple(A.shape)} B{tuple(Bm.shape)} C{tuple(Cm.shape)} {Cm.dtype}")
-        if aux is not None and tuple(aux.shape) != (M, N):
+        if bits:
+            if aux is None or aux.dtype != torch.uint8 or not aux.is_contiguous() or aux.numel() < lib.load().mmf_gemm_relu_bits_bytes(M, N):
+                raise ValueError("the bit forms take a contiguous uint8 buffer of mmf_gemm_relu_bits_bytes(M, N) bytes as aux")
+        elif aux is not None and tuple(aux.shape) != (M, N):
             raise ValueError("aux must match C")
         if bias is not None:
             _req(bias, torch.float32)
             if bias.numel() != (M if epilogue & EPI_COLSUM_A else N) or not bias.is_contiguous():
                 raise ValueError("bias must be contiguous [N] ([M] for the fused bias gradient)")
         ps.append(GemmProblem(A.data_ptr(), Bm.data_ptr(), Cm.data_ptr(), _ptr(bias), _ptr(aux), M, N, K,
-                              _ld(A), _ld(Bm), _ld(Cm), _ld(aux) if aux is not None else 0))
+                              _ld(A), _ld(Bm), _ld(Cm), _ld(aux) if aux is not None and not bits else 0))
     return ps
+
+
+def relu_bits_buffer(h: torch.Tensor) -> torch.Tensor:
+    return torch.empty(lib.load().mmf_gemm_relu_bits_bytes(*h.shape), dtype=torch.uint8, device=h.device)
+
+
+def relu_bits_available(layout: int, probs: Sequence[tuple], epilogue: int, alpha: float = 1.0,
+                        dropout: Optional[tuple] = None) -> bool:
+    if len(probs) > lib.GEMM_MAX_PROBLEMS or probs[0][2].dtype != BF16:
+        return False
+    ps = _gemm_problems(layout, probs, epilogue, BF16, BF16)
+    if dropout is not None:
+        return lib.gemm_relu_bits_available(ps, layout, epilogue | EPI_DROPOUT, alpha, dropout[0], rng_state().data_ptr(), dropout[1])
+    return lib.gemm_relu_bits_available(ps, layout, epilogue, alpha)
 
 
 def gemm(layout: int, A: torch.Tensor, Bm: torch.Tensor, C: torch.Tensor, *, bias=None, aux=None,
@@ -745,33 +763,41 @@
 class _GroupedFFN(torch.autograd.Function):
 
     @staticmethod
-    def forward(ctx, layers, drop, *tensors):
+    def forward(ctx, layers, drop, want_bits, *tensors):
         n = len(layers)
         xs = [tensors[5 * i] for i in range(n)]
         for x in xs:
             _req(x, BF16)
         hs = [torch.empty((x.shape[0], l1.weight.shape[0]), dtype=BF16, device=x.device) for x, (l1, _) in zip(xs, layers)]
-        gemm_group(GEMM_NT, [(x, shadow(l1.weight), h, l1.bias.detach(), None)
-                             for x, h, (l1, _) in zip(xs, hs, layers)], EPI_BIAS | EPI_RELU, dropout=drop)
+        bits = [relu_bits_buffer(h) for h in hs] if want_bits else [None] * n
+        ffn1 = [(x, shadow(l1.weight), h, l1.bias.detach(), b) for x, h, b, (l1, _) in zip(xs, hs, bits, layers)]
+        if want_bits and relu_bits_available(GEMM_NT, ffn1, EPI_BIAS | EPI_RELU | EPI_RELU_BITS, dropout=drop):
+            gemm_group(GEMM_NT, ffn1, EPI_BIAS | EPI_RELU | EPI_RELU_BITS, dropout=drop)
+        else:
+            bits = []
+            gemm_group(GEMM_NT, [q[:4] + (None,) for q in ffn1], EPI_BIAS | EPI_RELU, dropout=drop)
         ctx.keep_scale = 1.0 / (1.0 - drop[0]) if drop is not None else 1.0
         ys = [torch.empty_like(x) for x in xs]
         gemm_group(GEMM_NT, [(h, shadow(l2.weight), y, l2.bias.detach(), x)
                              for x, h, y, (_, l2) in zip(xs, hs, ys, layers)], EPI_BIAS | EPI_ADD_AUX)
         ctx.layers = layers
-        ctx.save_for_backward(*xs, *hs)
+        ctx.save_for_backward(*xs, *hs, *bits)
         return tuple(ys)
 
     @staticmethod
     def backward(ctx, *gys):
         layers = ctx.layers
         n = len(layers)
-        xs, hs = ctx.saved_tensors[:n], ctx.saved_tensors[n:]
+        xs, hs, bits = ctx.saved_tensors[:n], ctx.saved_tensors[n:2 * n], ctx.saved_tensors[2 * n:]
         idx = [i for i, g in enumerate(gys) if g is not None]
         dys = {i: gys[i].contiguous() for i in idx}
         dhs = {i: torch.empty_like(hs[i]) for i in idx}
         dxs = {i: torch.empty_like(xs[i]) for i in idx}
-        gemm_group(GEMM_NN, [(dys[i], shadow(layers[i][1].weight), dhs[i], None, hs[i]) for i in idx], EPI_MASK_AUX,
-                   alpha=ctx.keep_scale)
+        dh = [(dys[i], shadow(layers[i][1].weight), dhs[i], None, bits[i] if bits else hs[i]) for i in idx]
+        if bits and relu_bits_available(GEMM_NN, dh, EPI_MASK_BITS, alpha=ctx.keep_scale):
+            gemm_group(GEMM_NN, dh, EPI_MASK_BITS, alpha=ctx.keep_scale)
+        else:
+            gemm_group(GEMM_NN, [q[:4] + (hs[i],) for q, i in zip(dh, idx)], EPI_MASK_AUX, alpha=ctx.keep_scale)
         gemm_group(GEMM_NN, [(dhs[i], shadow(layers[i][0].weight), dxs[i], None, dys[i]) for i in idx], EPI_ADD_AUX)
         for i in idx:
             for l, dy_, x_ in ((layers[i][1], dys[i], hs[i]), (layers[i][0], dhs[i], xs[i])):
@@ -780,7 +806,7 @@
         grads: List[Optional[torch.Tensor]] = [None] * (5 * n)
         for i in idx:
             grads[5 * i] = dxs[i]
-        return (None, None, *grads)
+        return (None, None, None, *grads)
 
 
 def ffn_residual_group(items: Sequence[tuple], dropout_p: float = 0.0) -> List[torch.Tensor]:
@@ -796,7 +822,8 @@
         layers.append((l1, l2))
         tensors += [x, l1.weight, l1.bias, l2.weight, l2.bias]
     drop = (float(dropout_p), next_site()) if dropout_p > 0.0 else None
-    return list(_GroupedFFN.apply(layers, drop, *tensors))
+    want_bits = torch.is_grad_enabled() and any(t.requires_grad for t in tensors)
+    return list(_GroupedFFN.apply(layers, drop, want_bits, *tensors))
 
 
 class _GroupedLayerNorm(torch.autograd.Function):
@@ -860,6 +887,73 @@
     for x, g, b in items:
         flat += [x, g, b]
     return list(_GroupedLayerNorm.apply(eps, *flat))
+
+
+class _GroupedLn2Add3(torch.autograd.Function):
+
+    @staticmethod
+    def forward(ctx, eps: float, *tensors):
+        n = len(tensors) // 7
+        d = tensors[0].shape[-1]
+        outs, stats, probs, keep = [], [], [], []
+        for i in range(n):
+            x, pa, ga, ba, pb, gb, bb = tensors[7 * i:7 * i + 7]
+            _req(x, BF16), _req(pa, BF16), _req(pb, BF16)
+            if x.shape != pa.shape or x.shape != pb.shape:
+                raise ValueError("ln2_add3 group: operands of one sum must have one shape")
+            x, pa, pb = x.contiguous(), pa.contiguous(), pb.contiguous()
+            keep += [x, pa, pb]
+            rows = x.numel() // d
+            e = torch.empty_like(x)
+            st = torch.empty((4, rows), dtype=torch.float32, device=x.device)
+            probs.append(lib.Ln2Add3Problem(x.data_ptr(), pa.data_ptr(), ga.data_ptr(), ba.data_ptr(), pb.data_ptr(), gb.data_ptr(),
+                                            bb.data_ptr(), e.data_ptr(), st[0].data_ptr(), st[1].data_ptr(), st[2].data_ptr(),
+                                            st[3].data_ptr(), rows))
+            outs.append(e), stats.append(st)
+        lib.layernorm2_add3_fwd_grouped(probs, d, eps)
+        ctx.n, ctx.d = n, d
+        ctx.params = [tuple(tensors[7 * i + j] for j in (2, 3, 5, 6)) for i in range(n)]
+        ctx.save_for_backward(*[keep[3 * i + j] for i in range(n) for j in (1, 2)], *stats)
+        return tuple(outs)
+
+    @staticmethod
+    def backward(ctx, *gs):
+        n, d = ctx.n, ctx.d
+        pres, stats = ctx.saved_tensors[:2 * n], ctx.saved_tensors[2 * n:]
+        grads: List[Optional[torch.Tensor]] = [None] * (7 * n)
+        probs, keep = [], []
+        for i, g in enumerate(gs):
+            if g is None:
+                continue
+            g = g.contiguous()
+            keep.append(g)
+            grads[7 * i] = g
+            for j in (0, 1):
+                pre, gamma, beta = pres[2 * i + j], ctx.params[i][2 * j], ctx.params[i][2 * j + 1]
+                if gamma.grad is None or beta.grad is None:
+                    raise RuntimeError("LayerNorm parameters have no arena gradient")
+                dx = torch.empty_like(pre)
+                probs.append(LnProblem(pre.data_ptr(), None, gamma.data_ptr(), None, stats[i][2 * j].data_ptr(),
+                                       stats[i][2 * j + 1].data_ptr(), g.data_ptr(), dx.data_ptr(),
+                                       gamma.grad.data_ptr(), beta.grad.data_ptr(), pre.numel() // d))
+                grads[7 * i + 1 + 3 * j] = dx
+        if probs:
+            ws = torch.empty(lib.load().mmf_layernorm_bwd_workspace_bytes(d) // 4, dtype=torch.float32, device=pres[0].device)
+            keep.append(ws)
+            lib.layernorm_bwd_grouped(probs, d, ws)
+        return (None, *grads)
+
+
+def ln2_add3_group(items: Sequence[tuple], eps: float = 1e-5) -> List[torch.Tensor]:
+    rows = [x.numel() // x.shape[-1] for x, *_ in items]
+    if (_PRECISION == "fp32" or len(items) > lib.LN2_ADD3_MAX_PROBLEMS
+            or not lib.layernorm2_add3_available(rows, items[0][0].shape[-1])):
+        ys = layernorm_group([(pre, nm.weight, nm.bias) for _, pa, na, pb, nb in items for pre, nm in ((pa, na), (pb, nb))], eps)
+        return add3_group([(x, ys[2 * i], ys[2 * i + 1]) for i, (x, *_) in enumerate(items)])
+    flat = []
+    for x, pa, na, pb, nb in items:
+        flat += [x, pa, na.weight, na.bias, pb, nb.weight, nb.bias]
+    return list(_GroupedLn2Add3.apply(eps, *flat))
 
 
 @dataclass
diff --git a/simple-multimodal_amd/models/fusion_layers.py b/simple-multimodal_amd/models/fusion_layers.py
--- a/simple-multimodal_amd/models/fusion_layers.py
+++ b/simple-multimodal_amd/models/fusion_layers.py
@@ -128,12 +128,12 @@
 
 def _cross_blocks(blocks: Sequence["CrossModalTransformer"], qs: Sequence[torch.Tensor],
                   kvs: Sequence[torch.Tensor], B: int, Tqs: Sequence[int], Tks: Sequence[int],
-                  p: float = 0.0, ress: Optional[Sequence[torch.Tensor]] = None) -> List[torch.Tensor]:
+                  p: float = 0.0, ress: Optional[Sequence[torch.Tensor]] = None, norm2: bool = True) -> List[torch.Tensor]:
     proj = _cross_in_proj(blocks, qs, kvs)
     _tick()
     att = _cross_attention(blocks, proj, B, Tqs, Tks, p)
     _tick()
-    return _cross_tail(blocks, att, qs if ress is None else ress, p)
+    return _cross_tail(blocks, att, qs if ress is None else ress, p, norm2)
 
 
 def _cross_in_proj(blocks, qs, kvs) -> List[torch.Tensor]:
@@ -152,7 +152,7 @@
     return ops.attention_group(specs, H, dh, proj, dropout_p=p)
 
 
-def _cross_tail(blocks, att, qs, p) -> List[torch.Tensor]:
+def _cross_tail(blocks, att, qs, p, norm2: bool = True) -> List[torch.Tensor]:
     pre1 = ops.linear_group([(att[i], _lin(blk.attention.out_proj), qs[i]) for i, blk in enumerate(blocks)])
     _tick()
     x = ops.layernorm_group([(pre1[i], blk.norm1.weight, blk.norm1.bias) for i, blk in enumerate(blocks)],
@@ -160,8 +160,15 @@
     _tick()
     pre2 = ops.ffn_residual_group([(x[i], blk.ffn[0], blk.ffn[3]) for i, blk in enumerate(blocks)], dropout_p=p)
     _tick()
+    if not norm2:
+        return pre2
     return ops.layernorm_group([(pre2[i], blk.norm2.weight, blk.norm2.bias) for i, blk in enumerate(blocks)],
                                blocks[0].norm2.eps)
+
+
+def _norm2_sums(blocks, xs, pre2) -> List[torch.Tensor]:
+    return ops.ln2_add3_group([(x, pre2[2 * i], blocks[2 * i].norm2, pre2[2 * i + 1], blocks[2 * i + 1].norm2)
+                               for i, x in enumerate(xs)], blocks[0].norm2.eps)
 
 
 def _self_attention_core(mhas: Sequence[_MHAParams], xs: Sequence[torch.Tensor], B: int, Ts: Sequence[int],
@@ -275,9 +282,9 @@
 
             def chain(ms):
                 g = [2 * m + j for m in ms for j in (0, 1)]
-                outs = _cross_blocks([blocks[i] for i in g], [qs[i] for i in g], [kvs[i] for i in g], B,
-                                     [Tqs[i] for i in g], [Tks[i] for i in g], p, [ress[i] for i in g])
-                es = ops.add3_group([(xs3[m], outs[2 * i], outs[2 * i + 1]) for i, m in enumerate(ms)])
+                pre2 = _cross_blocks([blocks[i] for i in g], [qs[i] for i in g], [kvs[i] for i in g], B,
+                                     [Tqs[i] for i in g], [Tks[i] for i in g], p, [ress[i] for i in g], norm2=False)
+                es = _norm2_sums([blocks[i] for i in g], [xs3[m] for m in ms], pre2)
                 return _self_attention_core([mhas[m] for m in ms], es, B, [Ts3[m] for m in ms], p)
             main = torch.cuda.current_stream()
             side = ops.branch_stream(1)
@@ -289,8 +296,8 @@
             for x in att_side:
                 x.record_stream(main)
         else:
-            t_a, t_v, a_t, a_v, v_t, v_a = _cross_blocks(blocks, qs, kvs, B, Tqs, Tks, p, ress)
-            et, ea, ev = ops.add3_group([(t, t_a, t_v), (a, a_t, a_v), (v, v_t, v_a)])
+            pre2 = _cross_blocks(blocks, qs, kvs, B, Tqs, Tks, p, ress, norm2=False)
+            et, ea, ev = _norm2_sums(blocks, [t, a, v], pre2)
             att = _self_attention_core(mhas, [et, ea, ev], B, [Tt, Ta, Tv], p)
         pooled_att = ops.meanpool_cat([att[0].view(B, Tt, d), att[1].view(B, Ta, d), att[2].view(B, Tv, d)])
         pf = ops.linear_group([(x, _lin(m.out_proj), None) for x, m in zip(sops.split3(pooled_att), mhas)],
```

New measurement: 7713 (median of 6 runs). 1.01x the previous value.
